# pierrebarbera/epa-ng

Measured on AMD Instinct MI355X. Metric: query placements/sec (whole node), 512-tip GTR+G4 DNA ref, preplace+thorough, higher is better.
Workload: dtype f64; 1 GPU; cfg2: 512-tip DNA GTR+G4 ref, W=1500, 150 bp reads, dyn-heur 0.99999, preplace+thorough; branches=1021, parallelism=query-shard x1 (weak)

## Files before the change

epa_ng_amd/api.py:

```python
import ctypes as C
import os

import numpy as np

HERE = os.path.dirname(os.path.abspath(__file__))
DEV_SO = os.environ.get("EPA_DEV_SO", os.path.join(HERE, "libepa_dev.so"))

__all__ = ["EpaError", "dev_lib", "device_count", "encode_queries", "Evaluator", "PAIR_DTYPE",
           "RESULT_DTYPE", "ROW_DTYPE", "DEV_SO", "Packed4", "pack_codes_4bit", "unpack_codes_4bit", "Comm",
           "comm_unique_id", "mapped_rccl_path", "comm_set_library", "comm_library_path", "comm_set_default_timeout",
           "pci_id_str", "FLAG_LOOKUP_BLOCKS", "FLAG_LOOKUP_AUTO", "LOOKUP_RESIDENT", "LOOKUP_BLOCKS", "ERR_NO_MEMORY",
           "footprint", "lookup_plan", "set_mem_cap", "quadrature_legendre01", "quadrature_laguerre", "posterior_rule",
           "profile_from_phred"]

FLAG_LOOKUP_BLOCKS = 0x40
FLAG_LOOKUP_AUTO = 0x80
LOOKUP_RESIDENT = 0
LOOKUP_BLOCKS = 1
ERR_NO_MEMORY = -10

PAIR_DTYPE = np.dtype([("branch_id", np.uint32), ("seq_id", np.uint32)])
RESULT_DTYPE = np.dtype([("lnl", np.float64), ("pendant_length", np.float64),
                         ("distal_length", np.float64)])

ROW_DTYPE = np.dtype([("branch_id", np.uint32), ("seq_id", np.uint32), ("lnl", np.float64),
                      ("pendant_length", np.float64), ("distal_length", np.float64)])


class EpaError(RuntimeError):
    def __init__(self, code, msg):
        super().__init__("epa_dev error %d: %s" % (code, msg))
        self.code = code


class _RefDesc(C.Structure):
    _fields_ = [("states", C.c_uint32), ("rate_cats", C.c_uint32), ("sites", C.c_uint32),
                ("branches", C.c_uint32),
                ("eigenvals", C.c_void_p), ("eigenvecs_u", C.c_void_p),
                ("eigenvecs_uinv", C.c_void_p), ("freqs", C.c_void_p), ("rates", C.c_void_p),
                ("rate_weights", C.c_void_p), ("prop_invar", C.c_double),
                ("prox_clv", C.c_void_p), ("prox_scaler", C.c_void_p), ("dist_clv", C.c_void_p),
                ("dist_tipchars", C.c_void_p), ("dist_scaler", C.c_void_p),
                ("branch_length", C.c_void_p),
                ("tipmap", C.c_void_p), ("tipmap_size", C.c_uint32),
                ("blo_min_branch", C.c_double), ("blo_max_branch", C.c_double),
                ("blo_default_branch", C.c_double), ("blo_epsilon", C.c_double),
                ("pendant_default", C.c_double), ("blo_max_rounds", C.c_uint32),
                ("blo_max_newton", C.c_uint32), ("flags", C.c_uint32), ("aa_x_as_n", C.c_uint32),
                ("invariant_state", C.c_void_p)]


class _Stats(C.Structure):
    _fields_ = [("pairs", C.c_uint64), ("rounds", C.c_uint64), ("newton_evals", C.c_uint64),
                ("reverts", C.c_uint64)]


class _Footprint(C.Structure):
    _fields_ = [(n, C.c_uint64) for n in ("reft", "scsum", "lookup", "lookup2", "refi", "misc", "create_temp",
                                          "reference", "bank", "steady", "peak")]


_LIB = None


def dev_lib():
    global _LIB
    if _LIB is None:
        if not os.path.exists(DEV_SO):
            raise ImportError("libepa_dev.so is missing: run `python __graft_entry__.py` "
                              "(build()) -- the HIP extension is the only compute path")
        try:
            import torch
            if torch.cuda.is_available():
                torch.cuda.init()
        except ImportError:
            pass
        L = C.CDLL(DEV_SO)
        L.epa_dev_device_count.restype = C.c_int
        L.epa_dev_create.argtypes = [C.POINTER(_RefDesc), C.c_int, C.POINTER(C.c_void_p)]
        L.epa_dev_destroy.argtypes = [C.c_void_p]
        L.epa_dev_last_error.restype = C.c_char_p
        L.epa_dev_last_error.argtypes = [C.c_void_p]
        L.epa_dev_set_stream.argtypes = [C.c_void_p, C.c_void_p]
        L.epa_dev_build_lookup.argtypes = [C.c_void_p]
        L.epa_dev_set_option.argtypes = [C.c_void_p, C.c_char_p, C.c_int]
        L.epa_encode_queries.argtypes = [C.c_uint32, C.c_uint32, C.c_uint32,
                                         C.POINTER(C.c_char_p), C.c_int, C.c_int, C.c_void_p,
                                         C.c_void_p, C.c_void_p, C.POINTER(C.c_uint32)]
        L.epa_encode_queries_compact.argtypes = [C.c_uint32, C.c_uint32, C.c_uint32,
                                                 C.POINTER(C.c_char_p), C.c_int, C.c_int, C.c_uint32,
                                                 C.c_void_p, C.c_void_p, C.c_void_p,
                                                 C.POINTER(C.c_uint32)]
        L.epa_dev_set_query_layout.argtypes = [C.c_void_p, C.c_uint32]
        L.epa_dev_preplace.argtypes = [C.c_void_p, C.c_void_p, C.c_void_p, C.c_void_p, C.c_uint32,
                                       C.c_void_p]
        L.epa_dev_preplace_bounded.argtypes = [C.c_void_p, C.c_void_p, C.c_void_p, C.c_void_p, C.c_uint32, C.c_uint32,
                                               C.c_void_p, C.c_void_p]
        L.epa_dev_preplace_screen_probe.argtypes = [C.c_void_p, C.c_void_p, C.c_void_p, C.c_void_p, C.c_uint32, C.c_uint32,
                                                    C.c_double, C.c_void_p, C.c_void_p, C.c_void_p]
        L.epa_dev_preplace_screen_runs.argtypes = [C.c_void_p]
        L.epa_dev_preplace_screen_runs.restype = C.c_uint64
        L.epa_dev_thorough.argtypes = [C.c_void_p, C.c_void_p, C.c_uint64, C.c_void_p, C.c_void_p,
                                       C.c_void_p, C.c_uint32, C.c_void_p, C.POINTER(_Stats)]
        L.epa_dev_score_at.argtypes = [C.c_void_p, C.c_void_p, C.c_void_p, C.c_void_p, C.c_void_p, C.c_uint64,
                                       C.c_void_p, C.c_void_p, C.c_void_p, C.c_uint32, C.c_void_p]
        L.epa_dev_site_lnl.argtypes = [C.c_void_p, C.c_void_p, C.c_void_p, C.c_void_p, C.c_void_p, C.c_uint64,
                                       C.c_void_p, C.c_void_p, C.c_void_p, C.c_uint32, C.c_uint32, C.c_void_p]
        L.epa_dev_rell_support.argtypes = [C.c_void_p, C.c_void_p, C.c_void_p, C.c_void_p, C.c_void_p, C.c_uint64,
                                           C.c_void_p, C.c_void_p, C.c_void_p, C.c_uint32, C.c_void_p, C.c_uint32,
                                           C.c_uint64, C.c_void_p]
        L.epa_dev_rell_tests.argtypes = L.epa_dev_rell_support.argtypes + [C.c_void_p, C.c_void_p]
        L.epa_dev_rell_au.argtypes = L.epa_dev_rell_support.argtypes[:-1] + [C.c_void_p, C.c_uint32, C.c_void_p, C.c_void_p,
                                                                             C.c_void_p]
        L.epa_dev_rell_kh.argtypes = L.epa_dev_rell_tests.argtypes
        L.epa_dev_marginal_like.argtypes = [C.c_void_p, C.c_void_p, C.c_uint64, C.c_void_p, C.c_void_p, C.c_uint32,
                                            C.c_void_p, C.c_void_p, C.c_uint32, C.c_void_p, C.c_void_p, C.c_void_p,
                                            C.c_uint32, C.c_void_p, C.c_void_p]
        L.epa_dev_preplace_profile.argtypes = [C.c_void_p, C.c_void_p, C.c_uint32, C.c_void_p, C.c_void_p, C.c_uint32,
                                               C.c_void_p]
        L.epa_dev_thorough_profile.argtypes = [C.c_void_p, C.c_void_p, C.c_uint64, C.c_void_p, C.c_uint32, C.c_void_p,
                                               C.c_void_p, C.c_uint32, C.c_void_p, C.POINTER(_Stats)]
        L.epa_dev_score_at_profile.argtypes = [C.c_void_p, C.c_void_p, C.c_void_p, C.c_void_p, C.c_void_p, C.c_uint64,
                                               C.c_void_p, C.c_uint32, C.c_void_p, C.c_void_p, C.c_uint32, C.c_void_p]
        L.epa_dev_site_lnl_profile.argtypes = [C.c_void_p, C.c_void_p, C.c_void_p, C.c_void_p, C.c_void_p, C.c_uint64,
                                               C.c_void_p, C.c_uint32, C.c_void_p, C.c_void_p, C.c_uint32, C.c_uint32,
                                               C.c_void_p]
        L.epa_dev_place_chunk_profile.argtypes = [C.c_void_p, C.c_void_p, C.c_uint32, C.c_void_p, C.c_void_p, C.c_uint32,
                                                  C.c_double, C.c_void_p, C.c_void_p, C.c_uint64, C.POINTER(C.c_uint64),
                                                  C.POINTER(_Stats)]
        L.epa_profile_from_phred.argtypes = [C.c_uint32, C.c_uint32, C.c_uint32, C.c_void_p, C.c_void_p, C.c_void_p,
                                             C.c_void_p]
        L.epa_quadrature_legendre01.argtypes = [C.c_uint32, C.c_void_p, C.c_void_p]
        L.epa_quadrature_laguerre.argtypes = [C.c_uint32, C.c_void_p, C.c_void_p]
        L.epa_dev_set_heuristic.argtypes = [C.c_void_p, C.c_int, C.c_double]
        L.epa_dev_set_query_packing.argtypes = [C.c_void_p, C.c_int]
        L.epa_pack_codes_4bit.argtypes = [C.c_void_p, C.c_uint32, C.c_uint32, C.c_void_p]
        L.epa_unpack_codes_4bit.argtypes = [C.c_void_p, C.c_uint32, C.c_uint32, C.c_void_p]
        L.epa_dev_select_candidates.argtypes = [C.c_void_p, C.c_void_p, C.c_uint32, C.c_double,
                                                C.c_void_p, C.c_uint64, C.POINTER(C.c_uint64)]
        L.epa_dev_place_chunk.argtypes = [C.c_void_p, C.c_void_p, C.c_void_p, C.c_void_p, C.c_uint32,
                                          C.c_uint32, C.c_double, C.c_void_p, C.c_void_p,
                                          C.c_uint64, C.POINTER(C.c_uint64), C.POINTER(_Stats)]
        L.epa_dev_dedup_queries.argtypes = [C.c_void_p, C.c_void_p, C.c_void_p, C.c_void_p, C.c_uint32, C.c_void_p,
                                            C.c_void_p, C.POINTER(C.c_uint32)]
        L.epa_dev_place_chunk_dedup.argtypes = [C.c_void_p, C.c_void_p, C.c_void_p, C.c_void_p, C.c_uint32, C.c_uint32,
                                                C.c_double, C.c_void_p, C.c_void_p, C.c_uint64, C.POINTER(C.c_uint64),
                                                C.POINTER(_Stats), C.c_void_p, C.c_void_p, C.POINTER(C.c_uint32)]
        L.epa_dev_chunk_stage.argtypes = [C.c_void_p, C.c_int, C.c_void_p, C.c_void_p, C.c_void_p, C.c_uint32]
        L.epa_dev_chunk_launch.argtypes = [C.c_void_p, C.c_int, C.c_uint32, C.c_double, C.c_void_p,
                                           C.c_void_p, C.c_uint64, C.c_uint32]
        L.epa_dev_chunk_launch_begin.argtypes = [C.c_void_p, C.c_int, C.c_uint32, C.c_double, C.c_void_p,
                                           C.c_void_p, C.c_uint64, C.c_uint32]
        L.epa_dev_chunk_launch_end.argtypes = [C.c_void_p, C.c_int]
        L.epa_dev_chunk_launch_many_begin.argtypes = [C.c_void_p, C.POINTER(C.c_int), C.c_int, C.c_uint32, C.c_double,
                                                      C.c_uint64, C.c_uint32]
        L.epa_dev_chunk_launch_many.argtypes = L.epa_dev_chunk_launch_many_begin.argtypes
        L.epa_dev_chunk_finish.argtypes = [C.c_void_p, C.c_int, C.POINTER(C.c_void_p),
                                           C.POINTER(C.c_void_p), C.POINTER(C.c_uint64), C.POINTER(_Stats)]
        L.epa_dev_tree_logl.argtypes = [C.c_void_p, C.c_uint32, C.POINTER(C.c_double)]
        L.epa_dev_place_all.argtypes = [C.c_void_p, C.c_void_p, C.c_void_p, C.c_void_p, C.c_uint32,
                                        C.c_uint32, C.c_double, C.c_int, C.c_uint32, C.c_uint32,
                                        C.c_void_p, C.c_void_p, C.c_void_p, C.c_void_p,
                                        C.POINTER(_Stats)]
        L.epa_comm_get_unique_id.argtypes = [C.c_void_p]
        L.epa_comm_create.argtypes = [C.c_void_p, C.c_void_p, C.c_int, C.c_int, C.c_uint32, C.c_int,
                                      C.POINTER(C.c_void_p)]
        L.epa_comm_destroy.argtypes = [C.c_void_p]
        L.epa_comm_destroy.restype = None
        L.epa_dev_gather_results.argtypes = [C.c_void_p, C.c_void_p, C.c_void_p, C.c_void_p, C.c_uint64,
                                             C.c_uint32, C.POINTER(C.c_uint64)]
        L.epa_dev_gather_slot.argtypes = [C.c_void_p, C.c_void_p, C.c_int, C.c_uint32, C.POINTER(C.c_uint64)]
        L.epa_comm_collect.argtypes = [C.c_void_p, C.c_uint64, C.POINTER(C.c_void_p), C.POINTER(C.c_uint32),
                                       C.POINTER(C.c_uint64)]
        L.epa_comm_flush.argtypes = [C.c_void_p, C.c_void_p, C.POINTER(C.c_uint64), C.POINTER(C.c_uint32)]
        L.epa_comm_carried_rows.argtypes = [C.c_void_p]
        L.epa_comm_carried_rows.restype = C.c_uint64
        L.epa_dev_gather_rows.argtypes = [C.c_void_p, C.c_void_p, C.c_void_p, C.c_uint64, C.POINTER(C.c_uint64)]
        L.epa_dev_place_all_rows.argtypes = [C.c_void_p, C.c_void_p, C.c_void_p, C.c_void_p, C.c_uint32, C.c_uint32, C.c_double,
                                             C.c_int, C.c_uint32, C.c_uint32, C.c_uint32, C.POINTER(C.c_void_p),
                                             C.POINTER(C.c_uint64), C.c_void_p]
        L.epa_comm_abort.argtypes = [C.c_void_p]
        L.epa_comm_abort.restype = None
        L.epa_comm_set_library.argtypes = [C.c_char_p]
        L.epa_comm_library_path.restype = C.c_char_p
        L.epa_comm_set_timeout.argtypes = [C.c_void_p, C.c_double]
        L.epa_comm_probe.argtypes = [C.c_void_p, C.c_void_p, C.c_double, C.POINTER(C.c_uint64)]
        L.epa_comm_set_self_send.argtypes = [C.c_void_p, C.c_int]
        L.epa_comm_device_rows.argtypes = [C.c_void_p, C.c_uint64, C.c_int]
        L.epa_comm_device_rows.restype = C.c_void_p
        L.epa_dev_mem_info.argtypes = [C.c_void_p, C.POINTER(C.c_uint64), C.POINTER(C.c_uint64)]
        L.epa_dev_xcd_shares.argtypes = [C.c_void_p, C.POINTER(C.c_double)]
        L.epa_dev_xcd_shares.restype = C.c_int
        L.epa_dev_last_kernel_ms.restype = C.c_double
        L.epa_dev_last_sclk_mhz.argtypes = [C.c_void_p]
        L.epa_dev_last_sclk_mhz.restype = C.c_double
        L.epa_dev_last_kernel_ms.argtypes = [C.c_void_p, C.c_char_p]
        L.epa_dev_footprint.argtypes = [C.c_uint32, C.c_uint32, C.c_uint64, C.c_uint64, C.c_int, C.c_int, C.c_uint32,
                                        C.c_int, C.POINTER(_Footprint)]
        L.epa_dev_lookup_plan.argtypes = [C.c_uint64, C.c_uint32, C.c_uint32, C.c_uint64, C.c_uint64, C.c_int, C.c_int,
                                          C.c_int, C.POINTER(C.c_int), C.POINTER(C.c_uint32)]
        L.epa_dev_set_mem_cap.argtypes = [C.c_uint64]
        L.epa_dev_set_mem_cap.restype = None
        L.epa_dev_lookup_mode.argtypes = [C.c_void_p, C.POINTER(C.c_int), C.POINTER(C.c_uint32)]
        _LIB = L
    return _LIB


def device_count():
    return dev_lib().epa_dev_device_count()


def footprint(states, rate_cats, sites, branches, flags=0, from_tree=False, block_branches=0, banks=1):
    L = dev_lib()
    f = _Footprint()
    rc = L.epa_dev_footprint(states, rate_cats, sites, branches, int(flags), int(from_tree), block_branches, banks,
                             C.byref(f))
    if rc:
        raise EpaError(rc, (L.epa_dev_last_error(None) or b"").decode())
    return {n: int(getattr(f, n)) for n, _ in _Footprint._fields_}


def lookup_plan(usable_bytes, states, rate_cats, sites, branches, flags=0, from_tree=False, banks=1):
    L = dev_lib()
    mode, blk = C.c_int(0), C.c_uint32(0)
    rc = L.epa_dev_lookup_plan(int(usable_bytes), states, rate_cats, sites, branches, int(flags), int(from_tree), banks,
                               C.byref(mode), C.byref(blk))
    if rc:
        raise EpaError(rc, (L.epa_dev_last_error(None) or b"").decode())
    return mode.value, blk.value


def set_mem_cap(nbytes):
    dev_lib().epa_dev_set_mem_cap(int(nbytes))


class Packed4:

    def __init__(self, data, stride):
        self.data, self.stride = data, int(stride)


def pack_codes_4bit(codes):
    codes = np.ascontiguousarray(codes, np.uint8)
    Q, stride = codes.shape
    out = np.zeros((Q, (stride + 1) // 2), np.uint8)
    rc = dev_lib().epa_pack_codes_4bit(codes.ctypes.data, Q, stride, out.ctypes.data)
    if rc:
        raise EpaError(rc, "pack_codes_4bit: a code does not fit four bits")
    return Packed4(out, stride)


def unpack_codes_4bit(p):
# ... 68 lines not shown
                                       wb.ctypes.data, ws.ctypes.data, C.byref(bad)))
    stride = (int(ws.max()) + 15) // 16 * 16
    if stride == W:
        stride += 16
    codes = np.zeros((Q, stride), np.uint8)
    check(L.epa_encode_queries_compact(states, W, Q, arr, int(premasking), int(aa_x_as_n), stride,
                                       codes.ctypes.data, wb.ctypes.data, ws.ctypes.data, C.byref(bad)))
    return codes, wb, ws


def profile_from_phred(states, codes, phred, win_span, out=None):
    codes = np.ascontiguousarray(codes, np.uint8)
    phred = np.ascontiguousarray(phred, np.uint8)
    win_span = np.ascontiguousarray(win_span, np.uint32)
    if codes.ndim != 2 or phred.shape != codes.shape or len(win_span) != codes.shape[0]:
        raise ValueError("profile_from_phred: codes and phred must be [Q][stride] arrays of one shape, win_span [Q]")
    Q, stride = codes.shape
    if out is None:
        out = np.zeros((Q, stride, states), np.float64)
    assert out.shape == (Q, stride, states) and out.dtype == np.float64 and out.flags["C_CONTIGUOUS"]
    L = dev_lib()
    rc = L.epa_profile_from_phred(states, Q, stride, codes.ctypes.data, phred.ctypes.data, win_span.ctypes.data,
                                  out.ctypes.data)
    if rc:
        raise EpaError(rc, (L.epa_dev_last_error(None) or b"").decode())
    return out


class Evaluator:

    def __init__(self, states, rates, weights, eigenvals, u, uinv, freqs, branch_length,
                 prox_clv, dist_clv, prox_scaler=None, dist_scaler=None, dist_tip=None,
                 tipmap=None, device=0, aa_x_as_n=False, pinv=0.0, invariant_state=None, flags=0):
        L = dev_lib()
        B = len(branch_length)
        self.B, self.s, self.c = B, states, len(rates)
        W = None
        for a in list(prox_clv):
            W = a.shape[0]
            break
        self.W = W
        f64 = lambda a: np.ascontiguousarray(a, dtype=np.float64)
        keep = [f64(eigenvals), f64(u), f64(uinv), f64(freqs), f64(rates), f64(weights),
                f64(branch_length)]

        def ptr_array(items, dtype):
            arr = (C.c_void_p * B)()
            held = []
            for i, it in enumerate(items if items is not None else [None] * B):
                if it is None:
                    arr[i] = None
                else:
                    a = np.ascontiguousarray(it, dtype=dtype)
                    held.append(a)
                    arr[i] = a.ctypes.data
            return arr, held

        pc, h1 = ptr_array(prox_clv, np.float64)
        dc, h2 = ptr_array(dist_clv, np.float64)
        ps, h3 = ptr_array(prox_scaler, np.uint32)
        ds, h4 = ptr_array(dist_scaler, np.uint32)
        dt, h5 = ptr_array(dist_tip, np.uint8)
        tm = np.ascontiguousarray(tipmap, dtype=np.uint32) if tipmap is not None else None
        d = _RefDesc()
        d.states, d.rate_cats, d.sites, d.branches = states, self.c, W, B
        d.eigenvals, d.eigenvecs_u, d.eigenvecs_uinv = (keep[0].ctypes.data, keep[1].ctypes.data,
                                                       keep[2].ctypes.data)
        d.freqs, d.rates, d.rate_weights = keep[3].ctypes.data, keep[4].ctypes.data, keep[5].ctypes.data
        d.prop_invar = float(pinv)
        inv = None
        if invariant_state is not None:
            inv = np.ascontiguousarray(invariant_state, dtype=np.int8)
            d.invariant_state = inv.ctypes.data
        d.prox_clv = C.cast(pc, C.c_void_p)
        d.prox_scaler = C.cast(ps, C.c_void_p)
        d.dist_clv = C.cast(dc, C.c_void_p)
        d.dist_tipchars = C.cast(dt, C.c_void_p) if dist_tip is not None else None
        d.dist_scaler = C.cast(ds, C.c_void_p)
        d.branch_length = keep[6].ctypes.data
        if tm is not None:
            d.tipmap, d.tipmap_size = tm.ctypes.data, len(tm)
        d.aa_x_as_n = int(aa_x_as_n)
        d.flags = int(flags)
        h = C.c_void_p()
        rc = L.epa_dev_create(C.byref(d), device, C.byref(h))
        if rc:
            raise EpaError(rc, L.epa_dev_last_error(None).decode())
        self.h = h
        self.L = L
        self.last_stats = None

    def close(self):
        if getattr(self, "h", None):
            self.L.epa_dev_destroy(self.h)
            self.h = None

    def __del__(self):
        self.close()

    def _check(self, rc):
        if rc:
            raise EpaError(rc, self.L.epa_dev_last_error(self.h).decode())

    def set_stream(self, stream_ptr):
        self._check(self.L.epa_dev_set_stream(self.h, stream_ptr))

    def set_option(self, key, value=1):
        self._check(self.L.epa_dev_set_option(self.h, key.encode(), int(value)))

    def build_lookup(self):
        self._check(self.L.epa_dev_build_lookup(self.h))

    def _layout(self, codes):
        packed = isinstance(codes, Packed4)
        row = codes.stride if packed else (int(codes.shape[1]) if len(codes.shape) == 2 else self.W)
        self._check(self.L.epa_dev_set_query_layout(self.h, 0 if row == self.W else row))
        self._check(self.L.epa_dev_set_query_packing(self.h, 4 if packed else 8))

    def preplace(self, codes, win_begin, win_span, Q=None, out=None):
        Q = len(win_begin) if Q is None else Q
        if out is None:
            out = np.empty((Q, self.B), np.float64)
        self._layout(codes)
        self._check(self.L.epa_dev_preplace(self.h, _ptr(codes), _ptr(win_begin), _ptr(win_span),
                                            Q, _ptr(out)))
        return out

    def preplace_bounded(self, codes, win_begin, win_span, max_span, seg_keys=False):
        Q = len(win_begin)
        out = np.empty((Q, self.B), np.float64)
        keys = np.zeros((Q, ((self.B + 63) // 64 + 7) // 8 * 8), np.uint64) if seg_keys else None
        self._layout(codes)
        self._check(self.L.epa_dev_preplace_bounded(self.h, _ptr(codes), _ptr(win_begin), _ptr(win_span), Q,
                                                    int(max_span), _ptr(out), _ptr(keys)))
        return (out, keys) if seg_keys else out

    def preplace_screen_runs(self):
        return int(self.L.epa_dev_preplace_screen_runs(self.h))

    def preplace_screen_probe(self, codes, win_begin, win_span, max_span, threshold=0.99999, arrays=True):
        Q = len(win_begin)
        nseg = (self.B + 63) // 64
        seg32 = np.full((Q, nseg), np.nan, np.float32) if arrays else None
        mask = np.zeros(Q, np.uint64) if arrays else None
        info = np.zeros(8, np.float64)
        self._layout(codes)
        self._check(self.L.epa_dev_preplace_screen_probe(self.h, _ptr(codes), _ptr(win_begin), _ptr(win_span), Q,
                                                         int(max_span), float(threshold), _ptr(seg32), _ptr(mask),
                                                         _ptr(info)))
        return {"ran": bool(info[0]), "delta": float(info[1]), "included": int(info[2]), "M": float(info[3]),
                "nonfinite": int(info[4]), "band_t": float(info[5]), "ms_screen": float(info[6]),
                "ms_band": float(info[7]), "seg32": seg32, "mask": mask}

    def thorough(self, pairs, codes, win_begin, win_span, Q=None, n_pairs=None, out=None):
        Q = len(win_begin) if Q is None else Q
        n = len(pairs) if n_pairs is None else n_pairs
        if out is None:
            out = np.empty(n, RESULT_DTYPE)
        st = _Stats()
        self._layout(codes)
        self._check(self.L.epa_dev_thorough(self.h, _ptr(pairs), n, _ptr(codes), _ptr(win_begin),
                                            _ptr(win_span), Q, _ptr(out), C.byref(st)))
        self.last_stats = {"pairs": st.pairs, "rounds": st.rounds,
                           "newton_evals": st.newton_evals, "reverts": st.reverts}
        return out

    def _entries(self, pairs, pendant, distal, proximal, codes, win_begin, Q, stream_id=None):
        n, Q = len(pairs), (len(win_begin) if Q is None else Q)
        host = (np.ndarray, list, tuple)
        pendant, distal, proximal = (np.ascontiguousarray(a, dtype=np.float64) if isinstance(a, host) else a
                                     for a in (pendant, distal, proximal))
        if isinstance(stream_id, host):
            stream_id = np.ascontiguousarray(stream_id, dtype=np.uint64)
        self._layout(codes)
        return n, Q, pendant, distal, proximal, stream_id

    @staticmethod
    def _want(who, want, table):
        want = tuple(want)
        unknown = [w for w in want if w not in table]
        if unknown:
            raise ValueError("%s: unknown output %r" % (who, unknown[0]))
        return {w: np.empty(*table[w]) for w in want}

    def score_at(self, pairs, pendant, distal, codes, win_begin, win_span, proximal=None, Q=None, out=None):
        n, Q, pendant, distal, proximal, _ = self._entries(pairs, pendant, distal, proximal, codes, win_begin, Q)
        if out is None:
            out = np.empty(n, np.float64)
        self._check(self.L.epa_dev_score_at(self.h, _ptr(pairs), _ptr(pendant), _ptr(distal), _ptr(proximal), n,
                                            _ptr(codes), _ptr(win_begin), _ptr(win_span), Q, _ptr(out)))
        return out

    def site_lnl(self, pairs, pendant, distal, codes, win_begin, win_span, proximal=None, pitch=None, Q=None, out=None):
        n, Q, pendant, distal, proximal, _ = self._entries(pairs, pendant, distal, proximal, codes, win_begin, Q)
        if pitch is None:
            pitch = int(np.max(np.asarray(win_span)[:Q])) if Q else 0
        if out is None:
            out = np.empty((n, int(pitch)), np.float64)
        self._check(self.L.epa_dev_site_lnl(self.h, _ptr(pairs), _ptr(pendant), _ptr(distal), _ptr(proximal), n,
                                            _ptr(codes), _ptr(win_begin), _ptr(win_span), Q, int(pitch), _ptr(out)))
        return out

    def marginal_like(self, pairs, codes, win_begin, win_span, x_frac, x_logw, p_len, p_logw, Q=None, out=None, grid=False):
        n, Q = self._entries(pairs, None, None, None, codes, win_begin, Q)[:2]
        x_frac, x_logw, p_len, p_logw = (np.ascontiguousarray(a, dtype=np.float64) for a in (x_frac, x_logw, p_len, p_logw))
        if x_frac.shape != x_logw.shape or p_len.shape != p_logw.shape or x_frac.ndim != 1 or p_len.ndim != 1:
            raise ValueError("marginal_like: nodes and log weights must be 1-d arrays of equal length")
        Kx, Kp = len(x_frac), len(p_len)
        if out is None:
            out = np.empty(n, np.float64)
        g = np.empty((n, Kx, Kp), np.float64) if grid else None
        self._check(self.L.epa_dev_marginal_like(self.h, _ptr(pairs), n, _ptr(x_frac), _ptr(x_logw), Kx, _ptr(p_len),
                                                 _ptr(p_logw), Kp, _ptr(codes), _ptr(win_begin), _ptr(win_span), Q,
                                                 _ptr(out), _ptr(g)))
        return (out, g) if grid else out

    def rell_support(self, pairs, pendant, distal, codes, win_begin, win_span, replicates, seed=1, stream_id=None,
                     proximal=None, Q=None, out=None):
        n, Q, pendant, distal, proximal, stream_id = self._entries(pairs, pendant, distal, proximal, codes, win_begin, Q,
                                                                   stream_id)
        if out is None:
            out = np.empty(n, np.float64)
        self._check(self.L.epa_dev_rell_support(self.h, _ptr(pairs), _ptr(pendant), _ptr(distal), _ptr(proximal), n,
                                                _ptr(codes), _ptr(win_begin), _ptr(win_span), Q, _ptr(stream_id),
                                                int(replicates), int(seed), _ptr(out)))
        return out

    def rell_tests(self, pairs, pendant, distal, codes, win_begin, win_span, replicates, seed=1, stream_id=None,
                   proximal=None, want=("support", "elw", "p_sh"), Q=None):
        out = self._want("rell_tests", want, {w: ((len(pairs),), np.float64) for w in ("support", "elw", "p_sh")})
        n, Q, pendant, distal, proximal, stream_id = self._entries(pairs, pendant, distal, proximal, codes, win_begin, Q,
                                                                   stream_id)
        self._check(self.L.epa_dev_rell_tests(self.h, _ptr(pairs), _ptr(pendant), _ptr(distal), _ptr(proximal), n,
                                              _ptr(codes), _ptr(win_begin), _ptr(win_span), Q, _ptr(stream_id),
                                              int(replicates), int(seed), _ptr(out.get("support")), _ptr(out.get("elw")),
                                              _ptr(out.get("p_sh"))))
        return out

    def rell_au(self, pairs, pendant, distal, codes, win_begin, win_span, replicates, seed=1, stream_id=None,
                proximal=None, scales=None, want=("p_au", "counts", "fit"), Q=None):
        n, S = len(pairs), (10 if scales is None else np.size(scales))
        out = self._want("rell_au", want, {"p_au": ((n,), np.float64), "counts": ((S, n), np.uint32), "fit": ((n, 2), np.float64)})
        if scales is not None:
            scales = np.ascontiguousarray(scales, dtype=np.uint32)
            if scales.ndim != 1 or len(scales) == 0:
                raise ValueError("rell_au: scales must be a non-empty 1-d array (None: the default scales)")
        n, Q, pendant, distal, proximal, stream_id = self._entries(pairs, pendant, distal, proximal, codes, win_begin, Q,
                                                                   stream_id)
        self._check(self.L.epa_dev_rell_au(self.h, _ptr(pairs), _ptr(pendant), _ptr(distal), _ptr(proximal), n,
                                           _ptr(codes), _ptr(win_begin), _ptr(win_span), Q, _ptr(stream_id),
                                           int(replicates), int(seed), _ptr(scales), 0 if scales is None else S,
                                           _ptr(out.get("p_au")), _ptr(out.get("counts")), _ptr(out.get("fit"))))
        return out

    def rell_kh(self, pairs, pendant, distal, codes, win_begin, win_span, replicates, seed=1, stream_id=None,
                proximal=None, want=("p_kh", "p_wkh", "p_wsh"), Q=None):
        out = self._want("rell_kh", want, {w: ((len(pairs),), np.float64) for w in ("p_kh", "p_wkh", "p_wsh")})
        n, Q, pendant, distal, proximal, stream_id = self._entries(pairs, pendant, distal, proximal, codes, win_begin, Q,
                                                                   stream_id)
        self._check(self.L.epa_dev_rell_kh(self.h, _ptr(pairs), _ptr(pendant), _ptr(distal), _ptr(proximal), n,
                                           _ptr(codes), _ptr(win_begin), _ptr(win_span), Q, _ptr(stream_id),
                                           int(replicates), int(seed), _ptr(out.get("p_kh")), _ptr(out.get("p_wkh")),
                                           _ptr(out.get("p_wsh"))))
        return out

    @staticmethod
    def _prof(prof):
        if isinstance(prof, np.ndarray):
            prof = np.ascontiguousarray(prof, dtype=np.float64)
        return prof, int(prof.shape[1])

    def _stats(self, st):
        self.last_stats = {"pairs": st.pairs, "rounds": st.rounds, "newton_evals": st.newton_evals, "reverts": st.reverts}

    def preplace_profile(self, prof, win_begin, win_span, Q=None, out=None):
        Q = len(win_begin) if Q is None else Q
        prof, stride = self._prof(prof)
        if out is None:
            out = np.empty((Q, self.B), np.float64)
        self._check(self.L.epa_dev_preplace_profile(self.h, _ptr(prof), stride, _ptr(win_begin), _ptr(win_span), Q, _ptr(out)))
        return out

    def thorough_profile(self, pairs, prof, win_begin, win_span, Q=None, n_pairs=None, out=None):
        Q = len(win_begin) if Q is None else Q
        n = len(pairs) if n_pairs is None else n_pairs
        prof, stride = self._prof(prof)
        if out is None:
            out = np.empty(n, RESULT_DTYPE)
        st = _Stats()
        self._check(self.L.epa_dev_thorough_profile(self.h, _ptr(pairs), n, _ptr(prof), stride, _ptr(win_begin), _ptr(win_span),
                                                    Q, _ptr(out), C.byref(st)))
        self._stats(st)
        return out

    def _profile_entries(self, pairs, pendant, distal, proximal, win_begin, Q):
        host = (np.ndarray, list, tuple)
        pendant, distal, proximal = (np.ascontiguousarray(a, dtype=np.float64) if isinstance(a, host) else a
                                     for a in (pendant, distal, proximal))
        return len(pairs), (len(win_begin) if Q is None else Q), pendant, distal, proximal

    def score_at_profile(self, pairs, pendant, distal, prof, win_begin, win_span, proximal=None, Q=None, out=None):
        n, Q, pendant, distal, proximal = self._profile_entries(pairs, pendant, distal, proximal, win_begin, Q)
        prof, stride = self._prof(prof)
        if out is None:
            out = np.empty(n, np.float64)
        self._check(self.L.epa_dev_score_at_profile(self.h, _ptr(pairs), _ptr(pendant), _ptr(distal), _ptr(proximal), n,
# ... 335 lines not shown
```

epa_ng_amd/build.py:

```python
import os
import subprocess
import sys

HERE = os.path.dirname(os.path.abspath(__file__))
ROOT = os.path.dirname(HERE)
CSRC = os.path.join(HERE, "csrc")
HIPCC = os.environ.get("HIPCC", "/opt/rocm/bin/hipcc")

DEV_SOURCES = ["epa_dev.hip", "chunk.hip", "preplace.hip", "select.hip", "thorough_dna.hip", "thorough_dna_tipd.hip", "thorough_dna_tipd2h.hip", "thorough_aa.hip", "thorough_aa_mfma.hip", "thorough_generic.hip", "score_at.hip", "marginal.hip", "rell.hip", "profile.hip", "dedup.hip", "comm.hip"]
EXTRA_FLAGS = {"thorough_dna.hip": ["-mllvm", "-amdgpu-sched-strategy=iterative-ilp"],
               "thorough_dna_tipd.hip": ["-mllvm", "-amdgpu-sched-strategy=iterative-ilp"],
               "thorough_aa_mfma.hip": ["-mllvm", "-amdgpu-sched-strategy=iterative-ilp"]}
EXTRA_DEPS = {"thorough_dna_tipd.hip": ["thorough_dna.hip"], "thorough_dna_tipd2h.hip": ["thorough_dna.hip"]}
DEV_FLAGS = ["--offload-arch=gfx950", "-O3", "-std=c++17", "-fPIC", "-I", os.path.join(ROOT, "include"),
             "-I", CSRC, "-Wall", "-Wno-unused-function", "-Wno-unused-result"]


def _newer(target, deps):
    if not os.path.exists(target):
        return True
    t = os.path.getmtime(target)
    return any(os.path.getmtime(d) > t for d in deps)


def build_dev(force=False, verbose=False):
    out = os.path.join(HERE, "libepa_dev.so")
    objdir = os.path.join(HERE, "build")
    os.makedirs(objdir, exist_ok=True)
    hdrs = [os.path.join(CSRC, "epa_dev_internal.hpp"), os.path.join(CSRC, "wave_util.hpp"), os.path.join(CSRC, "rccl_abi.hpp"),
            os.path.join(ROOT, "include", "epa_dev.h")]
    objs, procs = [], []
    for src in DEV_SOURCES:
        sp = os.path.join(CSRC, src)
        op = os.path.join(objdir, src.replace(".hip", ".o"))
        objs.append(op)
        if force or _newer(op, [sp] + hdrs + [os.path.join(CSRC, d) for d in EXTRA_DEPS.get(src, [])]):
            cmd = [HIPCC] + DEV_FLAGS + EXTRA_FLAGS.get(src, []) + ["-c", sp, "-o", op]
            if verbose:
                print(" ".join(cmd), file=sys.stderr)
            procs.append((src, subprocess.Popen(cmd), [HIPCC] + DEV_FLAGS + ["-c", sp, "-o", op]))
    for src, p, plain in procs:
        if p.wait() != 0:
            if not EXTRA_FLAGS.get(src) or subprocess.call(plain) != 0:
                raise RuntimeError("hipcc failed on " + src)
    if force or procs or _newer(out, objs):
        cmd = [HIPCC, "--offload-arch=gfx950", "-shared", "-fPIC", "-o", out + ".tmp"] + objs
        subprocess.check_call(cmd)
        os.replace(out + ".tmp", out)
    return out


HOST_SOURCES = ["model.cpp", "aa_models.cpp", "parse_model.cpp", "tree.cpp", "place.cpp", "place_ranks.cpp", "rescore.cpp", "place_profile.cpp", "place_dedup.cpp", "io.cpp", "capi.cpp"]
HOST_FLAGS = ["-O2", "-std=c++17", "-fPIC", "-fopenmp", "-Wall", "-Wextra", "-Wno-unused-parameter",
              "-I", os.path.join(ROOT, "include")]


def build_host(force=False, verbose=False):
    hdir = os.path.join(CSRC, "host")
    out = os.path.join(HERE, "libepa_host.so")
    exe = os.path.join(HERE, "epa-ng-amd")
    srcs = [os.path.join(hdir, s) for s in HOST_SOURCES]
    deps = srcs + [os.path.join(hdir, "epa_host.hpp"), os.path.join(ROOT, "include", "epa_dev.h")]
    link = ["-L", HERE, "-lepa_dev", "-Wl,-rpath,$ORIGIN"]
    if force or _newer(out, deps):
        cmd = ["g++"] + HOST_FLAGS + ["-shared", "-o", out + ".tmp"] + srcs + link
        if verbose:
            print(" ".join(cmd), file=sys.stderr)
        subprocess.check_call(cmd)
        os.replace(out + ".tmp", out)
    main = os.path.join(hdir, "main.cpp")
    if force or _newer(exe, deps + [main, out]):
        cmd = ["g++"] + HOST_FLAGS + ["-o", exe + ".tmp", main, "-L", HERE, "-lepa_host", "-lepa_dev",
                                      "-Wl,-rpath,$ORIGIN"]
        subprocess.check_call(cmd)
        os.replace(exe + ".tmp", exe)
    return out


if __name__ == "__main__":
    print(build_dev(force="--force" in sys.argv, verbose=True))
    print(build_host(force="--force" in sys.argv, verbose=True))
```

epa_ng_amd/csrc/epa_dev.hip:

```cpp
#include "epa_dev_internal.hpp"

#include <math.h>
#include <string.h>

#include <algorithm>
#include <numeric>
#include <atomic>
#include <thread>

static thread_local std::string g_create_err;

int epa_fail(epa_ctx* ctx, int code, const std::string& msg) {
  if (ctx) ctx->err = msg; else g_create_err = msg;
  return code;
}

namespace {
__global__ void __launch_bounds__(256) k_zero(uint4* __restrict__ a, size_t na, uint4* __restrict__ b, size_t nb) {
  const size_t stride = (size_t)gridDim.x * 256, i0 = (size_t)blockIdx.x * 256 + threadIdx.x;
  const uint4 z = make_uint4(0u, 0u, 0u, 0u);
  for (size_t i = i0; i < na; i += stride) a[i] = z;
  for (size_t i = i0; i < nb; i += stride) b[i] = z;
}
}
// ... 412 lines not shown
        memset(out + (hi - lo), 0, stride - (hi - lo));
      }
    }
  };
  if (nt == 1) {
    work(0);
  } else {
    std::vector<std::thread> th;
    for (unsigned t = 0; t < nt; ++t) th.emplace_back(work, t);
    for (auto& x : th) x.join();
  }
  for (unsigned t = 0; t < nt; ++t)
    if (code[t] != EPA_OK) { if (bad_query) *bad_query = bad[t]; return code[t]; }
  return EPA_OK;
}

extern "C" int epa_encode_queries(uint32_t states, uint32_t sites, uint32_t Q,
                                  const char* const* seqs, int premasking, int aa_x_as_n,
                                  uint8_t* codes, uint32_t* win_begin, uint32_t* win_span,
                                  uint32_t* bad_query) {
  return encode_impl(states, sites, Q, seqs, premasking, aa_x_as_n, false, 0, codes, win_begin, win_span,
                     bad_query);
}

extern "C" int epa_encode_queries_compact(uint32_t states, uint32_t sites, uint32_t Q,
                                          const char* const* seqs, int premasking, int aa_x_as_n,
                                          uint32_t stride, uint8_t* codes, uint32_t* win_begin,
                                          uint32_t* win_span, uint32_t* bad_query) {
  if (stride && !codes) return EPA_ERR_INVALID_ARG;
  return encode_impl(states, sites, Q, seqs, premasking, aa_x_as_n, true, stride, codes, win_begin,
                     win_span, bad_query);
}

namespace {
void tridiag_eigenvalues(const std::vector<double>& d, const std::vector<double>& o, std::vector<double>& ev) {
  const size_t K = d.size();
  double lo = d[0], hi = d[0];
  for (size_t i = 0; i < K; ++i) {
    const double r = (i ? std::fabs(o[i - 1]) : 0.0) + (i + 1 < K ? std::fabs(o[i]) : 0.0);
    lo = std::min(lo, d[i] - r);
    hi = std::max(hi, d[i] + r);
  }
  auto below = [&](double x) {
    size_t n = 0;
    double q = 1.0;
    for (size_t i = 0; i < K; ++i) {
      q = d[i] - x - (i ? o[i - 1] * o[i - 1] / q : 0.0);
      if (q == 0.0) q = 1e-300;
      if (q < 0.0) ++n;
    }
    return n;
  };
  ev.resize(K);
  for (size_t j = 0; j < K; ++j) {
    double a = lo, b = hi;
    for (int it = 0; it < 200 && b - a > 4e-16 * std::max(std::fabs(a), std::fabs(b)); ++it) {
      const double mid = 0.5 * (a + b);
      if (below(mid) > j) b = mid; else a = mid;
    }
    ev[j] = 0.5 * (a + b);
  }
}

double log_sum_exp(const double* v, uint32_t K) {
  double mx = v[0], sum = 0.0;
  for (uint32_t j = 1; j < K; ++j) mx = std::max(mx, v[j]);
  for (uint32_t j = 0; j < K; ++j) sum += std::exp(v[j] - mx);
  return mx + std::log(sum);
}
}

extern "C" int epa_quadrature_legendre01(uint32_t K, double* nodes, double* log_weights) {
  if (K < 1 || K > 64 || !nodes || !log_weights) return EPA_ERR_INVALID_ARG;
  std::vector<double> d(K, 0.0), o(K > 1 ? K - 1 : 0), x;
  for (uint32_t i = 1; i < K; ++i) o[i - 1] = (double)i / std::sqrt(4.0 * i * i - 1.0);
  tridiag_eigenvalues(d, o, x);
  for (uint32_t j = 0; j < K; ++j) {
    double t = x[j], dp = 1.0;
    for (int it = 0; it < 3; ++it) {
      double p0 = 1.0, p1 = t;
      for (uint32_t n = 1; n < K; ++n) { const double p2 = ((2.0 * n + 1.0) * t * p1 - n * p0) / (n + 1.0); p0 = p1; p1 = p2; }
      dp = K * (t * p1 - p0) / (t * t - 1.0);
      if (it < 2) t -= p1 / dp;
    }
    nodes[j] = 0.5 * (1.0 + t);
    log_weights[j] = -std::log((1.0 - t) * (1.0 + t)) - 2.0 * std::log(std::fabs(dp));
  }
  const double norm = log_sum_exp(log_weights, K);
  for (uint32_t j = 0; j < K; ++j) log_weights[j] -= norm;
  return EPA_OK;
}

extern "C" int epa_quadrature_laguerre(uint32_t K, double* nodes, double* log_weights) {
  if (K < 1 || K > 64 || !nodes || !log_weights) return EPA_ERR_INVALID_ARG;
  std::vector<double> d(K), o(K > 1 ? K - 1 : 0), x;
  for (uint32_t i = 0; i < K; ++i) d[i] = 2.0 * i + 1.0;
  for (uint32_t i = 1; i < K; ++i) o[i - 1] = (double)i;
  tridiag_eigenvalues(d, o, x);
  for (uint32_t j = 0; j < K; ++j) {
    double t = x[j], lm = 1.0;
    for (int it = 0; it < 3; ++it) {
      double l0 = 1.0, l1 = 1.0 - t;
      for (uint32_t n = 1; n < K; ++n) { const double l2 = ((2.0 * n + 1.0 - t) * l1 - n * l0) / (n + 1.0); l0 = l1; l1 = l2; }
      lm = l0;
      if (it < 2) t -= l1 * t / (K * (l1 - l0));
    }
    nodes[j] = t;
    log_weights[j] = std::log(t) - 2.0 * std::log((double)K) - 2.0 * std::log(std::fabs(lm));
  }
  const double norm = log_sum_exp(log_weights, K);
  for (uint32_t j = 0; j < K; ++j) log_weights[j] -= norm;
  return EPA_OK;
}

extern "C" int epa_dev_device_count(void) {
  int n = 0;
  if (hipGetDeviceCount(&n) != hipSuccess) { (void)hipGetLastError(); return 0; }
  return n;
}

extern "C" const char* epa_dev_last_error(const epa_ctx* ctx) {
  return ctx ? ctx->err.c_str() : g_create_err.c_str();
}

extern "C" int epa_dev_set_query_layout(epa_ctx* ctx, uint32_t code_stride) {
  if (!ctx) return EPA_ERR_INVALID_ARG;
  ctx->code_stride = code_stride;
  return EPA_OK;
}

extern "C" int epa_dev_set_option(epa_ctx* ctx, const char* key, int value) {
  if (!ctx || !key) return EPA_ERR_INVALID_ARG;
  if (strcmp(key, "lookup_block") == 0) {
    if (!ctx->lookup_blocks) return epa_fail(ctx, EPA_ERR_INVALID_ARG, "set_option: lookup_block needs a context in the blocked lookup layout");
    if (value <= 0 || (value & 63)) return epa_fail(ctx, EPA_ERR_INVALID_ARG, "set_option: lookup_block must be a positive multiple of 64");
    for (void* p : ctx->blk_buf)
      if (p) return epa_fail(ctx, EPA_ERR_INVALID_ARG, "set_option: lookup_block must be set before the first preplacement");
    ctx->lookup_block = (uint32_t)value;
    return EPA_OK;
  }
  const bool dedup_key = strcmp(key, "dedup_key_bits") == 0;
  if (dedup_key || strcmp(key, "dedup_sort_bits") == 0) {
    if (value < 0 || value > 64) return epa_fail(ctx, EPA_ERR_INVALID_ARG, std::string("set_option: ") + key + " must be 0 .. 64");
    (dedup_key ? ctx->opt.dedup_key_bits : ctx->opt.dedup_sort_bits) = value;
    return EPA_OK;
  }
  struct Entry { const char* name; int EpaOptions::*field; };
  static const Entry table[] = {
      {"thorough_generic", &EpaOptions::thorough_generic}, {"preplace_generic", &EpaOptions::preplace_generic},
      {"select_full_rows", &EpaOptions::select_full_rows}, {"select_sort", &EpaOptions::select_sort},
      {"queued_thorough", &EpaOptions::queued_thorough},   {"xcd_balance", &EpaOptions::xcd_balance},
      {"aa_valu", &EpaOptions::aa_valu},                   {"timers", &EpaOptions::timers},
      {"newton_lds", &EpaOptions::newton_lds},             {"tip_distal", &EpaOptions::tip_distal},
      {"preplace_screen", &EpaOptions::preplace_screen},   {"preplace_screen_scale", &EpaOptions::preplace_screen_scale}};
  for (const Entry& e : table)
    if (strcmp(key, e.name) == 0) {
      ctx->opt.*e.field = value;
      ctx->generic_thorough = ctx->generic_native || ctx->opt.thorough_generic != 0;
      return EPA_OK;
    }
  return epa_fail(ctx, EPA_ERR_INVALID_ARG, std::string("set_option: unknown key '") + key + "'");
}

extern "C" int epa_dev_set_heuristic(epa_ctx* ctx, int mode, double param) {
  if (!ctx) return EPA_ERR_INVALID_ARG;
  if (mode < EPA_HEUR_DYNAMIC || mode > EPA_HEUR_BASEBALL)
    return epa_fail(ctx, EPA_ERR_INVALID_ARG, "set_heuristic: unknown mode");
  if (mode == EPA_HEUR_FIXED && !(param >= 0.0 && param <= 1.0))
    return epa_fail(ctx, EPA_ERR_INVALID_ARG, "set_heuristic: the fraction must lie in [0, 1]");
  ctx->heur_mode = mode;
  ctx->heur_param = param;
  return EPA_OK;
}

extern "C" int epa_dev_set_query_packing(epa_ctx* ctx, int bits) {
  if (!ctx) return EPA_ERR_INVALID_ARG;
  if (bits != 8 && bits != 4) return epa_fail(ctx, EPA_ERR_INVALID_ARG, "set_query_packing: 8 or 4 bits per code");
  if (bits == 4 && ctx->s != 4)
    return epa_fail(ctx, EPA_ERR_UNSUPPORTED, "set_query_packing: the 4-bit format holds nucleotide codes only");
  ctx->code_packed4 = bits == 4;
  return EPA_OK;
}

extern "C" int epa_pack_codes_4bit(const uint8_t* codes, uint32_t Q, uint32_t stride, uint8_t* packed) {
  if (!codes || !packed) return EPA_ERR_INVALID_ARG;
  const size_t ps = ((size_t)stride + 1) / 2;
  const unsigned cap = g_encode_threads.load(std::memory_order_relaxed);
  const unsigned hw = cap ? cap : std::max(1u, std::thread::hardware_concurrency());
  const unsigned nt = (unsigned)std::min<uint64_t>(std::min(hw, 32u), std::max<uint64_t>(1, (uint64_t)Q * stride >> 20));
  std::vector<int> bad(nt, 0);
  auto work = [&](unsigned t) {
    const uint32_t q0 = (uint32_t)((uint64_t)Q * t / nt), q1 = (uint32_t)((uint64_t)Q * (t + 1) / nt);
    unsigned over = 0;
    for (uint32_t q = q0; q < q1; ++q) {
      const uint8_t* r = codes + (size_t)q * stride;
      uint8_t* o = packed + (size_t)q * ps;
      for (uint32_t p = 0; p < stride / 2; ++p) {
        const uint8_t hi = r[2 * p], lo = r[2 * p + 1];
        over |= hi | lo;
        o[p] = (uint8_t)((hi << 4) | lo);
      }
      if (stride & 1) { const uint8_t hi = r[stride - 1]; over |= hi; o[ps - 1] = (uint8_t)(hi << 4); }
    }
    bad[t] = over > 15;
  };
  if (nt == 1) work(0);
  else {
    std::vector<std::thread> th;
    for (unsigned t = 0; t < nt; ++t) th.emplace_back(work, t);
    for (auto& x : th) x.join();
  }
  for (unsigned t = 0; t < nt; ++t) if (bad[t]) return EPA_ERR_INVALID_ARG;
  return EPA_OK;
}

extern "C" int epa_unpack_codes_4bit(const uint8_t* packed, uint32_t Q, uint32_t stride, uint8_t* codes) {
  if (!codes || !packed) return EPA_ERR_INVALID_ARG;
  const size_t ps = ((size_t)stride + 1) / 2;
  for (uint32_t q = 0; q < Q; ++q)
    for (uint32_t i = 0; i < stride; ++i) {
      const uint8_t b = packed[(size_t)q * ps + i / 2];
      codes[(size_t)q * stride + i] = (i & 1) ? (b & 15u) : (b >> 4);
    }
  return EPA_OK;
}

extern "C" int epa_dev_set_stream(epa_ctx* ctx, void* s) {
  if (!ctx) return EPA_ERR_INVALID_ARG;
  ctx->stream = (hipStream_t)s;
  return EPA_OK;
}

extern "C" void epa_dev_destroy(epa_ctx* ctx) {
  if (!ctx) return;
  (void)hipSetDevice(ctx->device);
  (void)hipDeviceSynchronize();
  for (int i = 0; i < epa_ctx::N_BANKS * epa_ctx::N_SCRATCH; ++i) if (ctx->scratch[i]) (void)hipFree(ctx->scratch[i]);
  if (ctx->refT) (void)hipFree(ctx->refT);
  if (ctx->scSum) (void)hipFree(ctx->scSum);
  if (ctx->blen) (void)hipFree(ctx->blen);
  if (ctx->lookup) (void)hipFree(ctx->lookup);
  if (ctx->lookup2) (void)hipFree(ctx->lookup2);
  if (ctx->lookup2f) (void)hipFree(ctx->lookup2f);
  if (ctx->prof_tab) (void)hipFree(ctx->prof_tab);
  for (void* p : ctx->blk_buf) if (p) (void)hipFree(p);
  for (auto& v : ctx->blk_ev) for (hipEvent_t e : v) if (e) (void)hipEventDestroy(e);
  if (ctx->th_ctr) (void)hipFree(ctx->th_ctr);
  for (hipEvent_t e : ctx->ev_rb) if (e) (void)hipEventDestroy(e);
  if (ctx->refI) (void)hipFree(ctx->refI);
  if (ctx->cinv) (void)hipFree(ctx->cinv);
  if (ctx->resc0) (void)hipFree(ctx->resc0);
  if (ctx->tip_row) (void)hipFree(ctx->tip_row);
  if (ctx->tipmask) (void)hipFree(ctx->tipmask);
  if (ctx->tipd) (void)hipFree(ctx->tipd);
  for (hipStream_t st : ctx->side_stream) if (st) (void)hipStreamDestroy(st);
  for (hipEvent_t e : ctx->ev_fork) if (e) (void)hipEventDestroy(e);
  for (hipEvent_t e : ctx->ev_join) if (e) (void)hipEventDestroy(e);
  if (ctx->dmodel) (void)hipFree(ctx->dmodel);
  for (ChunkSlot& sl : ctx->slots) {
    if (sl.h_in) (void)hipHostFree(sl.h_in);
    if (sl.h_out) (void)hipHostFree(sl.h_out);
    if (sl.h_stats) (void)hipHostFree(sl.h_stats);
    if (sl.h_sel) (void)hipHostFree(sl.h_sel);
    if (sl.d_in) (void)hipFree(sl.d_in);
    if (sl.d_unpacked) (void)hipFree(sl.d_unpacked);
    if (sl.d_pairs) (void)hipFree(sl.d_pairs);
    if (sl.d_res) (void)hipFree(sl.d_res);
    if (sl.d_stats) (void)hipFree(sl.d_stats);
    if (sl.d_merge) (void)hipFree(sl.d_merge);
    if (sl.d_gpairs) (void)hipFree(sl.d_gpairs);
    if (sl.d_gres) (void)hipFree(sl.d_gres);
    if (sl.d_goff) (void)hipFree(sl.d_goff);
    if (sl.h_goff) (void)hipHostFree(sl.h_goff);
    for (hipEvent_t e : {sl.ev_up, sl.ev_done, sl.ev_down, sl.ev_base}) if (e) (void)hipEventDestroy(e);
    if (sl.stream) (void)hipStreamDestroy(sl.stream);
  }
  if (ctx->copy_stream) (void)hipStreamDestroy(ctx->copy_stream);
  if (ctx->down_stream) (void)hipStreamDestroy(ctx->down_stream);
  std::vector<EvTimer*> ts = {&ctx->t_lookup};
  for (auto& bk : ctx->t_bank) for (auto& t : bk) ts.push_back(&t);
  for (auto* t : ts) { if (t->a) (void)hipEventDestroy(t->a); if (t->b) (void)hipEventDestroy(t->b); }
  delete ctx;
}

static int precompute_from_tree(epa_ctx* ctx, const epa_tree_desc* t, const uint32_t* d_tipmap);

static int padded_cats(int s, int c_in, uint32_t flags, bool from_tree) {
  int c = (c_in == 1 || c_in == 2) ? 4 : c_in;
  if (s == 4 && c_in >= 3 && (c_in & 3)) c = (c_in + 3) & ~3;
  if (s == 20 && (c_in == 3 || (c_in >= 5 && c_in <= 7))) c = (c_in + 3) & ~3;
  if (c_in >= 3 && c != c_in && (flags & EPA_FLAG_RATE_SCALERS) && !from_tree) c = c_in;
  return c;
}

static bool tuned_thorough_shape(int s, int c, uint32_t flags, bool zero0) {
  const bool sliding = !(flags & EPA_FLAG_RAXML_BLO);
  const bool dna_groups = s == 4 && (c & 3) == 0 && c <= 16;
  const bool tuned_local = (s == 4 && zero0) || s == 20;
  const bool tuned_cats = c == 4 || (dna_groups && sliding && zero0) || (s == 20 && c == 8);
  return tuned_cats && (sliding || tuned_local) &&
         !(flags & (EPA_FLAG_NEWTON_SLOW_BISECT | EPA_FLAG_NEWTON_STRICT_DF | EPA_FLAG_KEEP_EIGENVALUES));
}

static std::atomic<uint64_t> g_mem_cap{0};
extern "C" void epa_dev_set_mem_cap(uint64_t bytes) { g_mem_cap.store(bytes, std::memory_order_relaxed); }

constexpr uint32_t EPA_BLOCK_DEFAULT = 1024;
// ... 682 lines not shown

extern "C" int epa_dev_create(const epa_ref_desc* desc, int device, epa_ctx** out) {
  if (!desc || !out) return epa_fail(nullptr, EPA_ERR_INVALID_ARG, "null argument");
  *out = nullptr;
  if (epa_dev_device_count() <= 0)
    return epa_fail(nullptr, EPA_ERR_NO_DEVICE,
                    "no HIP device visible: libepa_dev has no CPU fallback by design");
  epa_ctx* ctx = new epa_ctx();
  int rc = create_impl(desc, device, ctx);
  if (rc != EPA_OK) {
    g_create_err = ctx->err;
    epa_dev_destroy(ctx);
    return rc;
  }
  *out = ctx;
  return EPA_OK;
}

extern "C" int epa_dev_build_lookup(epa_ctx* ctx) {
  if (!ctx) return EPA_ERR_INVALID_ARG;
  if (ctx->lookup_built || ctx->lookup_blocks) return EPA_OK;
  EPA_HIP(ctx, hipSetDevice(ctx->device));
  int rc = launch_build_lookup(ctx);
  if (rc) return rc;
  EPA_HIP(ctx, hipStreamSynchronize(ctx->stream));
  ctx->lookup_built = true;
  return EPA_OK;
}

const uint32_t* host_view(const uint32_t* p, size_t n, std::vector<uint32_t>& buf, hipStream_t st) {
  if (!epa_is_device_ptr(p)) return p;
  buf.resize(n);
  (void)hipStreamSynchronize(st);
  if (hipMemcpy(buf.data(), p, n * sizeof(uint32_t), hipMemcpyDeviceToHost) != hipSuccess)
    return nullptr;
  return buf.data();
}

static int check_windows(epa_ctx* ctx, const uint32_t* hb, const uint32_t* hs, uint32_t Q,
                         uint32_t* max_span, bool allow_empty = false) {
  uint32_t mx = 0;
  for (uint32_t q = 0; q < Q; ++q) {
    if (hs[q] == 0 && !allow_empty)
      return epa_fail(ctx, EPA_ERR_QUERY_ALL_GAP,
                      "Sequence " + std::to_string(q) + " does not appear to have any non-gap sites!");
    if ((uint64_t)hb[q] + hs[q] > ctx->W)
      return epa_fail(ctx, EPA_ERR_QUERY_WIDTH,
                      "Query sequence length not same as reference alignment!");
    mx = std::max(mx, hs[q]);
  }
  if (ctx->code_stride && mx > ctx->code_stride)
    return epa_fail(ctx, EPA_ERR_INVALID_ARG, "a window is longer than the compact code stride");
  *max_span = mx;
  return EPA_OK;
}

extern "C" int epa_dev_preplace(epa_ctx* ctx, const uint8_t* q_codes, const uint32_t* win_begin,
                                const uint32_t* win_span, uint32_t Q, double* lnl) {
  return epa_dev_preplace_bounded(ctx, q_codes, win_begin, win_span, Q, 0, lnl, nullptr);
}

extern "C" int epa_dev_preplace_bounded(epa_ctx* ctx, const uint8_t* q_codes, const uint32_t* win_begin,
                                        const uint32_t* win_span, uint32_t Q, uint32_t max_span, double* lnl,
                                        uint64_t* seg_keys) {
  if (!ctx || !q_codes || !win_begin || !win_span || !lnl)
    return epa_fail(ctx, EPA_ERR_INVALID_ARG, "null argument");
  if (Q == 0) return EPA_OK;
  EPA_HIP(ctx, hipSetDevice(ctx->device));
  int rc = epa_dev_build_lookup(ctx);
  if (rc) return rc;
  if (max_span > ctx->W) max_span = ctx->W;
  if (max_span && !epa_is_device_ptr(win_span))
    for (uint32_t q = 0; q < Q; ++q)
      if (win_span[q] > max_span) return epa_fail(ctx, EPA_ERR_INVALID_ARG, "preplace: a window is longer than max_span");
  const uint32_t nseg = (ctx->B + 63) / 64, segp = (nseg + 7u) & ~7u;
  unsigned long long* d_seg = nullptr;
  if (seg_keys) {
    if (nseg > 64) return epa_fail(ctx, EPA_ERR_INVALID_ARG, "preplace: segment maxima exist up to 4096 branches");
    d_seg = (unsigned long long*)epa_scratch(ctx, SLOT_SEGMAX, sizeof(unsigned long long) * (size_t)Q * segp);
    if (!d_seg) return epa_fail(ctx, EPA_ERR_HIP, "hipMalloc(segment maxima)");
  }
  const uint8_t* d_codes = epa_codes_to_device(ctx, q_codes, Q);
  const uint32_t* d_begin = (const uint32_t*)epa_to_device(ctx, SLOT_BEGIN, win_begin, sizeof(uint32_t) * Q);
  const uint32_t* d_span = (const uint32_t*)epa_to_device(ctx, SLOT_SPAN, win_span, sizeof(uint32_t) * Q);
  if (!d_codes || !d_begin || !d_span) return epa_fail(ctx, EPA_ERR_HIP, "query upload failed");
  const bool out_dev = epa_is_device_ptr(lnl);
  double* d_lnl = out_dev ? lnl : (double*)epa_scratch(ctx, SLOT_TABLE, sizeof(double) * (size_t)Q * ctx->B);
  if (!d_lnl) return epa_fail(ctx, EPA_ERR_HIP, "hipMalloc(lnl)");
  const uint32_t* d_status = nullptr;
  rc = launch_preplace(ctx, d_codes, d_begin, d_span, Q, PreTable{d_lnl, ctx->B, d_seg, segp}, max_span, &d_status);
  if (rc) return rc;
  if (!out_dev)
    EPA_HIP(ctx, hipMemcpyAsync(lnl, d_lnl, sizeof(double) * (size_t)Q * ctx->B,
                                hipMemcpyDeviceToHost, ctx->stream));
  if (d_seg)
    EPA_HIP(ctx, hipMemcpyAsync(seg_keys, d_seg, sizeof(unsigned long long) * (size_t)Q * segp,
                                epa_is_device_ptr(seg_keys) ? hipMemcpyDeviceToDevice : hipMemcpyDeviceToHost, ctx->stream));
  EPA_HIP(ctx, hipStreamSynchronize(ctx->stream));
  return preplace_check_status(ctx, d_status);
}

extern "C" uint64_t epa_dev_preplace_screen_runs(const epa_ctx* ctx) { return ctx ? ctx->screen_runs : 0; }

extern "C" int epa_dev_preplace_screen_probe(epa_ctx* ctx, const uint8_t* q_codes, const uint32_t* win_begin,
                                             const uint32_t* win_span, uint32_t Q, uint32_t max_span, double threshold,
                                             float* seg32, uint64_t* seg_mask, double* info) {
  if (!ctx || !q_codes || !win_begin || !win_span || !info)
    return epa_fail(ctx, EPA_ERR_INVALID_ARG, "null argument");
  for (int i = 0; i < 8; ++i) info[i] = 0.0;
  if (Q == 0) return EPA_OK;
  EPA_HIP(ctx, hipSetDevice(ctx->device));
  int rc = epa_dev_build_lookup(ctx);
  if (rc) return rc;
  if (max_span > ctx->W) max_span = ctx->W;
  if (max_span && !epa_is_device_ptr(win_span))
    for (uint32_t q = 0; q < Q; ++q)
      if (win_span[q] > max_span) return epa_fail(ctx, EPA_ERR_INVALID_ARG, "preplace: a window is longer than max_span");
  if (ctx->s == 4 && ctx->lookup2 && (rc = launch_build_lookup2f(ctx))) return rc;
  const uint8_t* d_codes = epa_codes_to_device(ctx, q_codes, Q);
  const uint32_t* d_begin = (const uint32_t*)epa_to_device(ctx, SLOT_BEGIN, win_begin, sizeof(uint32_t) * Q);
  const uint32_t* d_span = (const uint32_t*)epa_to_device(ctx, SLOT_SPAN, win_span, sizeof(uint32_t) * Q);
  if (!d_codes || !d_begin || !d_span) return epa_fail(ctx, EPA_ERR_HIP, "query upload failed");
  PreScreenProbe probe;
  probe.band_t = epa_select_band_t(threshold, ctx->B);
  const uint32_t* d_status = nullptr;
  rc = launch_preplace(ctx, d_codes, d_begin, d_span, Q, PreTable{}, max_span, &d_status, &probe);
  if (rc) return rc;
  EPA_HIP(ctx, hipStreamSynchronize(ctx->stream));
  if ((rc = preplace_check_status(ctx, d_status))) return rc;
  info[0] = probe.ran ? 1.0 : 0.0;
  info[3] = ctx->screen_M;
  info[4] = (double)ctx->screen_nonfinite;
  info[5] = probe.band_t;
  if (!probe.ran) return EPA_OK;
  const uint32_t nseg = (ctx->B + 63) / 64, segp = (nseg + 7u) & ~7u;
  unsigned long long n_incl = 0;
  EPA_HIP(ctx, hipMemcpy(&n_incl, probe.n_incl, sizeof(n_incl), hipMemcpyDeviceToHost));
  info[1] = probe.delta;
  info[2] = (double)n_incl;
  info[6] = probe.ms_screen;
  info[7] = probe.ms_band;
  if (seg_mask) EPA_HIP(ctx, hipMemcpy(seg_mask, probe.mask, sizeof(uint64_t) * Q, hipMemcpyDeviceToHost));
  if (seg32) {
    std::vector<uint32_t> keys((size_t)Q * segp);
    EPA_HIP(ctx, hipMemcpy(keys.data(), probe.seg32, sizeof(uint32_t) * keys.size(), hipMemcpyDeviceToHost));
    for (uint32_t q = 0; q < Q; ++q)
      for (uint32_t s = 0; s < nseg; ++s) {
        const uint32_t k = keys[(size_t)q * segp + s], u = (k >> 31) ? (k & 0x7fffffffu) : ~k;
        float v = NAN;
        if (k) memcpy(&v, &u, 4);
        seg32[(size_t)q * nseg + s] = v;
      }
  }
  return EPA_OK;
}

extern "C" int epa_dev_thorough(epa_ctx* ctx, const epa_pair* pairs, uint64_t n_pairs,
                                const uint8_t* q_codes, const uint32_t* win_begin,
                                const uint32_t* win_span, uint32_t Q, epa_result* out,
                                epa_thorough_stats* stats) {
  if (!ctx || !q_codes || !win_begin || !win_span || (n_pairs && (!pairs || !out)))
    return epa_fail(ctx, EPA_ERR_INVALID_ARG, "null argument");
  if (stats) memset(stats, 0, sizeof(*stats));
  if (n_pairs == 0) return EPA_OK;
  EPA_HIP(ctx, hipSetDevice(ctx->device));
  if (ctx->refI) {
    int brc = epa_dev_build_lookup(ctx);
    if (brc) return brc;
  }
  std::vector<uint32_t> hb_buf, hs_buf;
  const uint32_t* hb = host_view(win_begin, Q, hb_buf, ctx->stream);
  const uint32_t* hs = host_view(win_span, Q, hs_buf, ctx->stream);
  if (!hb || !hs) return epa_fail(ctx, EPA_ERR_HIP, "cannot read window arrays");
  uint32_t max_span = 0;
  int rc = check_windows(ctx, hb, hs, Q, &max_span);
  if (rc) return rc;
  if (!epa_is_device_ptr(pairs)) {
    for (uint64_t i = 0; i < n_pairs; ++i)
      if (pairs[i].branch_id >= ctx->B || pairs[i].seq_id >= Q)
        return epa_fail(ctx, EPA_ERR_INVALID_ARG, "pair index out of range");
  }
  const uint8_t* d_codes = epa_codes_to_device(ctx, q_codes, Q);
  const uint32_t* d_begin = (const uint32_t*)epa_to_device(ctx, SLOT_BEGIN, win_begin, sizeof(uint32_t) * Q);
  const uint32_t* d_span = (const uint32_t*)epa_to_device(ctx, SLOT_SPAN, win_span, sizeof(uint32_t) * Q);
  const epa_pair* d_pairs = (const epa_pair*)epa_to_device(ctx, SLOT_PAIRS, pairs, sizeof(epa_pair) * n_pairs);
  if (!d_codes || !d_begin || !d_span || !d_pairs)
    return epa_fail(ctx, EPA_ERR_HIP, "thorough input upload failed");
  const bool out_dev = epa_is_device_ptr(out);
  epa_result* d_out = out_dev ? out : (epa_result*)epa_scratch(ctx, SLOT_RESULTS, sizeof(epa_result) * n_pairs);
  unsigned long long* d_stats = (unsigned long long*)epa_scratch(ctx, SLOT_STATS, 256);
  if (!d_out || !d_stats) return epa_fail(ctx, EPA_ERR_HIP, "hipMalloc(thorough out)");
  rc = epa_zero_async(ctx, d_stats, 128);
  if (rc) return rc;
  rc = launch_thorough(ctx, d_pairs, n_pairs, d_codes, d_begin, d_span, max_span, d_out, d_stats);
  if (rc) return rc;
  unsigned long long hst[16];
  if (!out_dev)
    EPA_HIP(ctx, hipMemcpyAsync(out, d_out, sizeof(epa_result) * n_pairs, hipMemcpyDeviceToHost,
                                ctx->stream));
  if (!out_dev || stats) {
    EPA_HIP(ctx, hipMemcpyAsync(hst, d_stats, 128, hipMemcpyDeviceToHost, ctx->stream));
    EPA_HIP(ctx, hipStreamSynchronize(ctx->stream));
    return chunk_stats(ctx, n_pairs, hst, stats);
  }
  return EPA_OK;
}


namespace {

struct EntryArgs {
  const epa_pair* pairs;
  const double *pendant, *distal, *proximal;
  uint64_t n;
  const uint8_t* q_codes;
  const uint32_t *win_begin, *win_span;
  uint32_t Q;
  const double* prof = nullptr;
  uint32_t prof_stride = 0;
};

struct EntryCall {
  epa_ctx* ctx;
  const char* who;
  EntryArgs a;
  EntryStage st;
  std::vector<uint32_t> hb_buf, hs_buf;
  const uint64_t* d_sid = nullptr;
  bool empty = false;
  struct Out { void *user, *dev; size_t bytes; } out[3] = {};
  int n_out = 0;

  int stage() {
    const uint32_t* hb = host_view(a.win_begin, a.Q, hb_buf, ctx->stream);
    st.h_span = host_view(a.win_span, a.Q, hs_buf, ctx->stream);
    if (!hb || !st.h_span) return epa_fail(ctx, EPA_ERR_HIP, "cannot read window arrays");
    int rc = a.prof ? (int)EPA_OK : check_windows(ctx, hb, st.h_span, a.Q, &st.max_span, true);
    if (rc) return rc;
    const bool hp = !epa_is_device_ptr(a.pairs), hpe = a.pendant && !epa_is_device_ptr(a.pendant);
    const bool hd = a.distal && !epa_is_device_ptr(a.distal), hx = a.proximal && !epa_is_device_ptr(a.proximal);
    auto bad = [&](uint64_t i, const char* what) {
      return epa_fail(ctx, EPA_ERR_INVALID_ARG, std::string(who) + ": entry " + std::to_string(i) + ": " + what);
    };
    auto length_ok = [](double t) { return std::isfinite(t) && t >= 0.0; };
    for (uint64_t i = 0; i < a.n; ++i) {
      if (hp && a.pairs[i].branch_id >= ctx->B) return bad(i, "branch id out of range");
      if (hp && a.pairs[i].seq_id >= a.Q) return bad(i, "sequence id out of range");
      if (hpe && !length_ok(a.pendant[i])) return bad(i, "pendant length is negative or not finite");
      if (hd && !length_ok(a.distal[i])) return bad(i, "distal length is negative or not finite");
      if (hx && !length_ok(a.proximal[i])) return bad(i, "proximal length is negative or not finite");
      if (!a.proximal && hp && hd && a.distal[i] > ctx->h_blen[a.pairs[i].branch_id])
        return bad(i, "distal length beyond the branch's length");
    }
    auto lengths = [&](int slot, const double* t) { return t ? (const double*)epa_to_device(ctx, slot, t, sizeof(double) * a.n) : nullptr; };
    st.n = a.n;
    st.Q = a.Q;
    st.d_begin = (const uint32_t*)epa_to_device(ctx, SLOT_BEGIN, a.win_begin, sizeof(uint32_t) * a.Q);
    st.d_span = (const uint32_t*)epa_to_device(ctx, SLOT_SPAN, a.win_span, sizeof(uint32_t) * a.Q);
    if (a.prof) {
      if (!st.d_span) return epa_fail(ctx, EPA_ERR_HIP, std::string(who) + " input upload failed");
      const double* d_prof = nullptr;
      rc = epa_profile_stage(ctx, who, a.prof, a.prof_stride, hb, st.h_span, st.d_span, a.Q, true, &st.max_span, &d_prof, &st.d_qe);
      if (rc) return rc;
      st.qe_stride = a.prof_stride;
    } else {
      st.d_codes = epa_codes_to_device(ctx, a.q_codes, a.Q);
    }
    st.d_pairs = (const epa_pair*)epa_to_device(ctx, SLOT_PAIRS, a.pairs, sizeof(epa_pair) * a.n);
    st.d_pen = lengths(SLOT_PENDANT, a.pendant);
    st.d_dis = lengths(SLOT_DISTAL, a.distal);
    st.d_prx = lengths(SLOT_PROXIMAL, a.proximal);
    if ((!st.d_codes && !st.d_qe) || !st.d_begin || !st.d_span || !st.d_pairs || (a.pendant && !st.d_pen) || (a.distal && !st.d_dis) ||
        (a.proximal && !st.d_prx))
      return epa_fail(ctx, EPA_ERR_HIP, std::string(who) + " input upload failed");
    return EPA_OK;
  }

  template <class Checks>
  int begin(std::initializer_list<const void*> need, const uint64_t* const* stream_id, Checks own_checks) {
    bool null_arg = !ctx || (a.n && (!a.pairs || (!a.q_codes && !a.prof) || !a.win_begin || !a.win_span));
    for (const void* p : need) null_arg |= a.n && !p;
    if (null_arg) return epa_fail(ctx, EPA_ERR_INVALID_ARG, "null argument");
    int rc = own_checks();
    if (rc) return rc;
    empty = a.n == 0;
    if (empty) return EPA_OK;
    if (stream_id && a.n > 0xffffffffull)
      return epa_fail(ctx, EPA_ERR_INVALID_ARG, std::string(who) + ": more than 2^32 - 1 entries in one call");
    EPA_HIP(ctx, hipSetDevice(ctx->device));
    rc = stage();
    if (rc) return rc;
    if (stream_id && *stream_id) {
      d_sid = (const uint64_t*)epa_to_device(ctx, SLOT_RELL_STREAMS, *stream_id, sizeof(uint64_t) * a.Q);
      if (!d_sid) return epa_fail(ctx, EPA_ERR_HIP, std::string(who) + " input upload failed");
    }
    return EPA_OK;
  }
  int check_replicates(uint32_t replicates) {
    if (replicates == 0 || replicates > (1u << 20))
      return epa_fail(ctx, EPA_ERR_INVALID_ARG, std::string(who) + ": replicates must be 1 .. 2^20");
    return EPA_OK;
  }

  void output(void* p, size_t bytes) { out[n_out++] = Out{p, p && epa_is_device_ptr(p) ? p : nullptr, bytes}; }
  template <class T> T* dev(int i) const { return (T*)out[i].dev; }
  template <class Launch>
// ... 489 lines not shown
```

epa_ng_amd/csrc/epa_dev_internal.hpp:

```cpp
#pragma once

#include <hip/hip_runtime.h>
#include <stdint.h>

#include <algorithm>
#include <cmath>
#include <string>
#include <vector>

#include <rocprim/device/device_radix_sort.hpp>

#include "epa_dev.h"

using epa_radix_cfg = rocprim::radix_sort_config<rocprim::default_config, rocprim::default_config,
                                                 rocprim::default_config, 0>;

#define EPA_MAX_STATES 20
#define EPA_MAX_CATS 16
#define EPA_MAX_COLS 24
#define EPA_GRID_Y 65535u

struct ModelDNA {
  double U[16];
  double Ui[16];
// ... 65 lines not shown
inline double epa_select_band_x(double threshold, uint32_t B) { return 1.0 - std::log((1.0 - threshold) / (double)B); }
inline double epa_select_band_t(double threshold, uint32_t B) {
  return std::max(epa_select_band_x(threshold, B), std::log((double)B) + 38.0);
}

bool epa_select_takes_seg(const epa_ctx* ctx, const PreTable& t, uint32_t Q, double threshold);

struct SelectPending {
  PreTable table;
  const uint32_t* pre_status = nullptr;
  uint32_t Q = 0, cap = 0;
  double threshold = 0.0;
  epa_pair* d_pairs = nullptr;
  uint64_t max_pairs = 0;
  const uint32_t* d_span = nullptr;
  unsigned long long *stage = nullptr, *keys_a = nullptr, *keys_b = nullptr;
  uint32_t *counts = nullptr, *offsets = nullptr;
  uint32_t *bitmap = nullptr, *boffs = nullptr;
  uint32_t wpr = 0;
  void* temp = nullptr;
  size_t sort_bytes = 0;
  uint32_t* rb = nullptr;
  bool have_status = false;
  hipEvent_t ev_rb = nullptr;
  const uint32_t* d_rb = nullptr;
  bool emitted = false;
  int queued_cls = -1;
  uint32_t cls_hist[EPA_N_CLSX] = {};
  bool have_hist = false;
  bool tip_split = false;
};

enum class SlotState : int {
  Free,
  Staged,
  Begun,
  Launched,
  GroupMember,
};
constexpr int EPA_MAX_GROUP = 8;

struct ChunkInputs {
  const uint8_t* codes;
  const uint32_t *begin, *span;
};

struct __attribute__((visibility("hidden"))) ChunkSlot {
  void* h_in = nullptr;
  size_t h_in_sz = 0;
  void* d_in = nullptr;
  const uint8_t* x_codes = nullptr;
  const uint32_t* x_begin = nullptr;
  const uint32_t* x_span = nullptr;
  size_t d_in_sz = 0;
  uint8_t* d_unpacked = nullptr;
  size_t d_unpacked_sz = 0;
  size_t codes_bytes = 0;
  uint32_t Q = 0, stride = 0;
  bool packed4 = false;
  epa_pair* d_pairs = nullptr;
  epa_result* d_res = nullptr;
  size_t d_pairs_sz = 0, d_res_sz = 0;
  void* h_out = nullptr;
  size_t h_out_sz = 0;
  unsigned long long* h_stats = nullptr;
  unsigned long long* d_stats = nullptr;
  hipEvent_t ev_up = nullptr, ev_done = nullptr, ev_down = nullptr, ev_base = nullptr;
  hipStream_t stream = nullptr;
  const epa_pair* out_pairs = nullptr;
  const epa_result* out_res = nullptr;
  uint64_t n = 0;
  SlotState state = SlotState::Free;
  bool unfinished() const { return state == SlotState::Begun || state == SlotState::Launched || state == SlotState::GroupMember; }
  ChunkInputs staged_inputs() const {
    if (x_codes) return {x_codes, x_begin, x_span};
    const char* d = (const char*)d_in;
    const uint32_t* b = (const uint32_t*)(d + codes_bytes);
    return {(const uint8_t*)d, b, b + Q};
  }
  SelectPending sel;
  uint32_t* h_sel = nullptr;
  const uint8_t* l_codes = nullptr;
  const uint32_t *l_begin = nullptr, *l_span = nullptr;
  epa_pair* l_pairs = nullptr;
  epa_result* l_res = nullptr;
  uint32_t l_max_span = 0, l_flags = 0;
  int leader = -1;
  int g_index = 0;
  int g_n = 0;
  int g_left = 0;
  int g_slots[EPA_MAX_GROUP] = {};
  uint32_t g_qoff[EPA_MAX_GROUP + 1] = {};
  uint32_t own_Q = 0;
  const uint8_t* own_x_codes = nullptr;
  const uint32_t *own_x_begin = nullptr, *own_x_span = nullptr;
  void* d_merge = nullptr;
  size_t d_merge_sz = 0;
  epa_pair* d_gpairs = nullptr;
  epa_result* d_gres = nullptr;
  size_t g_cap = 0;
  uint32_t* d_goff = nullptr;
  uint32_t* h_goff = nullptr;

  void lead_merged(uint32_t total, const uint8_t* codes, const uint32_t* begin, const uint32_t* span) {
    own_Q = Q; own_x_codes = x_codes; own_x_begin = x_begin; own_x_span = x_span;
    Q = total; x_codes = codes; x_begin = begin; x_span = span;
  }
  void restore_own() { Q = own_Q; x_codes = own_x_codes; x_begin = own_x_begin; x_span = own_x_span; }
  void group_begun(ChunkSlot* all, const int* slots, int n, const uint32_t* qoff) {
    g_n = n;
    for (int i = 0; i <= n; ++i) g_qoff[i] = qoff[i];
    for (int i = 0; i < n; ++i) {
      g_slots[i] = slots[i];
      all[slots[i]].leader = slots[0];
      all[slots[i]].g_index = i;
      if (i) all[slots[i]].state = SlotState::GroupMember;
    }
  }
  void group_launched(ChunkSlot* all) {
    restore_own();
    g_left = g_n;
    for (int i = 1; i < g_n; ++i) {
      all[g_slots[i]].state = SlotState::Launched;
      all[g_slots[i]].l_flags = l_flags;
    }
  }
  void launch_over(ChunkSlot* all, SlotState to) {
    state = to;
    if (g_n <= 1) return;
    restore_own();
    for (int i = 0; i < g_n; ++i) {
      all[g_slots[i]].leader = -1;
      if (i) all[g_slots[i]].state = to;
    }
    g_n = 0;
    g_left = 0;
  }
};

struct EpaOptions {
  int thorough_generic = 0;
  int preplace_generic = 0;
  int select_full_rows = 0;
  int select_sort = 0;
  int queued_thorough = 0;
  int xcd_balance = 1;
  int aa_valu = 0;
  int timers = 1;
  int newton_lds = 0;
  int tip_distal = 1;
  int dedup_key_bits = 64;
  int preplace_screen = 1;
  int preplace_screen_scale = 1;
  int dedup_sort_bits = 32;
};

struct epa_ctx {
  int device = 0;
  EpaOptions opt;
  int n_cu = 256;
  hipStream_t stream = nullptr;
  std::string err;

  int s = 0, c = 0, ncols = 0;
  int c_in = 0;
  uint32_t W = 0, B = 0;
  ModelDev hmodel;
  ModelDev* dmodel = nullptr;
  ModelDNA dna;
  bool dna_zero0 = false;
  bool rate_scalers = false;
  bool generic_thorough = false;
  bool generic_native = false;
  BloConsts blo;
  int aa_x_as_n = 0;
  uint32_t code_stride = 0;

  double* refT = nullptr;
  uint32_t* scSum = nullptr;
  double* blen = nullptr;
  double* lookup = nullptr;
  double* refI = nullptr;
  uint8_t* resc0 = nullptr;
  double* cinv = nullptr;
  double inv_w0 = 0.0;
  double* lookup2 = nullptr;
  float2* lookup2f = nullptr;
  bool lookup2f_refused = false;
  uint64_t screen_runs = 0;
  double screen_M = 0.0;
  uint64_t screen_nonfinite = 0;
  uint32_t* tip_row = nullptr;
  uint8_t* tipmask = nullptr;
  double* tipd = nullptr;
  bool lookup_built = false;
  double* prof_tab = nullptr;
  bool lookup_blocks = false;
  uint32_t lookup_block = 1024;
  std::vector<double> h_blen;

  static constexpr int N_SCRATCH = 26;
  static constexpr int N_SLOTS = 24;
  static constexpr int N_BANKS = 1 + N_SLOTS;
  int bank = 0;
  void* scratch[N_BANKS * N_SCRATCH] = {};
  size_t scratch_sz[N_BANKS * N_SCRATCH] = {};

  uint32_t select_cap = 64;
  uint32_t* th_ctr = nullptr;
  bool code_packed4 = false;
  int heur_mode = 0;
  double heur_param = 0.0;

  hipStream_t copy_stream = nullptr, down_stream = nullptr;
  ChunkSlot slots[N_SLOTS];

  enum { T_PREPLACE = 0, T_THOROUGH = 1, T_SELECT = 2, T_SCORE = 3, T_SITES = 4, T_RELL = 5, T_MARGINAL = 6, T_RELL_TESTS = 7, T_RELL_AU = 8, T_RELL_KH = 9, T_PREPLACE_PROFILE = 10, T_DEDUP = 11, N_TIMERS = 12 };
  EvTimer t_lookup;
  std::vector<hipEvent_t> blk_ev[N_BANKS];
  uint32_t blk_ev_n[N_BANKS] = {};
  void* blk_buf[N_BANKS] = {};
  size_t blk_sz[N_BANKS] = {};
  EvTimer t_bank[N_BANKS][N_TIMERS];
  uint32_t xcd_cum[9] = {0u, 1u << 17, 2u << 17, 3u << 17, 4u << 17, 5u << 17, 6u << 17, 7u << 17, 1u << 20};
  double xcd_w[8] = {0.125, 0.125, 0.125, 0.125, 0.125, 0.125, 0.125, 0.125};
  double last_sclk_mhz = 0.0;
  bool xstamp_ok = false;
  hipEvent_t ev_rb[N_BANKS] = {};
  hipStream_t side_stream[N_BANKS] = {};
  hipEvent_t ev_fork[N_BANKS] = {}, ev_join[N_BANKS] = {};
  const void* clean_stats[N_BANKS] = {};
  bool clean_ctr[N_BANKS] = {};
  int t_last[N_TIMERS] = {};
  epa_thorough_stats last_stats{};
};

int epa_fail(epa_ctx* ctx, int code, const std::string& msg);
void* epa_scratch(epa_ctx* ctx, int slot, size_t bytes);
inline size_t align256(size_t x) { return (x + 255) & ~(size_t)255; }
struct Carver {
  char* base = nullptr;
  size_t off = 0;
  void* tail(size_t bytes) { char* p = base ? base + off : nullptr; off += bytes; return p; }
  template <typename T> T* take(size_t n) { return static_cast<T*>(tail(align256(sizeof(T) * n))); }
};
inline uint32_t* epa_th_ctr(epa_ctx* ctx) { return ctx->th_ctr ? ctx->th_ctr + 64 * ctx->bank : nullptr; }
int epa_zero_async(epa_ctx* ctx, void* p, size_t bytes, void* p2 = nullptr, size_t bytes2 = 0);
inline int epa_th_ctr_reset(epa_ctx* ctx, size_t bytes = 64) {
  if (ctx->clean_ctr[ctx->bank]) { ctx->clean_ctr[ctx->bank] = false; return 0; }
  return epa_zero_async(ctx, epa_th_ctr(ctx), bytes);
}
bool epa_is_device_ptr(const void* p);
const void* epa_to_device(epa_ctx* ctx, int slot, const void* p, size_t bytes);
const uint8_t* epa_codes_to_device(epa_ctx* ctx, const uint8_t* q_codes, uint32_t Q);
__attribute__((visibility("hidden"))) void launch_unpack4(hipStream_t st, const uint8_t* d_packed, uint8_t* d_codes, uint32_t Q, uint32_t stride);
__attribute__((visibility("hidden"))) const uint32_t* host_view(const uint32_t* p, size_t n, std::vector<uint32_t>& buf, hipStream_t st);
void epa_xcd_feedback(epa_ctx* ctx, uint64_t n_pairs, const unsigned long long* hst);
__attribute__((visibility("hidden"))) int chunk_stats(epa_ctx* ctx, uint64_t n, const unsigned long long* hst, epa_thorough_stats* stats);
#define EPA_XSTAMP_MASK 0x7ffffffffffull
void epa_timer_start(epa_ctx* ctx, EvTimer& t);
void epa_timer_stop(epa_ctx* ctx, EvTimer& t);
inline EvTimer& epa_t(epa_ctx* ctx, int which) { ctx->t_last[which] = ctx->bank; return ctx->t_bank[ctx->bank][which]; }

#define EPA_HIP(ctx, call)                                                               \
  do {                                                                                    \
    hipError_t e__ = (call);                                                              \
    if (e__ != hipSuccess)                                                                \
      return epa_fail(ctx, EPA_ERR_HIP, std::string(#call) + ": " + hipGetErrorString(e__)); \
  } while (0)

enum EpaSlot : int {
  SLOT_CODES = 0,
  SLOT_BEGIN = 1,
  SLOT_SPAN = 2,
  SLOT_OUT = 3,
  SLOT_PAIRS = 4,
  SLOT_CLV_PROX = 0,
  SLOT_CLV_DIST = 1,
  SLOT_TIPMAP = 2,
  SLOT_SCALER_PROX = 3,
  SLOT_SCALER_DIST = 4,
  SLOT_TABLE = 3,
  SLOT_RESULTS = 5,
  SLOT_PREPLACE = 6,
  SLOT_STATS = 6,
  SLOT_SELECT = 7,
  SLOT_NEWTON = 7,
  SLOT_CLASS_SORT = 8,
  SLOT_TREE_LNL = 9,
  SLOT_TH_TIMING = 9,
  SLOT_SEGMAX = 10,
  SLOT_PACKED4 = 10,
  SLOT_ROWS_OUT = 11,
  SLOT_ROWS = 12,
  SLOT_PENDANT = 7,
  SLOT_DISTAL = 8,
  SLOT_PROXIMAL = 9,
  SLOT_MG_RULE = 7,
  SLOT_MG_WAVES = 9,
  SLOT_RELL_SORT = 13,
  SLOT_RELL_BOUNDS = 14,
  SLOT_RELL_GROUPS = 15,
  SLOT_RELL_ROWS = 16,
  SLOT_RELL_STREAMS = 17,
  SLOT_RELL_TESTS = 18,
  SLOT_RELL_AU = 19,
  SLOT_RELL_KH = 20,
  SLOT_PROFILE = 21,
  SLOT_PROFILE_EIGEN = 22,
  SLOT_DEDUP = 23,
  SLOT_DEDUP_IN = 24,
  SLOT_DEDUP_ROWS = 25,
};

struct EntryStage {
  const epa_pair* d_pairs = nullptr;
  const double *d_pen = nullptr, *d_dis = nullptr, *d_prx = nullptr;
  uint64_t n = 0;
  const uint8_t* d_codes = nullptr;
  const uint32_t *d_begin = nullptr, *d_span = nullptr;
  const uint32_t* h_span = nullptr;
  const double* d_qe = nullptr;
  uint32_t qe_stride = 0;
  uint32_t Q = 0;
  uint32_t max_span = 0;
};

__host__ __device__ inline bool epa_tip_class_ok(int cls) { return cls <= 2 || cls == 10 || cls == 11; }
__host__ __device__ inline int epa_tip_class(int cls) { return cls <= 2 ? 12 + cls : cls == 10 ? 15 : cls == 11 ? 16 : cls; }
__host__ __device__ inline int epa_base_class(int key) { return key < 12 ? key : key <= 14 ? key - 12 : key == 15 ? 10 : 11; }
inline bool epa_tipd_active(const epa_ctx* ctx) {
  return ctx->tip_row && ctx->opt.tip_distal && ctx->s == 4 && !ctx->generic_thorough && ctx->dna.ng == 1 &&
         ctx->dna_zero0 && ctx->blo.sliding && !ctx->cinv;
}
constexpr uint32_t EPA_AA_LDS_MAX_SPAN = 102;
__host__ __device__ inline int epa_span_class(int states, uint32_t span) {
  if (states != 4) return span <= 64 ? 0 : span <= 128 ? 1 : span <= 192 ? 2 : 3;
  if (span > 64 && span <= 96) return 10;
  if (span > 128 && span <= 160) return 11;
  const uint32_t nch = (span + 63) / 64;
  return nch <= 4 ? (nch ? (int)nch - 1 : 0) : nch <= 6 ? 4 : nch <= 8 ? 5 : nch <= 12 ? 6 : nch <= 16 ? 7 : nch <= 24 ? 8 : 9;
}

int launch_transform(epa_ctx* ctx, const double* d_clv_or_null, const uint8_t* d_tip_or_null,
                     const uint32_t* d_tipmap, uint32_t tipmap_size, double* dst);
int launch_build_lookup(epa_ctx* ctx);
int launch_build_lookup2(epa_ctx* ctx);
int launch_build_lookup2f(epa_ctx* ctx);
double epa_screen_delta(const epa_ctx* ctx, uint32_t span_bound);
struct PreScreenProbe {
  double band_t = 0.0;
  bool ran = false;
  double delta = 0.0;
  const uint32_t* seg32 = nullptr;
  const unsigned long long* mask = nullptr;
  const unsigned long long* n_incl = nullptr;
  float ms_screen = -1.f, ms_band = -1.f;
};
uint32_t epa_block_branches(const epa_ctx* ctx);
size_t epa_block_bytes(int s, uint32_t W, uint32_t blk, size_t* off2);
void* epa_block_buffer(epa_ctx* ctx);
int launch_build_lookup_block(epa_ctx* ctx, uint32_t b0, uint32_t nb, double* blk_lookup);
int launch_build_lookup2_block(epa_ctx* ctx, uint32_t nb, const double* blk_lookup, double* blk_lookup2);
int launch_preplace(epa_ctx* ctx, const uint8_t* d_codes, const uint32_t* d_begin, const uint32_t* d_span, uint32_t Q,
                    const PreTable& t, uint32_t max_span, const uint32_t** d_status, PreScreenProbe* probe = nullptr);
int preplace_check_status(epa_ctx* ctx, const uint32_t* d_status);
__attribute__((visibility("hidden"))) int preplace_window_error(epa_ctx* ctx, const uint32_t* st);
__attribute__((visibility("hidden"))) void launch_scan_counts(epa_ctx* ctx, uint32_t* cnt, uint32_t K, const uint32_t* tip_row = nullptr,
                                                               uint32_t* tip_total = nullptr);
int launch_thorough(epa_ctx* ctx, const epa_pair* d_pairs, uint64_t n_pairs, const uint8_t* d_codes,
                    const uint32_t* d_begin, const uint32_t* d_span, uint32_t max_span,
                    epa_result* d_out, unsigned long long* d_stats,
                    const uint32_t* cls_hist = nullptr);
int launch_thorough_queued(epa_ctx* ctx, const epa_pair* d_pairs, const uint32_t* d_spec, uint64_t max_pairs,
                           const uint8_t* d_codes, const uint32_t* d_begin, const uint32_t* d_span, uint32_t max_span,
                           epa_result* d_out, unsigned long long* d_stats);
int launch_select_emit(epa_ctx* ctx, SelectPending* sp);
int launch_thorough_aa(epa_ctx* ctx, const epa_pair* d_pairs, const uint32_t* d_order, uint64_t n_pairs,
                       const uint8_t* d_codes, const uint32_t* d_begin, const uint32_t* d_span,
                       uint32_t max_span, bool want_lds, epa_result* d_out, unsigned long long* d_stats);
int launch_thorough_generic(epa_ctx* ctx, const epa_pair* d_pairs, uint64_t n_pairs, const uint8_t* d_codes,
                            const uint32_t* d_begin, const uint32_t* d_span, uint32_t max_span,
                            epa_result* d_out, unsigned long long* d_stats,
                            const uint32_t* d_order = nullptr, bool caller_times = false,
                            const double* d_qe = nullptr, uint32_t qe_stride = 0);
int launch_thorough_aa_mfma(epa_ctx* ctx, const epa_pair* d_pairs, const uint32_t* d_order, uint64_t n_pairs,
                            const uint8_t* d_codes, const uint32_t* d_begin, const uint32_t* d_span,
                            uint32_t max_span, epa_result* d_out, unsigned long long* d_stats);
__attribute__((visibility("hidden"))) uint32_t epa_column_mask(int s, int col);
__attribute__((visibility("hidden"))) int epa_profile_stage(epa_ctx* ctx, const char* who, const double* prof, uint32_t stride,
                                                            const uint32_t* hb, const uint32_t* hs, const uint32_t* d_span, uint32_t Q,
                                                            bool allow_empty, uint32_t* max_span, const double** d_prof, const double** d_qe);
int launch_score_at(epa_ctx* ctx, const EntryStage& e, double* d_lnl);
enum SiteLnlFlags : unsigned { SITES_PLAIN = 0u, SITES_PAD = 1u, SITES_TIMED = 2u };
int launch_site_lnl(epa_ctx* ctx, const EntryStage& e, const uint32_t* d_order, uint64_t n_rows, uint32_t pitch,
                    double* d_rows, unsigned flags);
struct RellDraws {
  const uint64_t* d_stream_id;
  uint32_t replicates;
  uint64_t seed;
};
int launch_rell(epa_ctx* ctx, const EntryStage& e, const RellDraws& dr, double* d_support);
int launch_rell_tests(epa_ctx* ctx, const EntryStage& e, const RellDraws& dr, double* d_support, double* d_elw, double* d_p_sh);
int launch_rell_au(epa_ctx* ctx, const EntryStage& e, const RellDraws& dr, const uint32_t* h_scale_pm, uint32_t n_scales,
                   double* d_p_au, uint32_t* d_counts, double* d_fit);
__attribute__((visibility("hidden"))) int launch_rell_kh(epa_ctx* ctx, const EntryStage& e, const RellDraws& dr, double* d_p_kh, double* d_p_wkh, double* d_p_wsh);
int launch_marginal(epa_ctx* ctx, const EntryStage& e, const double* d_rule, uint32_t Kx, uint32_t Kp, double* d_marginal,
                    double* d_grid);
int launch_select(epa_ctx* ctx, const PreTable& t, const uint32_t* pre_status, uint32_t Q, double threshold,
                  epa_pair* d_pairs, uint64_t max_pairs, uint64_t* n_pairs,
                  const uint32_t* d_span = nullptr);
int launch_select_begin(epa_ctx* ctx, const PreTable& t, const uint32_t* pre_status, uint32_t Q, double threshold,
                        epa_pair* d_pairs, uint64_t max_pairs, const uint32_t* d_span, uint32_t* rb, SelectPending* sp);
int launch_select_end(epa_ctx* ctx, SelectPending* sp, uint64_t* n_pairs);
int select_check_status(epa_ctx* ctx, const SelectPending* sp);
```

epa_ng_amd/csrc/preplace.hip:

```cpp
#include "epa_dev_internal.hpp"
#include "wave_util.hpp"

#include <cstdlib>
#include <cstring>

#include <algorithm>

namespace {

constexpr int GQ = 256;
constexpr int CH = 160;
constexpr int SPREAD = 96;
constexpr int TROWS = CH + SPREAD;
constexpr int NB = 16;
constexpr int CW = CH / 4;

struct Group {
  uint32_t start;
  uint32_t count;
  uint32_t min_begin;
  uint32_t cls;
};

__device__ __forceinline__ void validate_window(uint32_t i, uint32_t begin, uint32_t span, uint32_t W,
                                                uint32_t cmax, uint32_t* status) {
  if (span == 0) atomicMax(&status[0], 0x80000000u | i);
  else if ((uint64_t)begin + span > W || span > cmax) atomicMax(&status[1], 0x80000000u | i);
}
__global__ void k_validate(const uint32_t* __restrict__ win_begin, const uint32_t* __restrict__ win_span,
                           uint32_t Q, uint32_t W, uint32_t cmax, uint32_t* __restrict__ status) {
  const uint32_t i = blockIdx.x * blockDim.x + threadIdx.x;
  if (i < Q) validate_window(i, win_begin[i], win_span[i], W, cmax, status);
}

__global__ void k_iota(uint32_t* v, uint32_t n) {
  const uint32_t i = blockIdx.x * blockDim.x + threadIdx.x;
  if (i < n) v[i] = i;
}

__global__ void __launch_bounds__(256) k_count_keys(const uint32_t* __restrict__ keys, uint32_t Q,
                                                    uint32_t* __restrict__ cnt, uint32_t* __restrict__ rank) {
  const uint32_t q = blockIdx.x * 256 + threadIdx.x;
  if (q < Q) rank[q] = atomicAdd(&cnt[keys[q]], 1u);
}
__global__ void __launch_bounds__(1024) k_scan_counts(uint32_t* __restrict__ cnt, uint32_t K,
                                                      const uint32_t* __restrict__ tip_row = nullptr,
                                                      uint32_t* __restrict__ tip_total = nullptr) {
  __shared__ uint32_t wsum[16];
  __shared__ uint32_t carry_s;
  __shared__ uint32_t tips_s;
  const uint32_t t = threadIdx.x, lane = t & 63u, wv = t >> 6;
  if (t == 0) { carry_s = 0; tips_s = 0; }
  __syncthreads();
  constexpr uint32_t PER = 8;
  uint32_t tips = 0;
  for (uint32_t base = 0; base < K; base += 1024 * PER) {
    uint32_t v[PER], tot = 0;
#pragma unroll
    for (uint32_t i = 0; i < PER; ++i) {
      const uint32_t k = base + t * PER + i;
      v[i] = k < K ? cnt[k] : 0u;
      tot += v[i];
      if (tip_row && k + 1 < K && tip_row[k] != 0xffffffffu) tips += v[i];
    }
    uint32_t inc = tot;
#pragma unroll
    for (int o = 1; o < 64; o <<= 1) {
      const uint32_t u = __shfl_up(inc, o);
      if ((int)lane >= o) inc += u;
    }
    if (lane == 63) wsum[wv] = inc;
    __syncthreads();
    uint32_t before = carry_s;
    for (uint32_t w = 0; w < wv; ++w) before += wsum[w];
    uint32_t run = before + inc - tot;
#pragma unroll
    for (uint32_t i = 0; i < PER; ++i) {
      const uint32_t k = base + t * PER + i;
      if (k < K) cnt[k] = run;
      run += v[i];
    }
    __syncthreads();
    if (t == 1023) carry_s = run;
    __syncthreads();
  }
  if (tip_total) {
    if (tips) atomicAdd(&tips_s, tips);
    __syncthreads();
    if (t == 0) *tip_total = tips_s;
  }
}
__global__ void __launch_bounds__(256) k_scatter_sorted(const uint32_t* __restrict__ keys,
                                                        const uint32_t* __restrict__ rank,
                                                        const uint32_t* __restrict__ offs, uint32_t Q,
                                                        uint32_t* __restrict__ sorted_keys,
                                                        uint32_t* __restrict__ perm) {
  const uint32_t q = blockIdx.x * 256 + threadIdx.x;
  if (q >= Q) return;
  const uint32_t k = keys[q], pos = offs[k] + rank[q];
  sorted_keys[pos] = k;
  perm[pos] = q;
}

__global__ void __launch_bounds__(256) k_make_groups(const uint32_t* __restrict__ sorted_keys, uint32_t Q,
                                                     uint32_t Wp, uint32_t n_blocks,
                                                     uint32_t class_blocks, uint32_t gq0, uint32_t gq1,
                                                     uint32_t spr0, uint32_t max_runs, Group* __restrict__ groups,
                                                     uint32_t max_groups, uint32_t* __restrict__ status,
                                                     const uint32_t* __restrict__ n_dev = nullptr, uint32_t seg_div = 0) {
  extern __shared__ uint32_t sh[];
  if (n_dev) Q = min(Q, *n_dev);
  uint32_t* lo = sh;
  uint32_t* runbase = lo + n_blocks + 1;
  uint32_t* run_start = runbase + n_blocks + 1;
  uint32_t* run_end = run_start + max_runs;
  uint32_t* run_off = run_end + max_runs;
  auto lower_bound = [&](uint32_t a, uint32_t b, uint64_t key) {
    while (a < b) {
      const uint32_t m = (a + b) >> 1;
      if ((uint64_t)sorted_keys[m] < key) a = m + 1; else b = m;
    }
    return a;
  };
  for (uint32_t k = threadIdx.x; k <= n_blocks; k += blockDim.x)
    lo[k] = k == n_blocks ? Q : lower_bound(0, Q, (uint64_t)k * Wp);
  for (uint32_t i = threadIdx.x; i < max_groups; i += blockDim.x) groups[i] = Group{0, 0, 0, 0};
  __syncthreads();
  if (threadIdx.x == 0) {
    uint32_t r = 0;
    for (uint32_t b = 0; b < n_blocks; ++b) {
      const uint32_t gq = b >= class_blocks ? gq1 : gq0;
      runbase[b] = r;
      r += (lo[b + 1] - lo[b] + gq - 1) / gq;
    }
    runbase[n_blocks] = r;
  }
  __syncthreads();
  const uint32_t nruns = min(runbase[n_blocks], max_runs);
  for (uint32_t r = threadIdx.x; r < nruns; r += blockDim.x) {
    uint32_t b = 0;
    while (b + 1 < n_blocks && r >= runbase[b + 1]) ++b;
    const uint32_t gq = b >= class_blocks ? gq1 : gq0;
    const uint32_t start = lo[b] + (r - runbase[b]) * gq, end = min(lo[b + 1], start + gq);
    const uint32_t k0 = sorted_keys[start], k1 = sorted_keys[end - 1];
    const uint32_t spr = b >= class_blocks ? (uint32_t)SPREAD : spr0;
    run_start[r] = start;
    run_end[r] = end;
    run_off[r] = (k1 - k0 < spr) ? 1u : (k1 / spr - k0 / spr + 1);
  }
  __syncthreads();
  uint32_t* cnt = run_off + max_runs + 1;
  for (uint32_t r = threadIdx.x; r < nruns; r += blockDim.x) cnt[r] = run_off[r];
  __syncthreads();
  for (uint32_t r = threadIdx.x; r <= nruns; r += blockDim.x) {
    uint32_t g = 0;
    for (uint32_t i = 0; i < r; ++i) g += cnt[i];
    run_off[r] = g;
  }
  __syncthreads();
  if (threadIdx.x == 0) {
    const uint32_t r1 = class_blocks < n_blocks ? min(runbase[class_blocks], nruns) : nruns;
    status[4] = min(run_off[nruns], max_groups);
    status[5] = min(run_off[r1], max_groups);
  }
  for (uint32_t r = threadIdx.x; r < nruns; r += blockDim.x) {
    uint32_t b = 0;
    while (b + 1 < n_blocks && r >= runbase[b + 1]) ++b;
    const uint32_t cls = b >= class_blocks ? 1u : 0u;
    const uint32_t start = run_start[r], end = run_end[r], g0 = run_off[r], n = run_off[r + 1] - g0;
    if (n == 1) {
      if (g0 < max_groups) groups[g0] = Group{start, end - start, seg_div ? sorted_keys[start] / seg_div : 0u, cls};
    } else {
      const uint32_t spr = cls ? (uint32_t)SPREAD : spr0;
      const uint32_t kb = sorted_keys[start] / spr;
      uint32_t a = start;
      for (uint32_t k = 0; k < n; ++k) {
        const uint32_t e = k + 1 == n ? end : lower_bound(a, end, (uint64_t)(kb + k + 1) * spr);
        if (g0 + k < max_groups) groups[g0 + k] = Group{a, e - a, (seg_div && e > a) ? sorted_keys[a] / seg_div : 0u, cls};
        a = e;
      }
    }
  }
}

template <int NCOLS, bool ACC>
__global__ void __launch_bounds__(GQ, ACC ? 2 : 4) k_preplace(const double* __restrict__ lookup,
                                                 const uint8_t* __restrict__ codes,
                                                 const uint32_t* __restrict__ win_begin,
                                                 const uint32_t* __restrict__ win_span,
                                                 const uint32_t* __restrict__ perm,
                                                 const Group* __restrict__ groups, uint32_t W,
                                                 uint32_t cstride, uint32_t crel,
                                                 uint32_t B, uint32_t pitch, size_t codes_bytes, uint32_t want_cls,
                                                 const uint32_t* __restrict__ status,
                                                 double* __restrict__ lnl) {
  constexpr bool SWZ = NCOLS == 16;
  extern __shared__ __attribute__((aligned(16))) char smem[];
  double* tile = reinterpret_cast<double*>(smem);
  double* accs = tile + (size_t)TROWS * NCOLS;
  __shared__ uint32_t s_maxspan;
  const uint32_t gbeg = want_cls ? status[5] : 0, gend = want_cls ? status[4] : status[5];
  const uint32_t ng = gend - gbeg, ntiles = (B + NB - 1) / NB;
  const int t = threadIdx.x;
  for (uint32_t item = blockIdx.x; item < ng * ntiles; item += gridDim.x) {
  const Group g = groups[gbeg + item % ng];
  const uint32_t b0 = (item / ng) * NB;
  const uint32_t nb = min((uint32_t)NB, B - b0);
  __syncthreads();
  if (g.count == 0) continue;
  const bool active = t < (int)g.count;
  uint32_t qi = 0, begin = 0, span = 0;
  if (active) {
    qi = perm[g.start + t];
    begin = win_begin[qi];
    span = win_span[qi];
    if ((uint64_t)begin + span > W || (crel && span > cstride)) span = 0;
  }
  if (t == 0) s_maxspan = 0;
  __syncthreads();
  atomicMax(&s_maxspan, span);
  if (ACC) for (uint32_t j = 0; j < nb; ++j) accs[j * GQ + t] = 0.0;
  __syncthreads();
  const uint32_t gmin = win_begin[perm[g.start]];
  const uint32_t gspread = win_begin[perm[g.start + g.count - 1]] - gmin;
  const uint32_t rel = begin - gmin;
  const uint32_t nchunks = ACC ? (s_maxspan + CH - 1) / CH : 1;

  for (uint32_t c = 0; c < nchunks; ++c) {
    const uint32_t cbase = c * CH;
    const bool mine = active && cbase < span;
    const uint32_t rem = mine ? span - cbase : 0;
    uint32_t cw[CW];
    if (mine) {
      const size_t addr = (size_t)qi * cstride + (crel ? 0u : begin) + cbase;
      const size_t a0 = addr & ~(size_t)3;
      const uint32_t sh = (uint32_t)(addr & 3) * 8;
      const size_t last = (codes_bytes - 1) & ~(size_t)3;
      const uint32_t* p = reinterpret_cast<const uint32_t*>(codes);
      uint32_t prev = p[min(a0, last) >> 2];
#pragma unroll
      for (int i = 0; i < CW; ++i) {
        const uint32_t nxt = p[min(a0 + 4 * (i + 1), last) >> 2];
        const uint32_t v = __funnelshift_r(prev, nxt, sh);
        uint32_t o = v << 3;
        if (SWZ) {
          const uint32_t r = rel + 4 * i;
          o ^= (((r >> 1) & 15) << 3) | ((((r + 1) >> 1) & 15) << 11) | ((((r + 2) >> 1) & 15) << 19) |
               ((((r + 3) >> 1) & 15) << 27);
        }
        cw[i] = o;
        prev = nxt;
      }
    } else {
#pragma unroll
      for (int i = 0; i < CW; ++i) cw[i] = 0;
    }
    const uint32_t row0 = gmin + cbase;
    const uint32_t need = min((uint32_t)TROWS, gspread + min((uint32_t)CH, s_maxspan - cbase));
    for (uint32_t j = 0; j < nb; ++j) {
      __syncthreads();
      {
        const uint32_t rows = (row0 < W) ? min(need, W - row0) : 0;
        const double2* src = reinterpret_cast<const double2*>(
            lookup + ((size_t)(b0 + j) * W + row0) * NCOLS);
        double2* dst = reinterpret_cast<double2*>(tile);
        const uint32_t n2 = rows * NCOLS / 2;
        constexpr int PF = (TROWS * NCOLS / 2 + GQ - 1) / GQ;
        double2 pf[PF];
#pragma unroll
        for (int u = 0; u < PF; ++u) {
          const uint32_t i = u * GQ + t;
          if (i < n2) pf[u] = src[i];
        }
#pragma unroll
        for (int u = 0; u < PF; ++u) {
          const uint32_t i = u * GQ + t;
          if (i < n2) {
            double2 v = pf[u];
            uint32_t o = i;
            if (SWZ) {
              const uint32_t r = i >> 3, f = (r >> 1) & 15;
              o = (r << 3) | ((i & 7) ^ (f >> 1));
              if (f & 1) { const double x = v.x; v.x = v.y; v.y = x; }
            }
            dst[o] = v;
          }
        }
      }
      __syncthreads();
      if (mine) {
        double sum = ACC ? accs[j * GQ + t] : 0.0;
        uint32_t zj;
        asm volatile("v_mov_b32 %0, 0" : "=v"(zj) : "v"(j));
        const char* base = reinterpret_cast<const char*>(tile);
        const char* mybase = base + (size_t)(rel * (NCOLS * 8) + zj);
        auto at = [&](uint32_t s, uint32_t boff) -> double {
          return *reinterpret_cast<const double*>(mybase + s * (NCOLS * 8) + boff);
        };
        const uint32_t cur = min(rem, (uint32_t)CH);
        const uint32_t nfull = cur >> 2, ntail = cur & 3;
        constexpr int GPB = 2, NBATCH = CW / GPB;
        double rb[2][GPB * 4];
        auto issue = [&](int bt) {
#pragma unroll
          for (int g = 0; g < GPB; ++g) {
            const int i = bt * GPB + g;
            const uint32_t w = cw[i], s0 = 4 * i;
            rb[bt & 1][g * 4 + 0] = at(s0 + 0, w & 0xff);
            rb[bt & 1][g * 4 + 1] = at(s0 + 1, (w >> 8) & 0xff);
            rb[bt & 1][g * 4 + 2] = at(s0 + 2, (w >> 16) & 0xff);
            rb[bt & 1][g * 4 + 3] = at(s0 + 3, w >> 24);
          }
        };
        issue(0);
        __builtin_amdgcn_sched_barrier(0);
#pragma unroll
        for (int bt = 0; bt < NBATCH; ++bt) {
          if (bt + 1 < NBATCH) issue(bt + 1);
          __builtin_amdgcn_sched_barrier(0);
#pragma unroll
          for (int g = 0; g < GPB; ++g) {
            const double* v = &rb[bt & 1][g * 4];
            double s1 = v[0] + v[1];
            const double s2 = v[2] + v[3];
            s1 += s2;
            sum += ((uint32_t)(bt * GPB + g) < nfull) ? s1 : 0.0;
          }
          __builtin_amdgcn_sched_barrier(0);
        }
        if (ntail) {
          uint32_t w = 0;
#pragma unroll
          for (int i = 0; i < CW; ++i) w = ((uint32_t)i == nfull) ? cw[i] : w;
          const uint32_t s0 = 4 * nfull;
// ... 86 lines not shown
                                                    uint16_t* __restrict__ tails,
                                                    uint32_t* __restrict__ keys, uint32_t K,
                                                    uint32_t* __restrict__ status) {
  __shared__ uint16_t s_tab[256];
  s_tab[threadIdx.x] = PAIR_TAB.v[threadIdx.x];
  __syncthreads();
  const uint32_t l16 = threadIdx.x & 15, grp = (threadIdx.x >> 4) & 3u;
  const uint32_t cmax = min(span_bound, crel ? cstride : 0xffffffffu);
  constexpr uint32_t ZERO_W = ZERO_OFF | (ZERO_OFF << 16);
  constexpr int NWI = (PW + 15) / 16;
  const uint32_t lane_base = (2u * l16 * rowl) * 0x10001u + (rowl << 16);
  for (uint32_t q0 = blockIdx.x * 16; q0 < Q; q0 += gridDim.x * 16) {
    const uint32_t q = q0 + (threadIdx.x >> 4);
    const bool live = q < Q;
    const uint32_t begin = live ? win_begin[q] : 0u;
    uint32_t span = live ? win_span[q] : 0u;
    if (live && l16 == 0) validate_window(q, begin, span, W, cmax, status);
    if ((uint64_t)begin + span > W || span > cmax) span = 0;
    const uint8_t* c = codes + (size_t)(live ? q : 0u) * cstride + (crel ? 0u : begin);
    const uint32_t nfull = span >> 2, ntail = span & 3, npairs = 2 * nfull;
    uint32_t* prow = reinterpret_cast<uint32_t*>(packed + (size_t)(live ? q : 0u) * NP16);
    uint32_t racc = 0;
    uint32_t ctail = 0;
    if (l16 < ntail) ctail = c[4 * nfull + l16];
    for (uint32_t pb = 0; pb < NP16; pb += CP) {
      uint32_t cb[NWI][4];
#pragma unroll
      for (int i = 0; i < NWI; ++i) {
        const uint32_t gw = pb / 2 + (uint32_t)i * 16 + l16;
        const bool on = (i * 16 + (int)l16 < PW) && gw < nfull;
#pragma unroll
        for (int k = 0; k < 4; ++k) cb[i][k] = on ? c[4 * gw + k] : 0u;
      }
#pragma unroll
      for (int i = 0; i < NWI; ++i) {
        const uint32_t wl = (uint32_t)i * 16 + l16, gw = pb / 2 + wl;
        if (i * 16 + (int)l16 >= PW) continue;
        uint32_t c0 = cb[i][0], c1 = cb[i][1], c2 = cb[i][2], c3 = cb[i][3];
        if (__builtin_expect(((c0 | c1 | c2 | c3) >> 4) != 0u, 0)) {
          c0 = c0 > 15u ? 0u : c0; c1 = c1 > 15u ? 0u : c1; c2 = c2 > 15u ? 0u : c2; c3 = c3 > 15u ? 0u : c3;
        }
        const uint32_t e0 = s_tab[(c0 << 4) | c1], e1 = s_tab[(c2 << 4) | c3];
        const uint32_t word = ((e1 << 16) | e0) + lane_base + (uint32_t)i * ((32u * rowl) * 0x10001u);
        const bool on = gw < nfull;
        if (on) racc |= word;
        if (live) prow[gw] = on ? (word & 0x7fff7fffu) : ZERO_W;
      }
    }
    bool rare = (racc & 0x80008000u) != 0u;
    if (l16 < 4) {
      uint32_t v = ZERO_OFF;
      if (l16 < ntail) {
        uint32_t sy = dna_sym(ctail);
        rare |= sy > 4;
        sy = min(sy, 5u);
        const uint32_t kt = npairs % CP;
        const uint32_t e = l16 == 1 ? pair_entry(5, sy) : pair_entry(sy, 5);
        v = (kt + (l16 == 2 ? 1u : 0u)) * rowl + e * 8;
      }
      if (live) tails[(size_t)q * 4 + l16] = (uint16_t)v;
    }
    const bool any_rare = ((__ballot(rare) >> (16 * grp)) & 0xffffull) != 0ull;
    if (live && l16 == 0) {
      const uint32_t key = min((any_rare ? 2 * Wp : 0) + (begin & 1u) * Wp + min(begin, Wp - 1), K - 1);
      keys[q] = key;
    }
  }
}

#ifndef PP_XCD
#define PP_XCD 1
#endif
using epa_wave::seg_key;
struct SegTrack {
  double m = -INFINITY;
  __device__ __forceinline__ void add(unsigned long long* __restrict__ segmax, uint32_t segp, uint32_t qi, uint32_t b,
                                      bool last, double v) {
    m = fmax(m, v);
    if ((b & 63u) == 63u || last) {
      atomicMax(&segmax[(size_t)qi * segp + (b >> 6)], seg_key(m));
      m = -INFINITY;
    }
  }
};

#ifndef PP_PRIO
#define PP_PRIO 1
#endif
template <int NBATCH>
__device__ __forceinline__ void gather_prio(int bt) {
#if PP_PRIO == 1
  if (bt == 0) __builtin_amdgcn_s_setprio(3);
  else if (bt == NBATCH / 4) __builtin_amdgcn_s_setprio(2);
  else if (bt == NBATCH / 2) __builtin_amdgcn_s_setprio(1);
  else if (bt == (3 * NBATCH) / 4) __builtin_amdgcn_s_setprio(0);
#elif PP_PRIO == 2
  if (bt == 0) __builtin_amdgcn_s_setprio(3);
  else if (bt == NBATCH / 2) __builtin_amdgcn_s_setprio(0);
#elif PP_PRIO == 3
  if (bt == 0) __builtin_amdgcn_s_setprio(3);
  else if (bt == (2 * NBATCH) / 5) __builtin_amdgcn_s_setprio(2);
  else if (bt == (7 * NBATCH) / 10) __builtin_amdgcn_s_setprio(1);
  else if (bt == (9 * NBATCH) / 10) __builtin_amdgcn_s_setprio(0);
#elif PP_PRIO == 4
  if (bt == 0) __builtin_amdgcn_s_setprio(3);
  else if (bt == NBATCH / 10) __builtin_amdgcn_s_setprio(2);
  else if (bt == (3 * NBATCH) / 10) __builtin_amdgcn_s_setprio(1);
  else if (bt == (6 * NBATCH) / 10) __builtin_amdgcn_s_setprio(0);
#endif
}

struct ItemWalk { uint32_t pos, end, step, lo; };
__device__ __forceinline__ ItemWalk item_walk(uint32_t total) {
  if (PP_XCD && (gridDim.x & 7u) == 0) {
    const uint32_t x = blockIdx.x & 7u, local = blockIdx.x >> 3;
    const uint32_t lo = (uint32_t)((uint64_t)total * x / 8), hi = (uint32_t)((uint64_t)total * (x + 1) / 8);
    return {lo + local, hi, gridDim.x >> 3, lo};
  }
  return {blockIdx.x, total, gridDim.x, 0u};
}

#ifndef PP_XCD_GROUPS
#define PP_XCD_GROUPS 1
#endif
__device__ __forceinline__ void item_group_tile(uint32_t v, uint32_t lo, uint32_t hi, uint32_t ng, uint32_t ntiles,
                                                uint32_t& grp, uint32_t& tile) {
  if (!PP_XCD_GROUPS) { grp = v % ng; tile = v / ng; return; }
  const uint32_t gl = lo / ntiles, tl = lo - gl * ntiles, gh = (hi - 1) / ntiles, th = (hi - 1) - gh * ntiles;
  uint32_t r = v - lo;
  for (uint32_t t = 0; t < ntiles; ++t) {
    const uint32_t first = gl + (t < tl ? 1u : 0u), last1 = gh + 1u - (t > th ? 1u : 0u);
    const uint32_t c = last1 > first ? last1 - first : 0u;
    if (r < c) { grp = first + r; tile = t; return; }
    r -= c;
  }
  grp = 0; tile = ntiles;
}

__device__ __forceinline__ uint32_t choose_tile(uint32_t ng, uint32_t B, uint32_t nwg) {
  uint32_t best = 32, best_cost = 0xffffffffu;
  for (uint32_t n = 16; n <= 96; n += 8) {
    const uint32_t items = ng * ((B + n - 1) / n);
    const uint32_t cost = ((items + nwg - 1) / nwg) * (n + 3);
    if (cost <= best_cost) { best_cost = cost; best = n; }
  }
  return best;
}

#ifdef PP_SCHED_PIN
#define PP_SCHED_BARRIER() __builtin_amdgcn_sched_barrier(0)
#else
#define PP_SCHED_BARRIER()
#endif
template <bool ACC, int SPR, int ROWL, bool SPARSE = false>
__global__ void __launch_bounds__(GQ2, 4) k_preplace_pairs(
    const double* __restrict__ lookup2, const uint16_t* __restrict__ packed,
    const uint16_t* __restrict__ tails, const uint32_t* __restrict__ win_begin,
    const uint32_t* __restrict__ win_span, const uint32_t* __restrict__ perm,
    const Group* __restrict__ groups, uint32_t W, uint32_t B, uint32_t pitch, uint32_t NP16,
    const uint32_t* __restrict__ status, double* __restrict__ lnl,
    unsigned long long* __restrict__ segmax, uint32_t segp) {
  constexpr int TR2 = (CH + SPR) / 2;
  extern __shared__ __attribute__((aligned(16))) char smem[];
  static_assert(ROWL % 16 == 0 && ROWL >= PROWB && ((TR2 - 1) * ROWL + PROWB) < 65536, "16-bit LDS offsets");
  double* accs = reinterpret_cast<double*>(smem + (size_t)TR2 * ROWL);
  __shared__ uint32_t s_maxspan;
  __shared__ uint32_t s_qi[GQ2];
  constexpr uint32_t BSTR = GQ2 + 4;
  const uint32_t ng = status[5];
  const uint32_t NBP = SPARSE ? 64u : ACC ? NB2_ACC : choose_tile(ng, B, gridDim.x);
  const uint32_t ntiles = SPARSE ? 1u : (B + NBP - 1) / NBP;
  const int t = threadIdx.x;
  const ItemWalk iw = SPARSE ? ItemWalk{blockIdx.x, ng, gridDim.x, 0u} : item_walk(ng * ntiles);
  for (uint32_t item = iw.pos; item < iw.end; item += iw.step) {
  uint32_t item_g = item, item_t = 0;
  if (!SPARSE) item_group_tile(item, iw.lo, iw.end, ng, ntiles, item_g, item_t);
  const Group g = groups[item_g];
  const uint32_t b0 = SPARSE ? min(g.min_begin * 64u, B - 1u) : item_t * NBP;
  const uint32_t nb = min(NBP, B - b0);
  __syncthreads();
  if (g.count == 0) continue;
  const bool active = t < (int)g.count;
  uint32_t qi = 0, begin = 0, span = 0;
  if (active) {
    qi = perm[g.start + t];
    begin = win_begin[qi];
    span = win_span[qi];
    if ((uint64_t)begin + span > W) span = 0;
  }
  if (t == 0) s_maxspan = 0;
  const uint32_t my_q = (active && span > 0) ? qi : 0xffffffffu;
  s_qi[t] = my_q;
  __syncthreads();
  {
    uint32_t m = span;
#pragma unroll
    for (int off = 32; off; off >>= 1) m = max(m, (uint32_t)__shfl_xor((int)m, off));
    if ((t & 63) == 0) atomicMax(&s_maxspan, m);
  }
  if (ACC) for (uint32_t j = 0; j < nb; ++j) accs[j * GQ2 + t] = 0.0;
  __syncthreads();
  const uint32_t gmin = win_begin[perm[g.start]];
  const uint32_t gspread = win_begin[perm[g.start + g.count - 1]] - gmin;
  const uint32_t rowoff = ((begin - gmin) >> 1) * ROWL;
  const uint32_t rowoff2 = rowoff | (rowoff << 16);
  const uint32_t nchunks = ACC ? (s_maxspan + CH - 1) / CH : 1;
  uint32_t t0 = 0, t1 = 0, t2 = 0, tailchunk = 0xffffffffu;
  if (active && (span & 3)) {
    const uint16_t* tq = tails + (size_t)qi * 4;
    t0 = tq[0] + rowoff; t1 = tq[1] + rowoff; t2 = tq[2] + rowoff;
    tailchunk = ((span >> 2) * 2) / CP;
  }
  auto at = [&](uint32_t off) -> double { return *reinterpret_cast<const double*>(smem + off); };
  SegTrack seg;

  for (uint32_t c = 0; c < nchunks; ++c) {
    const uint32_t cbase = c * CH;
    const bool mine = active && cbase < span;
    uint32_t cw[PW];
    if (mine) {
      const uint4* p = reinterpret_cast<const uint4*>(packed + (size_t)qi * NP16 + (size_t)c * CP);
#pragma unroll
      for (int i = 0; i < PW / 4; ++i) {
        const uint4 v = p[i];
        cw[4 * i] = v.x + rowoff2;
        cw[4 * i + 1] = v.y + rowoff2;
        cw[4 * i + 2] = v.z + rowoff2;
        cw[4 * i + 3] = v.w + rowoff2;
      }
    } else {
#pragma unroll
      for (int i = 0; i < PW; ++i) cw[i] = 0;
    }
    const uint32_t row0 = gmin + cbase;
    const uint32_t need = min((uint32_t)TR2, (gspread >> 1) + (min((uint32_t)CH, s_maxspan - cbase) + 1) / 2);
    const uint32_t rows = (row0 < W) ? min(need, (W - row0 + 1) / 2) : 0;
    const uint32_t n2 = rows * (PE / 2);
    constexpr int PF = (TR2 * (PE / 2) + GQ2 - 1) / GQ2;
    auto request = [&](uint32_t j, double2 (&pfs)[PF]) {
      const double2* src = reinterpret_cast<const double2*>(
          lookup2 + (((size_t)(b0 + j) * 2 + (row0 & 1u)) * ((W + 1) / 2) + (row0 >> 1)) * PE);
#pragma unroll
      for (int u = 0; u < PF; ++u) {
        const uint32_t i = u * GQ2 + t;
        pfs[u] = make_double2(0.0, 0.0);
        if (i < n2) pfs[u] = src[i];
      }
    };
    auto stage = [&](const double2 (&pfs)[PF], uint32_t boff) {
#pragma unroll
      for (int u = 0; u < PF; ++u) {
        const uint32_t i = u * GQ2 + t;
        if (i < n2) {
          if (ROWL == PROWB) {
            reinterpret_cast<double2*>(smem + boff)[i] = pfs[u];
          } else {
            const uint32_t r = i / (PE / 2), c2 = i - r * (PE / 2);
            *reinterpret_cast<double2*>(smem + boff + r * ROWL + c2 * 16) = pfs[u];
          }
        }
      }
    };
    auto gather = [&](uint32_t j, uint32_t boff) {
      if (mine) {
        double sum = ACC ? accs[j * GQ2 + t] : 0.0;
#pragma unroll
        for (int i = 0; i < PW; ++i) asm volatile("" : "+v"(cw[i]));
#ifndef PP_WPB
#define PP_WPB 2
#endif
        constexpr int WPB = PP_WPB, NBATCH = PW / WPB;
        double rb[2][WPB * 2];
        auto issue = [&](int bt) {
#pragma unroll
          for (int w = 0; w < WPB; ++w) {
            const uint32_t v = cw[bt * WPB + w];
            rb[bt & 1][2 * w] = at((v & 0xffffu) + boff);
            rb[bt & 1][2 * w + 1] = at((v >> 16) + boff);
          }
        };
        issue(0);
        PP_SCHED_BARRIER();
#pragma unroll
        for (int bt = 0; bt < NBATCH; ++bt) {
          gather_prio<NBATCH>(bt);
          if (bt + 1 < NBATCH) issue(bt + 1);
          PP_SCHED_BARRIER();
#pragma unroll
          for (int w = 0; w < WPB; ++w) {
            const double s1 = rb[bt & 1][2 * w] + rb[bt & 1][2 * w + 1];
            sum += s1;
          }
          PP_SCHED_BARRIER();
        }
        if (c == tailchunk) {
          sum += at(t0 + boff);
          sum += at(t1 + boff);
          sum += at(t2 + boff);
        }
        if (ACC) {
          accs[j * GQ2 + t] = sum;
        } else {
          accs[(j & 7u) * BSTR + t] = sum;
          if (segmax) seg.add(segmax, segp, qi, b0 + j, j + 1 == nb, sum);
        }
      }
    };
    auto emit_burst = [&](uint32_t kb) {
      __builtin_amdgcn_wave_barrier();
      const uint32_t lane = (uint32_t)t & 63u, wbase = (uint32_t)t & ~63u, c4 = lane & 3u;
      const uint32_t ncol = min(8u, nb - 8u * kb), bcol = b0 + 8u * kb + 2u * c4;
      const uint32_t r0 = 2u * c4, r1 = 2u * c4 + 1u;
#pragma unroll
      for (uint32_t k = 0; k < 4; ++k) {
        const uint32_t tq = wbase + k * 16 + (lane >> 2);
        const uint32_t q = s_qi[tq];
        if (q != 0xffffffffu && 2u * c4 < ncol) {
          const double a0 = accs[r0 * BSTR + tq];
          double* dst = lnl + (size_t)q * pitch + bcol;
          if (2u * c4 + 1u < ncol) *reinterpret_cast<double2*>(dst) = make_double2(a0, accs[r1 * BSTR + tq]);
          else *dst = a0;
        }
      }
      __builtin_amdgcn_wave_barrier();
    };
    auto flush = [&](uint32_t j) {
      if (ACC) return;
      if ((j & 7u) == 7u) emit_burst(j >> 3);
      else if (j + 1 == nb) emit_burst(j >> 3);
    };
    {
      double2 pf[PF];
      request(0, pf);
      for (uint32_t j = 0; j < nb; ++j) {
        __syncthreads();
        stage(pf, 0);
        __syncthreads();
        if (j + 1 < nb) request(j + 1, pf);
        PP_SCHED_BARRIER();
        gather(j, 0);
        flush(j);
      }
    }
  }
  if (ACC && active) {
    double* out = lnl + (size_t)qi * pitch + b0;
    for (uint32_t j = 0; j < nb; ++j) out[j] = accs[j * GQ2 + t];
  }
  }
}

typedef float f2 __attribute__((ext_vector_type(2)));

__device__ __forceinline__ uint32_t seg_key32(float v) {
  const uint32_t u = __float_as_uint(v);
  return (u >> 31) ? ~u : (u | 0x80000000u);
}
__device__ __forceinline__ float seg_val32(uint32_t k) { return __uint_as_float((k >> 31) ? (k & 0x7fffffffu) : ~k); }

__global__ void __launch_bounds__(256) k_build_lookup2f(const double* __restrict__ lookup2, uint32_t W, uint32_t B,
                                                        float2* __restrict__ lookup2f, uint32_t p0,
                                                        uint32_t* __restrict__ stats) {
  const uint32_t p = p0 + blockIdx.y, Wh = (W + 1) / 2, n = 2 * Wh * PE;
  const uint32_t i = blockIdx.x * 256 + threadIdx.x;
  float amax = 0.f;
  uint32_t bad = 0;
  if (i < n) {
    const uint32_t par = i / (Wh * PE), rem = i - par * Wh * PE, r = rem / PE, e = rem - r * PE;
    const bool valid = 2 * r + par < W, two = 2 * p + 1 < B;
    float x = 0.f, y = 0.f;
    if (valid) {
      x = (float)lookup2[(size_t)(2 * p) * n + i];
      y = two ? (float)lookup2[(size_t)(2 * p + 1) * n + i] : (e == PE - 1 ? 0.f : -INFINITY);
      const bool fx = isfinite(x), fy = !two || isfinite(y);
      bad = (fx ? 0u : 1u) + (fy ? 0u : 1u);
      if (fx) amax = fabsf(x);
      if (two && fy) amax = fmaxf(amax, fabsf(y));
    }
    lookup2f[(size_t)p * n + i] = make_float2(x, y);
  }
#pragma unroll
  for (int off = 32; off; off >>= 1) {
    amax = fmaxf(amax, __shfl_xor(amax, off));
    bad += (uint32_t)__shfl_xor((int)bad, off);
  }
  if ((threadIdx.x & 63) == 0) {
    if (amax > 0.f) atomicMax(&stats[0], __float_as_uint(amax));
    if (bad) atomicAdd(&stats[1], bad);
  }
}

template <int SPR, int ROWL>
__global__ void __launch_bounds__(GQ2, 4) k_preplace_screen(
    const float2* __restrict__ lookup2f, const uint16_t* __restrict__ packed,
    const uint16_t* __restrict__ tails, const uint32_t* __restrict__ win_begin,
    const uint32_t* __restrict__ win_span, const uint32_t* __restrict__ perm,
    const Group* __restrict__ groups, uint32_t W, uint32_t BP, uint32_t NP16,
    const uint32_t* __restrict__ status, uint32_t* __restrict__ seg32, uint32_t segp) {
  constexpr int TR2 = (CH + SPR) / 2;
  extern __shared__ __attribute__((aligned(16))) char smem[];
  static_assert(ROWL % 16 == 0 && ROWL >= PROWB && ((TR2 - 1) * ROWL + PROWB) < 65536, "16-bit LDS offsets");
  __shared__ uint32_t s_maxspan;
  const uint32_t ng = status[5];
  const uint32_t NBP = choose_tile(ng, BP, gridDim.x);
  const uint32_t ntiles = (BP + NBP - 1) / NBP;
  const int t = threadIdx.x;
  const ItemWalk iw = item_walk(ng * ntiles);
  for (uint32_t item = iw.pos; item < iw.end; item += iw.step) {
    uint32_t item_g, item_t;
    item_group_tile(item, iw.lo, iw.end, ng, ntiles, item_g, item_t);
    const Group g = groups[item_g];
    const uint32_t b0 = item_t * NBP;
    const uint32_t nb = min(NBP, BP - b0);
    __syncthreads();
    if (g.count == 0) continue;
    const bool active = t < (int)g.count;
    uint32_t qi = 0, begin = 0, span = 0;
    if (active) {
      qi = perm[g.start + t];
      begin = win_begin[qi];
      span = win_span[qi];
      if ((uint64_t)begin + span > W) span = 0;
    }
    if (t == 0) s_maxspan = 0;
    __syncthreads();
    {
      uint32_t m = span;
#pragma unroll
      for (int off = 32; off; off >>= 1) m = max(m, (uint32_t)__shfl_xor((int)m, off));
      if ((t & 63) == 0) atomicMax(&s_maxspan, m);
    }
    __syncthreads();
    const uint32_t gmin = win_begin[perm[g.start]];
    const uint32_t gspread = win_begin[perm[g.start + g.count - 1]] - gmin;
    const uint32_t rowoff = ((begin - gmin) >> 1) * ROWL;
    const uint32_t rowoff2 = rowoff | (rowoff << 16);
    const bool mine = active && span > 0;
    uint32_t t0 = 0, t1 = 0, t2 = 0;
    if (mine && (span & 3)) {
      const uint16_t* tq = tails + (size_t)qi * 4;
      t0 = tq[0] + rowoff; t1 = tq[1] + rowoff; t2 = tq[2] + rowoff;
    }
    auto at = [&](uint32_t off) -> f2 { return *reinterpret_cast<const f2*>(smem + off); };
    uint32_t cw[PW];
    if (mine) {
      const uint4* p = reinterpret_cast<const uint4*>(packed + (size_t)qi * NP16);
#pragma unroll
      for (int i = 0; i < PW / 4; ++i) {
        const uint4 v = p[i];
        cw[4 * i] = v.x + rowoff2;
        cw[4 * i + 1] = v.y + rowoff2;
        cw[4 * i + 2] = v.z + rowoff2;
        cw[4 * i + 3] = v.w + rowoff2;
      }
    } else {
#pragma unroll
      for (int i = 0; i < PW; ++i) cw[i] = 0;
    }
    const uint32_t row0 = gmin;
    const uint32_t need = min((uint32_t)TR2, (gspread >> 1) + (min((uint32_t)CH, s_maxspan) + 1) / 2);
    const uint32_t rows = (row0 < W) ? min(need, (W - row0 + 1) / 2) : 0;
    const uint32_t n2 = rows * (PE / 2);
    constexpr int PF = (TR2 * (PE / 2) + GQ2 - 1) / GQ2;
    auto request = [&](uint32_t j, float4 (&pfs)[PF]) {
      const float4* src = reinterpret_cast<const float4*>(
          lookup2f + (((size_t)(b0 + j) * 2 + (row0 & 1u)) * ((W + 1) / 2) + (row0 >> 1)) * PE);
#pragma unroll
      for (int u = 0; u < PF; ++u) {
        const uint32_t i = u * GQ2 + t;
        pfs[u] = make_float4(0.f, 0.f, 0.f, 0.f);
        if (i < n2) pfs[u] = src[i];
      }
    };
    auto stage = [&](const float4 (&pfs)[PF]) {
#pragma unroll
      for (int u = 0; u < PF; ++u) {
        const uint32_t i = u * GQ2 + t;
        if (i < n2) {
          if (ROWL == PROWB) {
            reinterpret_cast<float4*>(smem)[i] = pfs[u];
          } else {
            const uint32_t r = i / (PE / 2), c2 = i - r * (PE / 2);
            *reinterpret_cast<float4*>(smem + r * ROWL + c2 * 16) = pfs[u];
          }
        }
      }
    };
    float segm = -INFINITY;
    auto gather = [&](uint32_t j) {
      if (!mine) return;
      f2 sum = {0.f, 0.f};
#pragma unroll
      for (int i = 0; i < PW; ++i) asm volatile("" : "+v"(cw[i]));
      constexpr int WPB = PP_WPB, NBATCH = PW / WPB;
      f2 rb[2][WPB * 2];
      auto issue = [&](int bt) {
#pragma unroll
        for (int w = 0; w < WPB; ++w) {
          const uint32_t v = cw[bt * WPB + w];
          rb[bt & 1][2 * w] = at(v & 0xffffu);
          rb[bt & 1][2 * w + 1] = at(v >> 16);
        }
      };
      issue(0);
#pragma unroll
      for (int bt = 0; bt < NBATCH; ++bt) {
        gather_prio<NBATCH>(bt);
        if (bt + 1 < NBATCH) issue(bt + 1);
#pragma unroll
        for (int w = 0; w < WPB; ++w) {
          const f2 s1 = rb[bt & 1][2 * w] + rb[bt & 1][2 * w + 1];
          sum += s1;
        }
      }
      if (span & 3) {
        sum += at(t0);
        sum += at(t1);
        sum += at(t2);
      }
      segm = fmaxf(segm, fmaxf(sum.x, sum.y));
      const uint32_t bp = b0 + j;
      if ((bp & 31u) == 31u || j + 1 == nb) {
        atomicMax(&seg32[(size_t)qi * segp + (bp >> 5)], seg_key32(segm));
        segm = -INFINITY;
      }
    };
    float4 pf[PF];
    request(0, pf);
    for (uint32_t j = 0; j < nb; ++j) {
      __syncthreads();
      stage(pf);
      __syncthreads();
      if (j + 1 < nb) request(j + 1, pf);
      gather(j);
    }
  }
}

__global__ void __launch_bounds__(256) k_screen_band(const uint32_t* __restrict__ seg32, uint32_t Q, uint32_t nseg,
                                                     uint32_t seg32p, double band, double delta,
                                                     const uint32_t* __restrict__ qkeys, uint32_t KB,
                                                     unsigned long long* __restrict__ segmax, uint32_t segp,
                                                     uint32_t* __restrict__ ccnt, uint32_t* __restrict__ rank,
                                                     unsigned long long* __restrict__ mask,
                                                     unsigned long long* __restrict__ n_incl) {
  const uint32_t q = blockIdx.x * 256 + threadIdx.x;
  uint32_t cnt = 0;
  if (q < Q) {
    const uint32_t* row = seg32 + (size_t)q * seg32p;
    const uint32_t qk = qkeys[q];
    float r = -INFINITY;
    bool all = qk < KB;
    for (uint32_t s = 0; s < nseg; ++s) {
      const uint32_t k = row[s];
      if (k) r = fmaxf(r, seg_val32(k)); else all = false;
    }
    unsigned long long m = 0;
    if (all) {
      const double lo = (double)r - band;
      for (uint32_t s = 0; s < nseg; ++s) {
        const double v = (double)seg_val32(row[s]);
        if (v >= lo) {
          m |= 1ull << s;
          if (ccnt) rank[(size_t)q * seg32p + s] = atomicAdd(&ccnt[s * KB + qk], 1u);
        } else if (segmax) {
          segmax[(size_t)q * segp + s] = seg_key(v + delta);
        }
      }
    }
    mask[q] = m;
    cnt = (uint32_t)__popcll(m);
  }
#pragma unroll
  for (int off = 32; off; off >>= 1) cnt += (uint32_t)__shfl_xor((int)cnt, off);
  if ((threadIdx.x & 63) == 0 && cnt) atomicAdd(n_incl, (unsigned long long)cnt);
}

__global__ void __launch_bounds__(256) k_scatter_cells(const unsigned long long* __restrict__ mask,
                                                       const uint32_t* __restrict__ qkeys, const uint32_t* __restrict__ rank,
                                                       const uint32_t* __restrict__ offs, uint32_t Q, uint32_t seg32p,
                                                       uint32_t KB, uint32_t ncell, uint32_t* __restrict__ sorted_keys,
                                                       uint32_t* __restrict__ perm) {
  const uint32_t q = blockIdx.x * 256 + threadIdx.x;
  if (q >= Q) return;
  unsigned long long m = mask[q];
  const uint32_t qk = qkeys[q];
  while (m) {
    const uint32_t s = (uint32_t)__ffsll((long long)m) - 1u;
    m &= m - 1;
    const uint32_t key = s * KB + qk, pos = offs[key] + rank[(size_t)q * seg32p + s];
    if (pos < ncell) {
      sorted_keys[pos] = key;
      perm[pos] = q;
    }
  }
}

constexpr int CHS = 128;
constexpr int PWS = CHS / 2;
constexpr int TROWS_S = CHS + SPREAD;

template <int NCOLS>
__global__ void __launch_bounds__(256) k_pack_sites(const uint8_t* __restrict__ codes,
                                                    const uint32_t* __restrict__ win_begin,
                                                    const uint32_t* __restrict__ win_span, uint32_t Q,
                                                    uint32_t W, uint32_t cstride, uint32_t crel,
                                                    uint32_t span_bound, uint32_t NP16,
                                                    uint16_t* __restrict__ packed,
                                                    uint16_t* __restrict__ tails,
                                                    uint32_t* __restrict__ keys, uint32_t K,
                                                    uint32_t* __restrict__ status) {
  const uint32_t q = blockIdx.x * 4 + (threadIdx.x >> 6);
  const uint32_t lane = threadIdx.x & 63;
  if (q >= Q) return;
  const uint32_t begin = win_begin[q];
  uint32_t span = win_span[q];
  const uint32_t cmax = min(span_bound, crel ? cstride : 0xffffffffu);
  if (lane == 0) validate_window(q, begin, span, W, cmax, status);
  if ((uint64_t)begin + span > W || span > cmax) span = 0;
  const uint8_t* c = codes + (size_t)q * cstride + (crel ? 0u : begin);
  const uint32_t nsum = span & ~3u;
  for (uint32_t p = lane; p < NP16; p += 64) {
    uint32_t v = 0;
    if (p < nsum) v = (p % CHS) * (NCOLS * 8) + min((uint32_t)c[p], (uint32_t)NCOLS - 1) * 8;
    packed[(size_t)q * NP16 + p] = (uint16_t)v;
  }
  if (lane < 4) {
    uint32_t v = 0;
    if (lane < (span & 3))
      v = ((nsum + lane) % CHS) * (NCOLS * 8) + min((uint32_t)c[nsum + lane], (uint32_t)NCOLS - 1) * 8;
    tails[(size_t)q * 4 + lane] = (uint16_t)v;
  }
  if (lane == 0) {
    const uint32_t key = min(begin, K - 1);
    keys[q] = key;
  }
}

template <int NCOLS, bool ACC>
__global__ void __launch_bounds__(GQ2, 4) k_preplace_sites(
    const double* __restrict__ lookup, const uint16_t* __restrict__ packed,
    const uint16_t* __restrict__ tails, const uint32_t* __restrict__ win_begin,
    const uint32_t* __restrict__ win_span, const uint32_t* __restrict__ perm,
    const Group* __restrict__ groups, uint32_t W, uint32_t B, uint32_t pitch, uint32_t NP16,
    const uint32_t* __restrict__ status, double* __restrict__ lnl,
    unsigned long long* __restrict__ segmax, uint32_t segp) {
  constexpr uint32_t ROWB = NCOLS * 8;
  extern __shared__ __attribute__((aligned(16))) char smem[];
  double* accs = reinterpret_cast<double*>(smem + (size_t)TROWS_S * ROWB);
  __shared__ uint32_t s_maxspan;
  __shared__ uint32_t s_qi[GQ2];
  constexpr uint32_t BSTR = GQ2 + 4;
  const uint32_t ng = status[5];
  const uint32_t NBP = ACC ? NB2_ACC_S : choose_tile(ng, B, gridDim.x);
  const uint32_t ntiles = (B + NBP - 1) / NBP;
  const int t = threadIdx.x;
  auto at = [&](uint32_t off) -> double { return *reinterpret_cast<const double*>(smem + off); };
  const ItemWalk iw = item_walk(ng * ntiles);
  for (uint32_t item = iw.pos; item < iw.end; item += iw.step) {
    const Group g = groups[item % ng];
    const uint32_t b0 = (item / ng) * NBP;
    const uint32_t nb = min(NBP, B - b0);
    __syncthreads();
    SegTrack seg;
    if (g.count == 0) continue;
    const bool active = t < (int)g.count;
    uint32_t qi = 0, begin = 0, span = 0;
    if (active) {
      qi = perm[g.start + t];
      begin = win_begin[qi];
      span = win_span[qi];
      if ((uint64_t)begin + span > W) span = 0;
    }
    if (t == 0) s_maxspan = 0;
    s_qi[t] = (active && span > 0) ? qi : 0xffffffffu;
    __syncthreads();
    {
      uint32_t m = span;
#pragma unroll
      for (int off = 32; off; off >>= 1) m = max(m, (uint32_t)__shfl_xor((int)m, off));
      if ((t & 63) == 0) atomicMax(&s_maxspan, m);
    }
    if (ACC) for (uint32_t j = 0; j < nb; ++j) accs[j * GQ2 + t] = 0.0;
    __syncthreads();
    const uint32_t gmin = win_begin[perm[g.start]];
    const uint32_t gspread = win_begin[perm[g.start + g.count - 1]] - gmin;
    const uint32_t rowoff = (begin - gmin) * ROWB;
    const uint32_t rowoff2 = rowoff | (rowoff << 16);
    const uint32_t nchunks = ACC ? (s_maxspan + CHS - 1) / CHS : 1;
    const uint32_t nsum = span & ~3u, ntail = span & 3;
    uint32_t t0 = 0, t1 = 0, t2 = 0, tailchunk = 0xffffffffu;
    if (active && ntail) {
      const uint16_t* tq = tails + (size_t)qi * 4;
      t0 = tq[0] + rowoff; t1 = tq[1] + rowoff; t2 = tq[2] + rowoff;
      tailchunk = nsum / CHS;
    }
    for (uint32_t c = 0; c < nchunks; ++c) {
      const uint32_t cbase = c * CHS;
      const bool mine = active && cbase < span;
      const uint32_t gfull = mine ? (min(nsum, cbase + CHS) > cbase ? (min(nsum, cbase + CHS) - cbase) >> 2 : 0) : 0;
      uint32_t cw[PWS];
      if (mine) {
        const uint4* p = reinterpret_cast<const uint4*>(packed + (size_t)qi * NP16 + (size_t)c * CHS);
#pragma unroll
        for (int i = 0; i < PWS / 4; ++i) {
          const uint4 v = p[i];
          cw[4 * i] = v.x + rowoff2;
          cw[4 * i + 1] = v.y + rowoff2;
          cw[4 * i + 2] = v.z + rowoff2;
          cw[4 * i + 3] = v.w + rowoff2;
        }
      } else {
#pragma unroll
        for (int i = 0; i < PWS; ++i) cw[i] = 0;
      }
      const uint32_t row0 = gmin + cbase;
      const uint32_t need = min((uint32_t)TROWS_S, gspread + min((uint32_t)CHS, s_maxspan - cbase));
      const uint32_t rows = (row0 < W) ? min(need, W - row0) : 0;
      const uint32_t n2 = rows * (NCOLS / 2);
      constexpr int PF = (TROWS_S * (NCOLS / 2) + GQ2 - 1) / GQ2;
      double2 pf[PF];
      auto request = [&](uint32_t j) {
        const double2* src = reinterpret_cast<const double2*>(lookup + ((size_t)(b0 + j) * W + row0) * NCOLS);
#pragma unroll
        for (int u = 0; u < PF; ++u) {
          const uint32_t i = u * GQ2 + t;
          pf[u] = make_double2(0.0, 0.0);
          if (i < n2) pf[u] = src[i];
        }
      };
      request(0);
      for (uint32_t j = 0; j < nb; ++j) {
        __syncthreads();
        {
          double2* dst = reinterpret_cast<double2*>(smem);
#pragma unroll
          for (int u = 0; u < PF; ++u) {
            const uint32_t i = u * GQ2 + t;
            if (i < n2) dst[i] = pf[u];
          }
        }
        __syncthreads();
        if (j + 1 < nb) request(j + 1);
        __builtin_amdgcn_sched_barrier(0);
        if (mine) {
          double sum = ACC ? accs[j * GQ2 + t] : 0.0;
#pragma unroll
// ... 11 lines not shown
          issue(0);
          __builtin_amdgcn_sched_barrier(0);
#pragma unroll
          for (int bt = 0; bt < NBATCH; ++bt) {
            gather_prio<NBATCH>(bt);
            if (bt + 1 < NBATCH) issue(bt + 1);
            __builtin_amdgcn_sched_barrier(0);
#pragma unroll
            for (int gq = 0; gq < 2; ++gq) {
              const double* v = &rb[bt & 1][gq * 4];
              double s1 = v[0] + v[1];
              const double s2 = v[2] + v[3];
              s1 += s2;
              sum += ((uint32_t)(bt * 2 + gq) < gfull) ? s1 : 0.0;
            }
            __builtin_amdgcn_sched_barrier(0);
          }
          if (c == tailchunk) {
            sum += at(t0);
            if (ntail > 1) sum += at(t1);
            if (ntail > 2) sum += at(t2);
          }
          if (ACC) {
            accs[j * GQ2 + t] = sum;
          } else {
            accs[(j & 7u) * BSTR + t] = sum;
            if (segmax) seg.add(segmax, segp, qi, b0 + j, j + 1 == nb, sum);
          }
        }
        if (!ACC && ((j & 7u) == 7u || j + 1 == nb)) {
          __builtin_amdgcn_wave_barrier();
          const uint32_t lane = (uint32_t)t & 63u, wbase = (uint32_t)t & ~63u, col = lane & 7u;
          const uint32_t ncol = (j & 7u) + 1u, bcol = b0 + (j & ~7u) + col;
#pragma unroll
          for (uint32_t k = 0; k < 8; ++k) {
            const uint32_t tq = wbase + k * 8 + (lane >> 3);
            const uint32_t q = s_qi[tq];
            if (q != 0xffffffffu && col < ncol) lnl[(size_t)q * pitch + bcol] = accs[col * BSTR + tq];
          }
          __builtin_amdgcn_wave_barrier();
        }
      }
    }
    if (ACC && active) {
      double* out = lnl + (size_t)qi * pitch + b0;
      for (uint32_t j = 0; j < nb; ++j) out[j] = accs[j * GQ2 + t];
    }
  }
}

}

void launch_scan_counts(epa_ctx* ctx, uint32_t* cnt, uint32_t K, const uint32_t* tip_row, uint32_t* tip_total) {
  hipLaunchKernelGGL(k_scan_counts, dim3(1), dim3(1024), 0, ctx->stream, cnt, K, tip_row, tip_total);
}

int launch_build_lookup2(epa_ctx* ctx) {
  if (!ctx->lookup2)
    EPA_HIP(ctx, hipMalloc(&ctx->lookup2, sizeof(double) * (size_t)ctx->B * 2 * ((ctx->W + 1) / 2) * PE));
  for (uint32_t b0 = 0; b0 < ctx->B; b0 += EPA_GRID_Y)
    hipLaunchKernelGGL(k_build_lookup2, dim3((ctx->W * PE + 255) / 256, std::min<uint32_t>(EPA_GRID_Y, ctx->B - b0)), dim3(256), 0,
                       ctx->stream, ctx->lookup, ctx->W, ctx->lookup2, b0);
  EPA_HIP(ctx, hipGetLastError());
  return EPA_OK;
}

int launch_build_lookup2_block(epa_ctx* ctx, uint32_t nb, const double* blk_lookup, double* blk_lookup2) {
  for (uint32_t r0 = 0; r0 < nb; r0 += EPA_GRID_Y)
    hipLaunchKernelGGL(k_build_lookup2, dim3((ctx->W * PE + 255) / 256, std::min<uint32_t>(EPA_GRID_Y, nb - r0)), dim3(256), 0,
                       ctx->stream, blk_lookup, ctx->W, blk_lookup2, r0);
  EPA_HIP(ctx, hipGetLastError());
  return EPA_OK;
}

int launch_build_lookup2f(epa_ctx* ctx) {
  if (ctx->lookup2f || ctx->lookup2f_refused) return EPA_OK;
  if (!ctx->lookup2) return epa_fail(ctx, EPA_ERR_INVALID_ARG, "the fp32 pair table needs the resident site-pair table");
  const uint32_t BP = (ctx->B + 1) / 2, n = 2 * ((ctx->W + 1) / 2) * PE;
  const size_t bytes = sizeof(float2) * (size_t)BP * n;
  char* buf = nullptr;
  constexpr size_t SCREEN_RESERVE = (size_t)4 << 30;
  size_t free_b = 0, total_b = 0;
  const bool room = hipMemGetInfo(&free_b, &total_b) == hipSuccess && free_b >= bytes + 16 + SCREEN_RESERVE;
  if (!room || hipMalloc(&buf, bytes + 16) != hipSuccess) {
    (void)hipGetLastError();
    ctx->lookup2f_refused = true;
    return EPA_OK;
  }
  uint32_t* stats = reinterpret_cast<uint32_t*>(buf + bytes);
  EPA_HIP(ctx, hipMemsetAsync(stats, 0, 16, ctx->stream));
  for (uint32_t p0 = 0; p0 < BP; p0 += EPA_GRID_Y)
    hipLaunchKernelGGL(k_build_lookup2f, dim3((n + 255) / 256, std::min<uint32_t>(EPA_GRID_Y, BP - p0)), dim3(256), 0, ctx->stream,
                       ctx->lookup2, ctx->W, ctx->B, reinterpret_cast<float2*>(buf), p0, stats);
  uint32_t h[4] = {0, 0, 0, 0};
  hipError_t e = hipGetLastError();
  if (e == hipSuccess) e = hipMemcpyAsync(h, stats, 16, hipMemcpyDeviceToHost, ctx->stream);
  if (e == hipSuccess) e = hipStreamSynchronize(ctx->stream);
  if (e != hipSuccess) { (void)hipFree(buf); EPA_HIP(ctx, e); }
  float m;
  memcpy(&m, &h[0], 4);
  ctx->screen_M = (double)m;
  ctx->screen_nonfinite = h[1];
  ctx->lookup2f = reinterpret_cast<float2*>(buf);
  return EPA_OK;
}

double epa_screen_delta(const epa_ctx* ctx, uint32_t span_bound) {
  if (!ctx->lookup2f || ctx->screen_nonfinite) return -1.0;
  const double u = 0x1p-24, n = 2.0 * (span_bound >> 2) + 3.0;
  const double delta = 2.0 * (n + 1.0) * u * n * ctx->screen_M * (double)std::max(ctx->opt.preplace_screen_scale, 1);
  return delta <= 1.0 ? delta : -1.0;
}

int launch_preplace(epa_ctx* ctx, const uint8_t* d_codes, const uint32_t* d_begin, const uint32_t* d_span, uint32_t Q,
                    const PreTable& t, uint32_t max_span, const uint32_t** d_status, PreScreenProbe* probe) {
  double* const d_lnl = t.lnl;
  const uint32_t pitch = t.pitch, segp = t.segp;
  unsigned long long* const segmax = t.segmax;
  const bool blocked = ctx->lookup_blocks;
  const bool pairs = ctx->s == 4 && (ctx->lookup2 || blocked) && !ctx->opt.preplace_generic;
  const bool sites = ctx->s == 20 && ctx->ncols == 24 && !ctx->opt.preplace_generic;
  const uint32_t crel = ctx->code_stride ? 1u : 0u, cstride = crel ? ctx->code_stride : ctx->W;
  const uint32_t n_buckets = (ctx->W + SPREAD - 1) / SPREAD;
  const uint32_t Wp = n_buckets * SPREAD;
  const uint32_t n_blocks = pairs ? 4 : 1, class_blocks = pairs ? 2 : 1;
  const uint32_t gq0 = (pairs || sites) ? GQ2 : GQ, gq1 = GQ;
  const uint32_t max_runs = (Q + GQ - 1) / GQ + n_blocks;
  const uint32_t max_groups = max_runs + n_blocks * n_buckets;
  const uint32_t span_bound = (max_span == 0 || max_span > ctx->W) ? ctx->W : max_span;
  const uint32_t NP16 = pairs ? ((span_bound + 1) / 2 + CP - 1) / CP * CP
                        : sites ? (span_bound + CHS - 1) / CHS * CHS : 0;
  const uint32_t K = pairs ? n_blocks * Wp : sites ? ctx->W + 1 : 0;
  size_t temp_bytes = 0;
  (void)rocprim::radix_sort_pairs<epa_radix_cfg>(nullptr, temp_bytes, (uint32_t*)nullptr, (uint32_t*)nullptr,
                                  (uint32_t*)nullptr, (uint32_t*)nullptr, Q, 0, 32, ctx->stream);
  uint32_t *status, *key_cnt, *iota, *sorted_keys, *perm, *keys;
  const uint32_t nseg = (ctx->B + 63) / 64, seg32p = (nseg + 7u) & ~7u;
  const uint32_t KB = 2 * Wp, n_blocks_c = 2 * nseg;
  const uint64_t max_cells = (uint64_t)Q * nseg;
  const uint32_t Kc = nseg * KB + 1;
  const uint32_t max_runs_c = (uint32_t)std::min<uint64_t>((max_cells + GQ2 - 1) / GQ2 + n_blocks_c, 0xffffffu);
  const uint32_t max_groups_c = max_runs_c + n_blocks_c * n_buckets;
  const size_t smem_c = sizeof(uint32_t) * (2 * (n_blocks_c + 1) + 4 * (size_t)max_runs_c + 2);
  double delta = -1.0;
  constexpr uint64_t SCREEN_MIN_CELLS = 80000000ull;
  const bool big = ctx->opt.preplace_screen >= 2 || probe || (uint64_t)Q * ctx->B >= SCREEN_MIN_CELLS;
  if (pairs && !blocked && nseg <= 64 && max_span != 0 && max_span <= (uint32_t)CH && ctx->opt.preplace_screen && big &&
      (probe || (segmax && t.band_t > 0.0)) && max_cells < 0x80000000ull && smem_c <= 65536) {
    const int brc = launch_build_lookup2f(ctx);
    if (brc) return brc;
    delta = epa_screen_delta(ctx, span_bound);
  }
  const bool screen = delta >= 0.0;
  uint32_t *seg32, *cstatus, *ccnt, *crank, *csorted, *cperm;
  unsigned long long *seg_mask, *n_incl;
  Group* cgroups;
  Group* groups;
  uint16_t *packed, *tails;
  void* temp;
  auto layout = [&](Carver c) {
    status = c.take<uint32_t>(64);
    key_cnt = c.take<uint32_t>(K);
    seg32 = c.take<uint32_t>(screen ? (size_t)Q * seg32p : 0);
    n_incl = c.take<unsigned long long>(screen ? 1 : 0);
    cstatus = c.take<uint32_t>(screen ? 64 : 0);
    ccnt = c.take<uint32_t>(screen ? Kc : 0);
    iota = c.take<uint32_t>(Q);
    sorted_keys = c.take<uint32_t>(Q);
    perm = c.take<uint32_t>(Q);
    keys = c.take<uint32_t>(Q);
    groups = c.take<Group>(max_groups);
    packed = c.take<uint16_t>((size_t)Q * NP16);
    tails = c.take<uint16_t>((pairs || sites) ? 4 * (size_t)Q : 0);
    seg_mask = c.take<unsigned long long>(screen ? Q : 0);
    crank = c.take<uint32_t>(screen ? (size_t)Q * seg32p : 0);
    csorted = c.take<uint32_t>(screen ? max_cells : 0);
    cperm = c.take<uint32_t>(screen ? max_cells : 0);
    cgroups = c.take<Group>(screen ? max_groups_c : 0);
    temp = c.tail(temp_bytes);
    return c.off;
  };
  char* base = (char*)epa_scratch(ctx, SLOT_PREPLACE, layout(Carver{}));
  if (!base) return epa_fail(ctx, EPA_ERR_HIP, "hipMalloc(preplace scratch)");
  layout(Carver{base});
  *d_status = status;
  {
    const int zr = epa_zero_async(ctx, status, (char*)iota - (char*)status, segmax, sizeof(unsigned long long) * (size_t)Q * segp);
    if (zr) return zr;
  }
  const bool acc = max_span == 0 || max_span > (uint32_t)CH;
  const bool wide = pairs && !acc && (uint64_t)Q * SPREAD < (uint64_t)1400 * ctx->W;
  const uint32_t rowl = (wide || acc) ? ROWL_PACKED : ROWL_NARROW;
  if (pairs) {
    constexpr uint32_t pack_grid = 64;
    hipLaunchKernelGGL(k_pack_pairs, dim3(std::min<uint32_t>((Q + 15) / 16, (uint32_t)ctx->n_cu * pack_grid)), dim3(256), 0, ctx->stream, d_codes, d_begin,
                       d_span, Q, ctx->W, cstride, crel, span_bound, Wp, NP16, rowl, packed, tails, keys, K, status);
  } else if (sites) {
    hipLaunchKernelGGL(k_pack_sites<24>, dim3((Q + 3) / 4), dim3(256), 0, ctx->stream, d_codes, d_begin,
                       d_span, Q, ctx->W, cstride, crel, span_bound, NP16, packed, tails, keys, K, status);
  }
  if (pairs || sites) {
    hipLaunchKernelGGL(k_count_keys, dim3((Q + 255) / 256), dim3(256), 0, ctx->stream, keys, Q, key_cnt, iota);
    launch_scan_counts(ctx, key_cnt, K);
    hipLaunchKernelGGL(k_scatter_sorted, dim3((Q + 255) / 256), dim3(256), 0, ctx->stream, keys, iota, key_cnt, Q,
                       sorted_keys, perm);
  } else {
    hipLaunchKernelGGL(k_iota, dim3((Q + 255) / 256), dim3(256), 0, ctx->stream, iota, Q);
    hipLaunchKernelGGL(k_validate, dim3((Q + 255) / 256), dim3(256), 0, ctx->stream, d_begin, d_span, Q,
                       ctx->W, std::min(span_bound, crel ? cstride : 0xffffffffu), status);
    int wbits = 1;
    while (wbits < 32 && (1ull << wbits) <= (uint64_t)ctx->W) ++wbits;
    EPA_HIP(ctx, rocprim::radix_sort_pairs<epa_radix_cfg>(temp, temp_bytes, d_begin, sorted_keys, iota, perm, Q, 0, wbits,
                                           ctx->stream));
  }
  constexpr int SPREAD_WIDE = 288;
  hipLaunchKernelGGL(k_make_groups, dim3(1), dim3(256),
                     sizeof(uint32_t) * (2 * (n_blocks + 1) + 4 * (size_t)max_runs + 2), ctx->stream,
                     sorted_keys, Q, pairs ? Wp : 0xffffffffu, n_blocks, class_blocks, gq0, gq1,
                     (uint32_t)(wide ? SPREAD_WIDE : SPREAD), max_runs, groups, max_groups, status);
  const size_t codes_bytes = (size_t)Q * cstride;
  const uint32_t want_cls = pairs ? 1u : 0u;
  const size_t lds = sizeof(double) * ((size_t)TROWS * ctx->ncols + (acc ? (size_t)NB * GQ : 0));
  const size_t lds2 = wide ? (size_t)((CH + SPREAD_WIDE) / 2) * ROWL_PACKED + sizeof(double) * NB2_BURST * (GQ2 + 4)
                           : (size_t)TROWS2 * rowl + sizeof(double) * (acc ? NB2_ACC * GQ2 : NB2_BURST * (GQ2 + 4));
  const bool acc_s = max_span == 0 || max_span > (uint32_t)CHS;
  const size_t lds_s = (size_t)TROWS_S * 24 * 8 + sizeof(double) * (acc_s ? NB2_ACC_S * GQ2 : NB2_BURST * (GQ2 + 4));
  using FastKernel = decltype(&k_preplace_sites<24, false>);
  using GenericKernel = decltype(&k_preplace<16, false>);
  FastKernel k_fast = nullptr;
  if (pairs) k_fast = wide ? k_preplace_pairs<false, SPREAD_WIDE, ROWL_PACKED> : acc ? k_preplace_pairs<true, SPREAD, ROWL_PACKED> : k_preplace_pairs<false, SPREAD, ROWL_NARROW>;
  else if (sites) k_fast = acc_s ? k_preplace_sites<24, true> : k_preplace_sites<24, false>;
  const bool fast_acc = pairs ? acc : acc_s;
  const size_t lds_fast = pairs ? lds2 : lds_s;
  const GenericKernel k_generic = sites ? nullptr : ctx->ncols == 16 ? (acc ? k_preplace<16, true> : k_preplace<16, false>) : (acc ? k_preplace<24, true> : k_preplace<24, false>);
  if (k_fast) EPA_HIP(ctx, hipFuncSetAttribute((const void*)k_fast, hipFuncAttributeMaxDynamicSharedMemorySize, (int)lds_fast));
  if (k_generic) EPA_HIP(ctx, hipFuncSetAttribute((const void*)k_generic, hipFuncAttributeMaxDynamicSharedMemorySize, (int)lds));
  auto kernels = [&](const double* lk, const double* lk2, uint32_t nB, double* lnl, unsigned long long* sm, bool fast = true) {
    if (k_fast && fast) {
      const uint32_t tile = fast_acc ? (pairs ? NB2_ACC : NB2_ACC_S) : 16;
      const dim3 grid_f((uint32_t)std::min<uint64_t>((uint64_t)max_groups * ((nB + tile - 1) / tile), (uint64_t)ctx->n_cu));
      hipLaunchKernelGGL(k_fast, grid_f, dim3(GQ2), (uint32_t)lds_fast, ctx->stream, pairs ? lk2 : lk, (const uint16_t*)packed,
                         (const uint16_t*)tails, d_begin, d_span, perm, groups, ctx->W, nB, pitch, NP16, status, lnl,
                         fast_acc ? nullptr : sm, segp);
    }
    if (!k_generic) return;
    const uint32_t ntiles = (nB + NB - 1) / NB;
    const dim3 grid(pairs ? (uint32_t)std::min<uint64_t>((uint64_t)max_groups * ntiles, (uint64_t)ctx->n_cu * (acc ? 2 : 4))
                          : max_groups * ntiles);
    hipLaunchKernelGGL(k_generic, grid, dim3(GQ), (uint32_t)lds, ctx->stream, lk, d_codes, d_begin, d_span, perm, groups, ctx->W,
                       cstride, crel, nB, pitch, codes_bytes, want_cls, status, lnl);
  };
  if (probe) probe->ran = screen;
  if (probe && !screen) return EPA_OK;
  if (screen) {
    using ScreenKernel = decltype(&k_preplace_screen<SPREAD, ROWL_NARROW>);
    const ScreenKernel k_screen = wide ? k_preplace_screen<SPREAD_WIDE, ROWL_PACKED> : k_preplace_screen<SPREAD, ROWL_NARROW>;
    const FastKernel k_exact = wide ? k_preplace_pairs<false, SPREAD_WIDE, ROWL_PACKED, true> : k_preplace_pairs<false, SPREAD, ROWL_NARROW, true>;
    const size_t lds_scr = wide ? (size_t)((CH + SPREAD_WIDE) / 2) * ROWL_PACKED : (size_t)TROWS2 * ROWL_NARROW;
    EPA_HIP(ctx, hipFuncSetAttribute((const void*)k_screen, hipFuncAttributeMaxDynamicSharedMemorySize, (int)lds_scr));
    EPA_HIP(ctx, hipFuncSetAttribute((const void*)k_exact, hipFuncAttributeMaxDynamicSharedMemorySize, (int)lds_fast));
    const uint32_t BP = (ctx->B + 1) / 2;
    struct Events {
      hipEvent_t e[3] = {nullptr, nullptr, nullptr};
      ~Events() { for (hipEvent_t x : e) if (x) (void)hipEventDestroy(x); }
    } evs;
    hipEvent_t* const ev = evs.e;
    if (probe) for (hipEvent_t& e : evs.e) EPA_HIP(ctx, hipEventCreate(&e));
    if (probe) EPA_HIP(ctx, hipEventRecord(ev[0], ctx->stream));
    else epa_timer_start(ctx, epa_t(ctx, epa_ctx::T_PREPLACE));
    const dim3 grid_s((uint32_t)std::min<uint64_t>((uint64_t)max_groups * ((BP + 15) / 16), (uint64_t)ctx->n_cu));
    hipLaunchKernelGGL(k_screen, grid_s, dim3(GQ2), (uint32_t)lds_scr, ctx->stream, (const float2*)ctx->lookup2f, (const uint16_t*)packed,
                       (const uint16_t*)tails, d_begin, d_span, perm, groups, ctx->W, BP, NP16, status, seg32, seg32p);
    if (probe) EPA_HIP(ctx, hipEventRecord(ev[1], ctx->stream));
    const double band = (probe ? probe->band_t : t.band_t) + 2.0 * delta;
    hipLaunchKernelGGL(k_screen_band, dim3((Q + 255) / 256), dim3(256), 0, ctx->stream, (const uint32_t*)seg32, Q, nseg, seg32p, band,
                       delta, (const uint32_t*)keys, KB, probe ? nullptr : segmax, segp, probe ? nullptr : ccnt, crank, seg_mask, n_incl);
    if (probe) {
      EPA_HIP(ctx, hipEventRecord(ev[2], ctx->stream));
      EPA_HIP(ctx, hipGetLastError());
      EPA_HIP(ctx, hipEventSynchronize(ev[2]));
      (void)hipEventElapsedTime(&probe->ms_screen, ev[0], ev[1]);
      (void)hipEventElapsedTime(&probe->ms_band, ev[1], ev[2]);
      probe->delta = delta;
      probe->seg32 = seg32;
      probe->mask = seg_mask;
      probe->n_incl = n_incl;
      return EPA_OK;
    }
    ++ctx->screen_runs;
    launch_scan_counts(ctx, ccnt, Kc);
    hipLaunchKernelGGL(k_scatter_cells, dim3((Q + 255) / 256), dim3(256), 0, ctx->stream, (const unsigned long long*)seg_mask,
                       (const uint32_t*)keys, (const uint32_t*)crank, (const uint32_t*)ccnt, Q, seg32p, KB, (uint32_t)max_cells, csorted, cperm);
    hipLaunchKernelGGL(k_make_groups, dim3(1), dim3(256), smem_c, ctx->stream, (const uint32_t*)csorted, (uint32_t)max_cells, Wp, n_blocks_c,
                       n_blocks_c, (uint32_t)GQ2, (uint32_t)GQ2, (uint32_t)(wide ? SPREAD_WIDE : SPREAD), max_runs_c, cgroups, max_groups_c,
                       cstatus, (const uint32_t*)(ccnt + (Kc - 1)), KB);
    hipLaunchKernelGGL(k_exact, dim3(std::min<uint32_t>(max_groups_c, (uint32_t)ctx->n_cu)), dim3(GQ2), (uint32_t)lds_fast, ctx->stream,
                       (const double*)ctx->lookup2, (const uint16_t*)packed, (const uint16_t*)tails, d_begin, d_span, (const uint32_t*)cperm,
                       (const Group*)cgroups, ctx->W, ctx->B, pitch, NP16, (const uint32_t*)cstatus, d_lnl, segmax, segp);
    kernels(ctx->lookup, ctx->lookup2, ctx->B, d_lnl, segmax, false);
    epa_timer_stop(ctx, epa_t(ctx, epa_ctx::T_PREPLACE));
    EPA_HIP(ctx, hipGetLastError());
    return EPA_OK;
  }
  if (!blocked) {
    epa_timer_start(ctx, epa_t(ctx, epa_ctx::T_PREPLACE));
    kernels(ctx->lookup, ctx->lookup2, ctx->B, d_lnl, segmax);
    epa_timer_stop(ctx, epa_t(ctx, epa_ctx::T_PREPLACE));
    EPA_HIP(ctx, hipGetLastError());
    return EPA_OK;
  }
  const uint32_t blk = epa_block_branches(ctx);
  size_t off2 = 0;
  (void)epa_block_bytes(ctx->s, ctx->W, blk, &off2);
  char* buf = (char*)epa_block_buffer(ctx);
  if (!buf) return epa_fail(ctx, EPA_ERR_NO_MEMORY, "hipMalloc(lookup block buffer): " + std::to_string(epa_block_bytes(ctx->s, ctx->W, blk, nullptr)) +
                                                    " bytes needed for blocks of " + std::to_string(blk) + " branches (option lookup_block)");
  double* blk_lookup = reinterpret_cast<double*>(buf);
  double* blk_lookup2 = ctx->s == 4 ? reinterpret_cast<double*>(buf + off2) : nullptr;
  const uint32_t nblocks = (ctx->B + blk - 1) / blk;
  std::vector<hipEvent_t>& ev = ctx->blk_ev[ctx->bank];
  const bool timed = ctx->opt.timers != 0;
  ctx->blk_ev_n[ctx->bank] = 0;
  (void)epa_t(ctx, epa_ctx::T_PREPLACE);
  auto mark = [&](uint32_t i) -> int {
    if (!timed) return EPA_OK;
    while (ev.size() <= i) { hipEvent_t e = nullptr; EPA_HIP(ctx, hipEventCreate(&e)); ev.push_back(e); }
    EPA_HIP(ctx, hipEventRecord(ev[i], ctx->stream));
    return EPA_OK;
  };
  for (uint32_t k = 0; k < nblocks; ++k) {
    const uint32_t b0 = k * blk, nB = std::min(blk, ctx->B - b0);
    int rc = mark(2 * k);
    if (!rc) rc = launch_build_lookup_block(ctx, b0, nB, blk_lookup);
    if (!rc && pairs) rc = launch_build_lookup2_block(ctx, nB, blk_lookup, blk_lookup2);
    if (!rc) rc = mark(2 * k + 1);
    if (rc) return rc;
    kernels(blk_lookup, blk_lookup2, nB, d_lnl + b0, segmax ? segmax + (b0 >> 6) : nullptr);
  }
  { const int rc = mark(2 * nblocks); if (rc) return rc; }
  if (timed) ctx->blk_ev_n[ctx->bank] = 2 * nblocks + 1;
  EPA_HIP(ctx, hipGetLastError());
  return EPA_OK;
}

int preplace_window_error(epa_ctx* ctx, const uint32_t* st) {
  if (st[0])
    return epa_fail(ctx, EPA_ERR_QUERY_ALL_GAP, "Sequence " + std::to_string(st[0] & 0x7fffffffu) +
                                                    " does not appear to have any non-gap sites!");
  if (st[1])
    return epa_fail(ctx, EPA_ERR_QUERY_WIDTH, "Query sequence length not same as reference alignment!");
  return EPA_OK;
}

int preplace_check_status(epa_ctx* ctx, const uint32_t* d_status) {
  uint32_t st[4];
  EPA_HIP(ctx, hipMemcpy(st, d_status, sizeof(st), hipMemcpyDeviceToHost));
  return preplace_window_error(ctx, st);
}
```

include/epa_dev.h:

```cpp
#ifndef EPA_DEV_H
#define EPA_DEV_H

#include <stddef.h>
#include <stdint.h>

#ifdef __cplusplus
extern "C" {
#endif

typedef struct epa_ctx epa_ctx;

typedef enum {
  EPA_OK = 0,
  EPA_ERR_INVALID_ARG = -1,
  EPA_ERR_HIP = -2,
  EPA_ERR_NO_DEVICE = -3,
  EPA_ERR_QUERY_WIDTH = -4,
  EPA_ERR_QUERY_ALL_GAP = -5,
  EPA_ERR_INVALID_CHAR = -6,
  EPA_ERR_NEG_INF = -7,
  EPA_ERR_UNSUPPORTED = -8,
  EPA_ERR_PAIR_OVERFLOW = -9,
  EPA_ERR_NO_MEMORY = -10
} epa_status;

#define EPA_FLAG_SLIDING_BLO 0x1u
#define EPA_FLAG_RAXML_BLO 0x4u
#define EPA_FLAG_NEWTON_SLOW_BISECT 0x8u
#define EPA_FLAG_NEWTON_STRICT_DF 0x10u
#define EPA_FLAG_KEEP_EIGENVALUES 0x20u
#define EPA_FLAG_RATE_SCALERS 0x2u

#define EPA_FLAG_LOOKUP_BLOCKS 0x40u
#define EPA_FLAG_LOOKUP_AUTO 0x80u

typedef struct {
  uint32_t states;
  uint32_t rate_cats;
  uint32_t sites;
  uint32_t branches;

  const double* eigenvals;
  const double* eigenvecs_u;
  const double* eigenvecs_uinv;
  const double* freqs;
  const double* rates;
  const double* rate_weights;
  double prop_invar;

  const double* const* prox_clv;
  const uint32_t* const* prox_scaler;
  const double* const* dist_clv;
  const uint8_t* const* dist_tipchars;
  const uint32_t* const* dist_scaler;
  const double* branch_length;

  const uint32_t* tipmap;
  uint32_t tipmap_size;

  double blo_min_branch;
  double blo_max_branch;
  double blo_default_branch;
  double blo_epsilon;
  double pendant_default;
  uint32_t blo_max_rounds;
  uint32_t blo_max_newton;
  uint32_t flags;
  uint32_t aa_x_as_n;
  const int8_t* invariant_state;
} epa_ref_desc;

#define EPA_TIP 0x80000000u
typedef struct {
  epa_ref_desc ref;
  uint32_t tips;
  uint32_t inner_records;
  const uint8_t* tipchars;
  const uint32_t* rec_child_a;
  const uint32_t* rec_child_b;
  const double* rec_length_a;
  const double* rec_length_b;
  const uint32_t* branch_prox;
  const uint32_t* branch_dist;
} epa_tree_desc;

typedef struct {
  uint32_t branch_id;
  uint32_t seq_id;
} epa_pair;

typedef struct {
  double lnl;
  double pendant_length;
  double distal_length;
} epa_result;

typedef struct {
  uint64_t pairs;
  uint64_t rounds;
  uint64_t newton_evals;
  uint64_t reverts;
} epa_thorough_stats;

int epa_dev_device_count(void);

int epa_dev_create(const epa_ref_desc* desc, int device, epa_ctx** out);
void epa_dev_destroy(epa_ctx* ctx);
const char* epa_dev_last_error(const epa_ctx* ctx);

int epa_dev_create_from_tree(const epa_tree_desc* tree, int device, epa_ctx** out);

int epa_dev_tree_logl(epa_ctx* ctx, uint32_t branch, double* lnl);

int epa_dev_set_stream(epa_ctx* ctx, void* hip_stream);

int epa_dev_set_option(epa_ctx* ctx, const char* key, int value);

int epa_dev_build_lookup(epa_ctx* ctx);

typedef struct {
  uint64_t reft;
  uint64_t scsum;
  uint64_t lookup;
  uint64_t lookup2;
  uint64_t refi;
  uint64_t misc;
  uint64_t create_temp;
  uint64_t reference;
  uint64_t bank;
  uint64_t steady;
  uint64_t peak;
} epa_footprint;
int epa_dev_footprint(uint32_t states, uint32_t rate_cats, uint64_t sites, uint64_t branches, int flags, int from_tree,
                      uint32_t block_branches, int banks, epa_footprint* out);

#define EPA_LOOKUP_RESIDENT 0
#define EPA_LOOKUP_BLOCKS 1
int epa_dev_lookup_plan(uint64_t usable_bytes, uint32_t states, uint32_t rate_cats, uint64_t sites, uint64_t branches,
                        int flags, int from_tree, int banks, int* mode, uint32_t* block_branches);
void epa_dev_set_mem_cap(uint64_t bytes);
int epa_dev_lookup_mode(const epa_ctx* ctx, int* mode, uint32_t* block_branches);


int epa_encode_queries(uint32_t states, uint32_t sites, uint32_t Q, const char* const* seqs,
                       int premasking, int aa_x_as_n, uint8_t* codes, uint32_t* win_begin,
                       uint32_t* win_span, uint32_t* bad_query);

void epa_encode_set_threads(unsigned n);
int epa_encode_queries_compact(uint32_t states, uint32_t sites, uint32_t Q, const char* const* seqs,
                               int premasking, int aa_x_as_n, uint32_t stride, uint8_t* codes,
                               uint32_t* win_begin, uint32_t* win_span, uint32_t* bad_query);
int epa_dev_set_query_layout(epa_ctx* ctx, uint32_t code_stride);

int epa_pack_codes_4bit(const uint8_t* codes, uint32_t Q, uint32_t stride, uint8_t* packed);
int epa_unpack_codes_4bit(const uint8_t* packed, uint32_t Q, uint32_t stride, uint8_t* codes);
int epa_dev_set_query_packing(epa_ctx* ctx, int bits);

int epa_dev_preplace(epa_ctx* ctx, const uint8_t* q_codes, const uint32_t* win_begin,
                     const uint32_t* win_span, uint32_t Q, double* lnl);

int epa_dev_preplace_bounded(epa_ctx* ctx, const uint8_t* q_codes, const uint32_t* win_begin,
                             const uint32_t* win_span, uint32_t Q, uint32_t max_span, double* lnl, uint64_t* seg_keys);

int epa_dev_preplace_screen_probe(epa_ctx* ctx, const uint8_t* q_codes, const uint32_t* win_begin,
                                  const uint32_t* win_span, uint32_t Q, uint32_t max_span, double threshold,
                                  float* seg32, uint64_t* seg_mask, double* info);
uint64_t epa_dev_preplace_screen_runs(const epa_ctx* ctx);

int epa_dev_thorough(epa_ctx* ctx, const epa_pair* pairs, uint64_t n_pairs,
                     const uint8_t* q_codes, const uint32_t* win_begin, const uint32_t* win_span,
                     uint32_t Q, epa_result* out, epa_thorough_stats* stats);

int epa_dev_score_at(epa_ctx* ctx, const epa_pair* pairs, const double* pendant, const double* distal,
                     const double* proximal , uint64_t n,
                     const uint8_t* q_codes, const uint32_t* win_begin, const uint32_t* win_span, uint32_t Q,
                     double* lnl);

int epa_dev_site_lnl(epa_ctx* ctx, const epa_pair* pairs, const double* pendant, const double* distal,
                     const double* proximal , uint64_t n,
                     const uint8_t* q_codes, const uint32_t* win_begin, const uint32_t* win_span, uint32_t Q,
                     uint32_t pitch, double* site_lnl );

int epa_dev_preplace_profile(epa_ctx* ctx, const double* prof, uint32_t stride, const uint32_t* win_begin,
                             const uint32_t* win_span, uint32_t Q, double* lnl);
int epa_dev_thorough_profile(epa_ctx* ctx, const epa_pair* pairs, uint64_t n_pairs, const double* prof, uint32_t stride,
                             const uint32_t* win_begin, const uint32_t* win_span, uint32_t Q, epa_result* out,
                             epa_thorough_stats* stats);
int epa_dev_score_at_profile(epa_ctx* ctx, const epa_pair* pairs, const double* pendant, const double* distal,
                             const double* proximal , uint64_t n, const double* prof, uint32_t stride,
                             const uint32_t* win_begin, const uint32_t* win_span, uint32_t Q, double* lnl);
int epa_dev_site_lnl_profile(epa_ctx* ctx, const epa_pair* pairs, const double* pendant, const double* distal,
                             const double* proximal , uint64_t n, const double* prof, uint32_t stride,
                             const uint32_t* win_begin, const uint32_t* win_span, uint32_t Q, uint32_t pitch,
                             double* site_lnl );
int epa_dev_place_chunk_profile(epa_ctx* ctx, const double* prof, uint32_t stride, const uint32_t* win_begin,
                                const uint32_t* win_span, uint32_t Q, double threshold, epa_pair* pairs,
                                epa_result* results, uint64_t max_pairs, uint64_t* n_pairs, epa_thorough_stats* stats);
int epa_profile_from_phred(uint32_t states, uint32_t Q, uint32_t stride, const uint8_t* codes, const uint8_t* phred,
                           const uint32_t* win_span, double* prof);

int epa_dev_marginal_like(epa_ctx* ctx, const epa_pair* pairs, uint64_t n,
                          const double* x_frac, const double* x_logw, uint32_t Kx,
                          const double* p_len,  const double* p_logw, uint32_t Kp,
                          const uint8_t* q_codes, const uint32_t* win_begin, const uint32_t* win_span, uint32_t Q,
                          double* marginal , double* grid_lnl );

int epa_quadrature_legendre01(uint32_t K, double* nodes, double* log_weights);
int epa_quadrature_laguerre(uint32_t K, double* nodes, double* log_weights);

int epa_dev_rell_support(epa_ctx* ctx, const epa_pair* pairs, const double* pendant, const double* distal,
                         const double* proximal , uint64_t n,
                         const uint8_t* q_codes, const uint32_t* win_begin, const uint32_t* win_span, uint32_t Q,
                         const uint64_t* stream_id ,
                         uint32_t replicates, uint64_t seed, double* support );

int epa_dev_rell_tests(epa_ctx* ctx, const epa_pair* pairs, const double* pendant, const double* distal,
                       const double* proximal , uint64_t n,
                       const uint8_t* q_codes, const uint32_t* win_begin, const uint32_t* win_span, uint32_t Q,
                       const uint64_t* stream_id ,
                       uint32_t replicates, uint64_t seed,
                       double* support , double* elw , double* p_sh );

int epa_dev_rell_au(epa_ctx* ctx, const epa_pair* pairs, const double* pendant, const double* distal,
                    const double* proximal , uint64_t n,
                    const uint8_t* q_codes, const uint32_t* win_begin, const uint32_t* win_span, uint32_t Q,
                    const uint64_t* stream_id ,
                    uint32_t replicates, uint64_t seed,
                    const uint32_t* scale_pm , uint32_t n_scales,
                    double* p_au , uint32_t* counts ,
                    double* fit );

int epa_dev_rell_kh(epa_ctx* ctx, const epa_pair* pairs, const double* pendant, const double* distal,
                    const double* proximal , uint64_t n,
                    const uint8_t* q_codes, const uint32_t* win_begin, const uint32_t* win_span, uint32_t Q,
                    const uint64_t* stream_id ,
                    uint32_t replicates, uint64_t seed,
                    double* p_kh , double* p_wkh , double* p_wsh );

int epa_dev_select_candidates(epa_ctx* ctx, const double* lnl, uint32_t Q, double threshold,
                              epa_pair* pairs, uint64_t max_pairs, uint64_t* n_pairs);

#define EPA_HEUR_DYNAMIC 0
#define EPA_HEUR_FIXED 1
#define EPA_HEUR_BASEBALL 2
int epa_dev_set_heuristic(epa_ctx* ctx, int mode, double param);

int epa_dev_place_chunk(epa_ctx* ctx, const uint8_t* q_codes, const uint32_t* win_begin,
                        const uint32_t* win_span, uint32_t Q, uint32_t max_span, double threshold,
                        epa_pair* pairs, epa_result* results, uint64_t max_pairs,
                        uint64_t* n_pairs, epa_thorough_stats* stats);

int epa_dev_dedup_queries(epa_ctx* ctx, const uint8_t* q_codes, const uint32_t* win_begin, const uint32_t* win_span,
                          uint32_t Q, uint32_t* rep , uint32_t* first , uint32_t* n_unique);
int epa_dev_place_chunk_dedup(epa_ctx* ctx, const uint8_t* q_codes, const uint32_t* win_begin, const uint32_t* win_span,
                              uint32_t Q, uint32_t max_span, double threshold,
                              epa_pair* pairs, epa_result* results, uint64_t max_pairs, uint64_t* n_pairs,
                              epa_thorough_stats* stats,
                              uint32_t* rep , uint32_t* first , uint32_t* n_unique);

#define EPA_CHUNK_NO_D2H 0x1u
#define EPA_CHUNK_HOST_ORDERED 0x2u
int epa_dev_chunk_stage(epa_ctx* ctx, int slot, const uint8_t* q_codes, const uint32_t* win_begin,
                        const uint32_t* win_span, uint32_t Q);
int epa_dev_chunk_launch(epa_ctx* ctx, int slot, uint32_t max_span, double threshold,
                         epa_pair* d_pairs, epa_result* d_results, uint64_t max_pairs,
                         uint32_t flags);
int epa_dev_chunk_launch_begin(epa_ctx* ctx, int slot, uint32_t max_span, double threshold,
                               epa_pair* d_pairs, epa_result* d_results, uint64_t max_pairs,
                               uint32_t flags);
int epa_dev_chunk_launch_end(epa_ctx* ctx, int slot);
int epa_dev_chunk_finish(epa_ctx* ctx, int slot, const epa_pair** pairs, const epa_result** results,
                         uint64_t* n_pairs, epa_thorough_stats* stats);

int epa_dev_chunk_launch_many_begin(epa_ctx* ctx, const int* slots, int n_slots, uint32_t max_span,
                                    double threshold, uint64_t max_pairs, uint32_t flags);
int epa_dev_chunk_launch_many(epa_ctx* ctx, const int* slots, int n_slots, uint32_t max_span, double threshold,
                              uint64_t max_pairs, uint32_t flags);

int epa_dev_place_all(epa_ctx* ctx, const uint8_t* q_codes, const uint32_t* win_begin,
                      const uint32_t* win_span, uint32_t Q, uint32_t max_span, double min_lwr,
                      int acc_threshold, uint32_t filter_min, uint32_t filter_max, epa_pair* pairs,
                      epa_result* results, double* lwr, uint32_t* counts,
                      epa_thorough_stats* stats);

#define EPA_COMM_ID_BYTES 128
typedef struct epa_comm epa_comm;
typedef struct {
  uint32_t branch_id, seq_id;
  double lnl, pendant_length, distal_length;
} epa_row;
int epa_comm_set_library(const char* path);
const char* epa_comm_library_path(void);
int epa_comm_set_timeout(epa_comm* comm_or_null, double seconds);
int epa_comm_get_unique_id(void* id128);
int epa_comm_create(epa_ctx* ctx, const void* id128, int rank, int world, uint32_t rows_cap, int depth,
                    epa_comm** out);
void epa_comm_destroy(epa_comm* comm);
int epa_comm_probe(epa_ctx* ctx, epa_comm* comm, double timeout_s, uint64_t* device_ids);
int epa_comm_set_self_send(epa_comm* comm, int on);
int epa_dev_gather_results(epa_ctx* ctx, epa_comm* comm, const epa_pair* d_pairs, const epa_result* d_results,
                           uint64_t n, uint32_t seq_offset, uint64_t* ticket);
int epa_dev_gather_slot(epa_ctx* ctx, epa_comm* comm, int slot, uint32_t seq_offset, uint64_t* ticket);
#define EPA_ROW_LWR 0xfffffffeu
int epa_dev_place_all_rows(epa_ctx* ctx, const uint8_t* q_codes, const uint32_t* win_begin, const uint32_t* win_span,
                           uint32_t Q, uint32_t max_span, double min_lwr, int acc_threshold, uint32_t filter_min,
                           uint32_t filter_max, uint32_t seq_offset, const epa_row** d_rows, uint64_t* n_rows,
                           epa_thorough_stats* stats);
int epa_dev_gather_rows(epa_ctx* ctx, epa_comm* comm, const epa_row* d_rows, uint64_t n, uint64_t* ticket);
int epa_comm_collect(epa_comm* comm, uint64_t ticket, const epa_row** rows, uint32_t* counts, uint64_t* pending);
const epa_row* epa_comm_device_rows(const epa_comm* comm, uint64_t ticket, int rank);
int epa_comm_flush(epa_ctx* ctx, epa_comm* comm, uint64_t* first_extra_ticket, uint32_t* n_extra);
uint64_t epa_comm_carried_rows(const epa_comm* comm);
void epa_comm_abort(epa_comm* comm);

int epa_dev_mem_info(epa_ctx* ctx, uint64_t* free_bytes, uint64_t* total_bytes);

int epa_dev_xcd_shares(const epa_ctx* ctx, double shares[8]);

double epa_dev_last_sclk_mhz(const epa_ctx* ctx);
// ... 8 lines not shown
```

Before: 17.87 million placements/s.

## Bundle up to three adjacent window-slice groups per exact-pass preplace block

The screened exact preplace pass now packs several adjacent window-start slices of the same branch segment into one block as a bundle, each member on its own waves, instead of one group per block. The block stages a wider LDS row range (up to three spreads) so the members share the lookup gather and block launch slots. This is meant to cut underfilled blocks and per-group overhead when screened cells are sparse. The trade-off is more LDS per block, which may lower occupancy. A table-dump API is also added for checking the screen results.

```diff
diff --git a/epa_ng_amd/api.py b/epa_ng_amd/api.py
--- a/epa_ng_amd/api.py
+++ b/epa_ng_amd/api.py
@@ -98,6 +98,8 @@
                                                C.c_void_p, C.c_void_p]
         L.epa_dev_preplace_screen_probe.argtypes = [C.c_void_p, C.c_void_p, C.c_void_p, C.c_void_p, C.c_uint32, C.c_uint32,
                                                     C.c_double, C.c_void_p, C.c_void_p, C.c_void_p]
+        L.epa_dev_preplace_screen_table.argtypes = [C.c_void_p, C.c_void_p, C.c_void_p, C.c_void_p, C.c_uint32, C.c_uint32,
+                                                    C.c_double, C.c_void_p, C.c_void_p, C.c_void_p, C.c_void_p]
         L.epa_dev_preplace_screen_runs.argtypes = [C.c_void_p]
         L.epa_dev_preplace_screen_runs.restype = C.c_uint64
         L.epa_dev_thorough.argtypes = [C.c_void_p, C.c_void_p, C.c_uint64, C.c_void_p, C.c_void_p,
@@ -472,6 +474,19 @@
                 "nonfinite": int(info[4]), "band_t": float(info[5]), "ms_screen": float(info[6]),
                 "ms_band": float(info[7]), "seg32": seg32, "mask": mask}
 
+    def preplace_screen_table(self, codes, win_begin, win_span, max_span, threshold=0.99999):
+        Q = len(win_begin)
+        lnl = np.empty((Q, self.B), np.float64)
+        keys = np.zeros((Q, ((self.B + 63) // 64 + 7) // 8 * 8), np.uint64)
+        mask = np.zeros(Q, np.uint64)
+        info = np.zeros(4, np.float64)
+        self._layout(codes)
+        self._check(self.L.epa_dev_preplace_screen_table(self.h, _ptr(codes), _ptr(win_begin), _ptr(win_span), Q,
+                                                         int(max_span), float(threshold), _ptr(lnl), _ptr(keys),
+                                                         _ptr(mask), _ptr(info)))
+        return {"ran": bool(info[0]), "delta": float(info[1]), "included": int(info[2]), "bundles": int(info[3]),
+                "lnl": lnl, "keys": keys, "mask": mask}
+
     def thorough(self, pairs, codes, win_begin, win_span, Q=None, n_pairs=None, out=None):
         Q = len(win_begin) if Q is None else Q
         n = len(pairs) if n_pairs is None else n_pairs
diff --git a/epa_ng_amd/build.py b/epa_ng_amd/build.py
--- a/epa_ng_amd/build.py
+++ b/epa_ng_amd/build.py
@@ -11,7 +11,8 @@
 EXTRA_FLAGS = {"thorough_dna.hip": ["-mllvm", "-amdgpu-sched-strategy=iterative-ilp"],
                "thorough_dna_tipd.hip": ["-mllvm", "-amdgpu-sched-strategy=iterative-ilp"],
                "thorough_aa_mfma.hip": ["-mllvm", "-amdgpu-sched-strategy=iterative-ilp"]}
-EXTRA_DEPS = {"thorough_dna_tipd.hip": ["thorough_dna.hip"], "thorough_dna_tipd2h.hip": ["thorough_dna.hip"]}
+EXTRA_DEPS = {"thorough_dna_tipd.hip": ["thorough_dna.hip"], "thorough_dna_tipd2h.hip": ["thorough_dna.hip"],
+              "preplace.hip": ["preplace_bundle.hpp"]}
 DEV_FLAGS = ["--offload-arch=gfx950", "-O3", "-std=c++17", "-fPIC", "-I", os.path.join(ROOT, "include"),
              "-I", CSRC, "-Wall", "-Wno-unused-function", "-Wno-unused-result"]
 
diff --git a/epa_ng_amd/csrc/epa_dev.hip b/epa_ng_amd/csrc/epa_dev.hip
--- a/epa_ng_amd/csrc/epa_dev.hip
+++ b/epa_ng_amd/csrc/epa_dev.hip
@@ -588,7 +588,8 @@
       {"queued_thorough", &EpaOptions::queued_thorough},   {"xcd_balance", &EpaOptions::xcd_balance},
       {"aa_valu", &EpaOptions::aa_valu},                   {"timers", &EpaOptions::timers},
       {"newton_lds", &EpaOptions::newton_lds},             {"tip_distal", &EpaOptions::tip_distal},
-      {"preplace_screen", &EpaOptions::preplace_screen},   {"preplace_screen_scale", &EpaOptions::preplace_screen_scale}};
+      {"preplace_screen", &EpaOptions::preplace_screen},   {"preplace_screen_scale", &EpaOptions::preplace_screen_scale},
+      {"preplace_bundle", &EpaOptions::preplace_bundle}};
   for (const Entry& e : table)
     if (strcmp(key, e.name) == 0) {
       ctx->opt.*e.field = value;
@@ -1577,6 +1578,54 @@
         seg32[(size_t)q * nseg + s] = v;
       }
   }
+  return EPA_OK;
+}
+
+extern "C" int epa_dev_preplace_screen_table(epa_ctx* ctx, const uint8_t* q_codes, const uint32_t* win_begin,
+                                             const uint32_t* win_span, uint32_t Q, uint32_t max_span, double threshold,
+                                             double* lnl, uint64_t* seg_keys, uint64_t* seg_mask, double* info) {
+  if (!ctx || !q_codes || !win_begin || !win_span || !lnl || !seg_keys || !seg_mask || !info)
+    return epa_fail(ctx, EPA_ERR_INVALID_ARG, "null argument");
+  for (int i = 0; i < 4; ++i) info[i] = 0.0;
+  if (Q == 0) return EPA_OK;
+  EPA_HIP(ctx, hipSetDevice(ctx->device));
+  int rc = epa_dev_build_lookup(ctx);
+  if (rc) return rc;
+  if (max_span > ctx->W) max_span = ctx->W;
+  if (max_span && !epa_is_device_ptr(win_span))
+    for (uint32_t q = 0; q < Q; ++q)
+      if (win_span[q] > max_span) return epa_fail(ctx, EPA_ERR_INVALID_ARG, "preplace: a window is longer than max_span");
+  const uint32_t nseg = (ctx->B + 63) / 64, segp = (nseg + 7u) & ~7u;
+  if (nseg > 64) return epa_fail(ctx, EPA_ERR_INVALID_ARG, "preplace: segment maxima exist up to 4096 branches");
+  const size_t tab_bytes = sizeof(double) * (size_t)Q * ctx->B, seg_bytes = sizeof(unsigned long long) * (size_t)Q * segp;
+  unsigned long long* d_seg = (unsigned long long*)epa_scratch(ctx, SLOT_SEGMAX, seg_bytes);
+  double* d_lnl = (double*)epa_scratch(ctx, SLOT_TABLE, tab_bytes);
+  const uint8_t* d_codes = epa_codes_to_device(ctx, q_codes, Q);
+  const uint32_t* d_begin = (const uint32_t*)epa_to_device(ctx, SLOT_BEGIN, win_begin, sizeof(uint32_t) * Q);
+  const uint32_t* d_span = (const uint32_t*)epa_to_device(ctx, SLOT_SPAN, win_span, sizeof(uint32_t) * Q);
+  if (!d_seg || !d_lnl || !d_codes || !d_begin || !d_span) return epa_fail(ctx, EPA_ERR_HIP, "query upload or scratch failed");
+  EPA_HIP(ctx, hipMemsetAsync(d_lnl, 0xff, tab_bytes, ctx->stream));
+  PreScreenProbe probe;
+  probe.full = true;
+  PreTable t{d_lnl, ctx->B, d_seg, segp};
+  t.band_t = epa_select_band_t(threshold, ctx->B);
+  const uint32_t* d_status = nullptr;
+  rc = launch_preplace(ctx, d_codes, d_begin, d_span, Q, t, max_span, &d_status, &probe);
+  if (rc) return rc;
+  EPA_HIP(ctx, hipMemcpyAsync(lnl, d_lnl, tab_bytes, hipMemcpyDeviceToHost, ctx->stream));
+  EPA_HIP(ctx, hipMemcpyAsync(seg_keys, d_seg, seg_bytes, hipMemcpyDeviceToHost, ctx->stream));
+  EPA_HIP(ctx, hipStreamSynchronize(ctx->stream));
+  if ((rc = preplace_check_status(ctx, d_status))) return rc;
+  info[0] = probe.ran ? 1.0 : 0.0;
+  if (!probe.ran) return EPA_OK;
+  unsigned long long n_incl = 0;
+  uint32_t n_bundles = 0;
+  EPA_HIP(ctx, hipMemcpy(&n_incl, probe.n_incl, sizeof(n_incl), hipMemcpyDeviceToHost));
+  EPA_HIP(ctx, hipMemcpy(&n_bundles, probe.n_bundles, sizeof(n_bundles), hipMemcpyDeviceToHost));
+  EPA_HIP(ctx, hipMemcpy(seg_mask, probe.mask, sizeof(uint64_t) * Q, hipMemcpyDeviceToHost));
+  info[1] = probe.delta;
+  info[2] = (double)n_incl;
+  info[3] = (double)n_bundles;
   return EPA_OK;
 }
 
diff --git a/epa_ng_amd/csrc/epa_dev_internal.hpp b/epa_ng_amd/csrc/epa_dev_internal.hpp
--- a/epa_ng_amd/csrc/epa_dev_internal.hpp
+++ b/epa_ng_amd/csrc/epa_dev_internal.hpp
@@ -241,6 +241,7 @@
   int dedup_key_bits = 64;
   int preplace_screen = 1;
   int preplace_screen_scale = 1;
+  int preplace_bundle = 3;
   int dedup_sort_bits = 32;
 };
 
@@ -439,11 +440,13 @@
 double epa_screen_delta(const epa_ctx* ctx, uint32_t span_bound);
 struct PreScreenProbe {
   double band_t = 0.0;
+  bool full = false;
   bool ran = false;
   double delta = 0.0;
   const uint32_t* seg32 = nullptr;
   const unsigned long long* mask = nullptr;
   const unsigned long long* n_incl = nullptr;
+  const uint32_t* n_bundles = nullptr;
   float ms_screen = -1.f, ms_band = -1.f;
 };
 uint32_t epa_block_branches(const epa_ctx* ctx);
diff --git a/epa_ng_amd/csrc/preplace.hip b/epa_ng_amd/csrc/preplace.hip
--- a/epa_ng_amd/csrc/preplace.hip
+++ b/epa_ng_amd/csrc/preplace.hip
@@ -1,10 +1,12 @@
 #include "epa_dev_internal.hpp"
+#include "preplace_bundle.hpp"
 #include "wave_util.hpp"
 
 #include <cstdlib>
 #include <cstring>
 
 #include <algorithm>
+#include <type_traits>
 
 namespace {
 
@@ -106,10 +108,8 @@
                                                      uint32_t Wp, uint32_t n_blocks,
                                                      uint32_t class_blocks, uint32_t gq0, uint32_t gq1,
                                                      uint32_t spr0, uint32_t max_runs, Group* __restrict__ groups,
-                                                     uint32_t max_groups, uint32_t* __restrict__ status,
-                                                     const uint32_t* __restrict__ n_dev = nullptr, uint32_t seg_div = 0) {
+                                                     uint32_t max_groups, uint32_t* __restrict__ status) {
   extern __shared__ uint32_t sh[];
-  if (n_dev) Q = min(Q, *n_dev);
   uint32_t* lo = sh;
   uint32_t* runbase = lo + n_blocks + 1;
   uint32_t* run_start = runbase + n_blocks + 1;
@@ -169,17 +169,40 @@
     const uint32_t cls = b >= class_blocks ? 1u : 0u;
     const uint32_t start = run_start[r], end = run_end[r], g0 = run_off[r], n = run_off[r + 1] - g0;
     if (n == 1) {
-      if (g0 < max_groups) groups[g0] = Group{start, end - start, seg_div ? sorted_keys[start] / seg_div : 0u, cls};
+      if (g0 < max_groups) groups[g0] = Group{start, end - start, 0, cls};
     } else {
       const uint32_t spr = cls ? (uint32_t)SPREAD : spr0;
       const uint32_t kb = sorted_keys[start] / spr;
       uint32_t a = start;
       for (uint32_t k = 0; k < n; ++k) {
         const uint32_t e = k + 1 == n ? end : lower_bound(a, end, (uint64_t)(kb + k + 1) * spr);
-        if (g0 + k < max_groups) groups[g0 + k] = Group{a, e - a, (seg_div && e > a) ? sorted_keys[a] / seg_div : 0u, cls};
+        if (g0 + k < max_groups) groups[g0 + k] = Group{a, e - a, 0, cls};
         a = e;
       }
     }
+  }
+}
+
+__global__ void __launch_bounds__(256) k_make_bundles(const uint32_t* __restrict__ offs, uint32_t Wp, uint32_t n_blocks,
+                                                      uint32_t spr, uint32_t maxb, uint32_t maxm, Bundle* __restrict__ bundles,
+                                                      uint32_t max_bundles, uint32_t* __restrict__ status) {
+  __shared__ uint32_t s_off[256];
+  for (uint32_t b0 = 0, total = 0; b0 < n_blocks; b0 += 256) {
+    const uint32_t b = b0 + threadIdx.x;
+    uint32_t n = 0;
+    if (b < n_blocks) n = bundle_cut(offs, b * Wp, b >> 1, b & 1u, Wp, spr, maxb, maxm, [](const Bundle&) {});
+    __syncthreads();
+    s_off[threadIdx.x] = n;
+    __syncthreads();
+    uint32_t o = total;
+    for (uint32_t i = 0; i < threadIdx.x; ++i) o += s_off[i];
+    if (b < n_blocks)
+      bundle_cut(offs, b * Wp, b >> 1, b & 1u, Wp, spr, maxb, maxm, [&](const Bundle& x) {
+        if (o < max_bundles) bundles[o] = x;
+        ++o;
+      });
+    for (uint32_t i = 0; i < 256; ++i) total += s_off[i];
+    if (threadIdx.x == 0 && b0 + 256 >= n_blocks) status[4] = status[5] = min(total, max_bundles);
   }
 }
 
@@ -572,17 +595,18 @@
 #else
 #define PP_SCHED_BARRIER()
 #endif
-template <bool ACC, int SPR, int ROWL, bool SPARSE = false>
+template <bool ACC, int SPR, int ROWL, bool SPARSE = false, int RSPAN = SPR>
 __global__ void __launch_bounds__(GQ2, 4) k_preplace_pairs(
     const double* __restrict__ lookup2, const uint16_t* __restrict__ packed,
     const uint16_t* __restrict__ tails, const uint32_t* __restrict__ win_begin,
     const uint32_t* __restrict__ win_span, const uint32_t* __restrict__ perm,
-    const Group* __restrict__ groups, uint32_t W, uint32_t B, uint32_t pitch, uint32_t NP16,
+    const std::conditional_t<SPARSE, Bundle, Group>* __restrict__ groups, uint32_t W, uint32_t B, uint32_t pitch, uint32_t NP16,
     const uint32_t* __restrict__ status, double* __restrict__ lnl,
     unsigned long long* __restrict__ segmax, uint32_t segp) {
-  constexpr int TR2 = (CH + SPR) / 2;
+  constexpr int TR2 = (CH + RSPAN) / 2;
   extern __shared__ __attribute__((aligned(16))) char smem[];
-  static_assert(ROWL % 16 == 0 && ROWL >= PROWB && ((TR2 - 1) * ROWL + PROWB) < 65536, "16-bit LDS offsets");
+  static_assert(RSPAN >= SPR && (SPARSE || RSPAN == SPR), "only the exact pass stages more than one slice");
+  static_assert(ROWL % 16 == 0 && ROWL >= PROWB && (((CH + SPR) / 2 - 1) * ROWL + PROWB) < 65536, "16-bit LDS offsets");
   double* accs = reinterpret_cast<double*>(smem + (size_t)TR2 * ROWL);
   __shared__ uint32_t s_maxspan;
   __shared__ uint32_t s_qi[GQ2];
@@ -595,15 +619,36 @@
   for (uint32_t item = iw.pos; item < iw.end; item += iw.step) {
   uint32_t item_g = item, item_t = 0;
   if (!SPARSE) item_group_tile(item, iw.lo, iw.end, ng, ntiles, item_g, item_t);
-  const Group g = groups[item_g];
-  const uint32_t b0 = SPARSE ? min(g.min_begin * 64u, B - 1u) : item_t * NBP;
+  uint32_t g_start, g_count, g_lane = (uint32_t)t, b0;
+  uint32_t gmin, gspread, slice0, wboff = 0;
+  if constexpr (SPARSE) {
+    const Bundle* bd = groups + item_g;
+    const uint32_t nmem = bd->nmem, wv = (uint32_t)__builtin_amdgcn_readfirstlane(t >> 6);
+    uint32_t m = 0;
+    for (uint32_t k = 1; k < nmem; ++k) if (wv >= bd->wave[k]) m = k;
+    g_start = bd->start[m];
+    g_count = nmem ? bd->count[m] : 0u;
+    g_lane = (uint32_t)t - bd->wave[m] * 64u;
+    gmin = bd->min_begin[m];
+    slice0 = bd->first;
+    gspread = bd->spread;
+    wboff = ((gmin - slice0) >> 1) * ROWL;
+    b0 = min(bd->seg * 64u, B - 1u);
+    __syncthreads();
+    if (nmem == 0) continue;
+  } else {
+    const Group g = groups[item_g];
+    g_start = g.start;
+    g_count = g.count;
+    b0 = item_t * NBP;
+    __syncthreads();
+    if (g.count == 0) continue;
+  }
   const uint32_t nb = min(NBP, B - b0);
-  __syncthreads();
-  if (g.count == 0) continue;
-  const bool active = t < (int)g.count;
+  const bool active = g_lane < g_count;
   uint32_t qi = 0, begin = 0, span = 0;
   if (active) {
-    qi = perm[g.start + t];
+    qi = perm[g_start + g_lane];
     begin = win_begin[qi];
     span = win_span[qi];
     if ((uint64_t)begin + span > W) span = 0;
@@ -620,8 +665,10 @@
   }
   if (ACC) for (uint32_t j = 0; j < nb; ++j) accs[j * GQ2 + t] = 0.0;
   __syncthreads();
-  const uint32_t gmin = win_begin[perm[g.start]];
-  const uint32_t gspread = win_begin[perm[g.start + g.count - 1]] - gmin;
+  if constexpr (!SPARSE) {
+    gmin = slice0 = win_begin[perm[g_start]];
+    gspread = win_begin[perm[g_start + g_count - 1]] - gmin;
+  }
   const uint32_t rowoff = ((begin - gmin) >> 1) * ROWL;
   const uint32_t rowoff2 = rowoff | (rowoff << 16);
   const uint32_t nchunks = ACC ? (s_maxspan + CH - 1) / CH : 1;
@@ -652,7 +699,7 @@
 #pragma unroll
       for (int i = 0; i < PW; ++i) cw[i] = 0;
     }
-    const uint32_t row0 = gmin + cbase;
+    const uint32_t row0 = slice0 + cbase;
     const uint32_t need = min((uint32_t)TR2, (gspread >> 1) + (min((uint32_t)CH, s_maxspan - cbase) + 1) / 2);
     const uint32_t rows = (row0 < W) ? min(need, (W - row0 + 1) / 2) : 0;
     const uint32_t n2 = rows * (PE / 2);
@@ -758,7 +805,7 @@
         __syncthreads();
         if (j + 1 < nb) request(j + 1, pf);
         PP_SCHED_BARRIER();
-        gather(j, 0);
+        gather(j, SPARSE ? wboff : 0u);
         flush(j);
       }
     }
@@ -999,8 +1046,7 @@
 __global__ void __launch_bounds__(256) k_scatter_cells(const unsigned long long* __restrict__ mask,
                                                        const uint32_t* __restrict__ qkeys, const uint32_t* __restrict__ rank,
                                                        const uint32_t* __restrict__ offs, uint32_t Q, uint32_t seg32p,
-                                                       uint32_t KB, uint32_t ncell, uint32_t* __restrict__ sorted_keys,
-                                                       uint32_t* __restrict__ perm) {
+                                                       uint32_t KB, uint32_t ncell, uint32_t* __restrict__ perm) {
   const uint32_t q = blockIdx.x * 256 + threadIdx.x;
   if (q >= Q) return;
   unsigned long long m = mask[q];
@@ -1009,10 +1055,7 @@
     const uint32_t s = (uint32_t)__ffsll((long long)m) - 1u;
     m &= m - 1;
     const uint32_t key = s * KB + qk, pos = offs[key] + rank[(size_t)q * seg32p + s];
-    if (pos < ncell) {
-      sorted_keys[pos] = key;
-      perm[pos] = q;
-    }
+    if (pos < ncell) perm[pos] = q;
   }
 }
 
@@ -1330,9 +1373,10 @@
     delta = epa_screen_delta(ctx, span_bound);
   }
   const bool screen = delta >= 0.0;
-  uint32_t *seg32, *cstatus, *ccnt, *crank, *csorted, *cperm;
+  const bool screen_only = probe && !probe->full;
+  uint32_t *seg32, *cstatus, *ccnt, *crank, *cperm;
   unsigned long long *seg_mask, *n_incl;
-  Group* cgroups;
+  Bundle* cbundles;
   Group* groups;
   uint16_t *packed, *tails;
   void* temp;
@@ -1352,9 +1396,8 @@
     tails = c.take<uint16_t>((pairs || sites) ? 4 * (size_t)Q : 0);
     seg_mask = c.take<unsigned long long>(screen ? Q : 0);
     crank = c.take<uint32_t>(screen ? (size_t)Q * seg32p : 0);
-    csorted = c.take<uint32_t>(screen ? max_cells : 0);
     cperm = c.take<uint32_t>(screen ? max_cells : 0);
-    cgroups = c.take<Group>(screen ? max_groups_c : 0);
+    cbundles = c.take<Bundle>(screen ? max_groups_c : 0);
     temp = c.tail(temp_bytes);
     return c.off;
   };
@@ -1429,52 +1472,59 @@
                        cstride, crel, nB, pitch, codes_bytes, want_cls, status, lnl);
   };
   if (probe) probe->ran = screen;
-  if (probe && !screen) return EPA_OK;
+  if (screen_only && !screen) return EPA_OK;
   if (screen) {
     using ScreenKernel = decltype(&k_preplace_screen<SPREAD, ROWL_NARROW>);
     const ScreenKernel k_screen = wide ? k_preplace_screen<SPREAD_WIDE, ROWL_PACKED> : k_preplace_screen<SPREAD, ROWL_NARROW>;
-    const FastKernel k_exact = wide ? k_preplace_pairs<false, SPREAD_WIDE, ROWL_PACKED, true> : k_preplace_pairs<false, SPREAD, ROWL_NARROW, true>;
+    constexpr int RSPAN_NARROW = (int)BUNDLE_MAX * SPREAD;
+    using ExactKernel = decltype(&k_preplace_pairs<false, SPREAD, ROWL_NARROW, true, RSPAN_NARROW>);
+    const ExactKernel k_exact = wide ? k_preplace_pairs<false, SPREAD_WIDE, ROWL_PACKED, true, SPREAD_WIDE> : k_preplace_pairs<false, SPREAD, ROWL_NARROW, true, RSPAN_NARROW>;
+    const size_t lds_exact = (wide ? (size_t)((CH + SPREAD_WIDE) / 2) * ROWL_PACKED : (size_t)((CH + RSPAN_NARROW) / 2) * ROWL_NARROW) +
+                             sizeof(double) * NB2_BURST * (GQ2 + 4);
     const size_t lds_scr = wide ? (size_t)((CH + SPREAD_WIDE) / 2) * ROWL_PACKED : (size_t)TROWS2 * ROWL_NARROW;
     EPA_HIP(ctx, hipFuncSetAttribute((const void*)k_screen, hipFuncAttributeMaxDynamicSharedMemorySize, (int)lds_scr));
-    EPA_HIP(ctx, hipFuncSetAttribute((const void*)k_exact, hipFuncAttributeMaxDynamicSharedMemorySize, (int)lds_fast));
+    EPA_HIP(ctx, hipFuncSetAttribute((const void*)k_exact, hipFuncAttributeMaxDynamicSharedMemorySize, (int)lds_exact));
     const uint32_t BP = (ctx->B + 1) / 2;
     struct Events {
       hipEvent_t e[3] = {nullptr, nullptr, nullptr};
       ~Events() { for (hipEvent_t x : e) if (x) (void)hipEventDestroy(x); }
     } evs;
     hipEvent_t* const ev = evs.e;
-    if (probe) for (hipEvent_t& e : evs.e) EPA_HIP(ctx, hipEventCreate(&e));
-    if (probe) EPA_HIP(ctx, hipEventRecord(ev[0], ctx->stream));
+    if (screen_only) for (hipEvent_t& e : evs.e) EPA_HIP(ctx, hipEventCreate(&e));
+    if (screen_only) EPA_HIP(ctx, hipEventRecord(ev[0], ctx->stream));
     else epa_timer_start(ctx, epa_t(ctx, epa_ctx::T_PREPLACE));
     const dim3 grid_s((uint32_t)std::min<uint64_t>((uint64_t)max_groups * ((BP + 15) / 16), (uint64_t)ctx->n_cu));
     hipLaunchKernelGGL(k_screen, grid_s, dim3(GQ2), (uint32_t)lds_scr, ctx->stream, (const float2*)ctx->lookup2f, (const uint16_t*)packed,
                        (const uint16_t*)tails, d_begin, d_span, perm, groups, ctx->W, BP, NP16, status, seg32, seg32p);
-    if (probe) EPA_HIP(ctx, hipEventRecord(ev[1], ctx->stream));
-    const double band = (probe ? probe->band_t : t.band_t) + 2.0 * delta;
+    if (screen_only) EPA_HIP(ctx, hipEventRecord(ev[1], ctx->stream));
+    const double band = (screen_only ? probe->band_t : t.band_t) + 2.0 * delta;
     hipLaunchKernelGGL(k_screen_band, dim3((Q + 255) / 256), dim3(256), 0, ctx->stream, (const uint32_t*)seg32, Q, nseg, seg32p, band,
-                       delta, (const uint32_t*)keys, KB, probe ? nullptr : segmax, segp, probe ? nullptr : ccnt, crank, seg_mask, n_incl);
+                       delta, (const uint32_t*)keys, KB, screen_only ? nullptr : segmax, segp, screen_only ? nullptr : ccnt, crank, seg_mask, n_incl);
     if (probe) {
+      probe->delta = delta;
+      probe->seg32 = seg32;
+      probe->mask = seg_mask;
+      probe->n_incl = n_incl;
+      probe->n_bundles = cstatus + 5;
+    }
+    if (screen_only) {
       EPA_HIP(ctx, hipEventRecord(ev[2], ctx->stream));
       EPA_HIP(ctx, hipGetLastError());
       EPA_HIP(ctx, hipEventSynchronize(ev[2]));
       (void)hipEventElapsedTime(&probe->ms_screen, ev[0], ev[1]);
       (void)hipEventElapsedTime(&probe->ms_band, ev[1], ev[2]);
-      probe->delta = delta;
-      probe->seg32 = seg32;
-      probe->mask = seg_mask;
-      probe->n_incl = n_incl;
       return EPA_OK;
     }
     ++ctx->screen_runs;
     launch_scan_counts(ctx, ccnt, Kc);
     hipLaunchKernelGGL(k_scatter_cells, dim3((Q + 255) / 256), dim3(256), 0, ctx->stream, (const unsigned long long*)seg_mask,
-                       (const uint32_t*)keys, (const uint32_t*)crank, (const uint32_t*)ccnt, Q, seg32p, KB, (uint32_t)max_cells, csorted, cperm);
-    hipLaunchKernelGGL(k_make_groups, dim3(1), dim3(256), smem_c, ctx->stream, (const uint32_t*)csorted, (uint32_t)max_cells, Wp, n_blocks_c,
-                       n_blocks_c, (uint32_t)GQ2, (uint32_t)GQ2, (uint32_t)(wide ? SPREAD_WIDE : SPREAD), max_runs_c, cgroups, max_groups_c,
-                       cstatus, (const uint32_t*)(ccnt + (Kc - 1)), KB);
-    hipLaunchKernelGGL(k_exact, dim3(std::min<uint32_t>(max_groups_c, (uint32_t)ctx->n_cu)), dim3(GQ2), (uint32_t)lds_fast, ctx->stream,
+                       (const uint32_t*)keys, (const uint32_t*)crank, (const uint32_t*)ccnt, Q, seg32p, KB, (uint32_t)max_cells, cperm);
+    const uint32_t maxm = (uint32_t)std::clamp(ctx->opt.preplace_bundle, 1, (int)BUNDLE_MAX);
+    hipLaunchKernelGGL(k_make_bundles, dim3(1), dim3(256), 0, ctx->stream, (const uint32_t*)ccnt, Wp, n_blocks_c,
+                       (uint32_t)(wide ? SPREAD_WIDE : SPREAD), wide ? 1u : BUNDLE_MAX, maxm, cbundles, max_groups_c, cstatus);
+    hipLaunchKernelGGL(k_exact, dim3(std::min<uint32_t>(max_groups_c, (uint32_t)ctx->n_cu)), dim3(GQ2), (uint32_t)lds_exact, ctx->stream,
                        (const double*)ctx->lookup2, (const uint16_t*)packed, (const uint16_t*)tails, d_begin, d_span, (const uint32_t*)cperm,
-                       (const Group*)cgroups, ctx->W, ctx->B, pitch, NP16, (const uint32_t*)cstatus, d_lnl, segmax, segp);
+                       (const Bundle*)cbundles, ctx->W, ctx->B, pitch, NP16, (const uint32_t*)cstatus, d_lnl, segmax, segp);
     kernels(ctx->lookup, ctx->lookup2, ctx->B, d_lnl, segmax, false);
     epa_timer_stop(ctx, epa_t(ctx, epa_ctx::T_PREPLACE));
     EPA_HIP(ctx, hipGetLastError());
diff --git a/epa_ng_amd/csrc/preplace_bundle.hpp b/epa_ng_amd/csrc/preplace_bundle.hpp
--- /dev/null
+++ b/epa_ng_amd/csrc/preplace_bundle.hpp
@@ -0,0 +1,59 @@
+#pragma once
+#include <cstdint>
+
+#if defined(__HIPCC__) || defined(__CUDACC__)
+#define EPA_HD __host__ __device__
+#else
+#define EPA_HD
+#endif
+
+constexpr uint32_t BUNDLE_MAX = 3;
+constexpr uint32_t BUNDLE_LANES = 1024;
+constexpr uint32_t BUNDLE_WAVE = 64;
+
+struct Bundle {
+  uint32_t seg;
+  uint32_t nmem;
+  uint32_t first;
+  uint32_t spread;
+  uint32_t start[BUNDLE_MAX];
+  uint32_t count[BUNDLE_MAX];
+  uint32_t wave[BUNDLE_MAX];
+  uint32_t min_begin[BUNDLE_MAX];
+};
+
+template <class Emit>
+EPA_HD inline uint32_t bundle_cut(const uint32_t* offs, uint32_t key0, uint32_t seg, uint32_t parity, uint32_t wp,
+                                  uint32_t spr, uint32_t maxb, uint32_t maxm, Emit&& emit) {
+  Bundle cur{};
+  uint32_t n_out = 0, lanes = 0, kfirst = 0;
+  auto close = [&]() {
+    if (cur.nmem) { emit(cur); ++n_out; }
+    cur = Bundle{};
+    lanes = 0;
+  };
+  uint32_t a = offs[key0];
+  for (uint32_t k = 0; k * spr < wp; ++k) {
+    const uint32_t e = offs[key0 + ((k + 1) * spr < wp ? (k + 1) * spr : wp)];
+    while (a < e) {
+      const uint32_t n = e - a < BUNDLE_LANES ? e - a : BUNDLE_LANES;
+      const uint32_t w = (n + BUNDLE_WAVE - 1) / BUNDLE_WAVE * BUNDLE_WAVE;
+      if (cur.nmem && (cur.nmem >= maxm || lanes + w > BUNDLE_LANES || k - kfirst >= maxb)) close();
+      if (!cur.nmem) {
+        kfirst = k;
+        cur.seg = seg;
+        cur.first = k * spr + parity;
+      }
+      const uint32_t m = cur.nmem++;
+      cur.start[m] = a;
+      cur.count[m] = n;
+      cur.wave[m] = lanes / BUNDLE_WAVE;
+      cur.min_begin[m] = k * spr + parity;
+      cur.spread = (k + 1) * spr - 2 + parity - cur.first;
+      lanes += w;
+      a += n;
+    }
+  }
+  close();
+  return n_out;
+}
diff --git a/include/epa_dev.h b/include/epa_dev.h
--- a/include/epa_dev.h
+++ b/include/epa_dev.h
@@ -165,6 +165,9 @@
 int epa_dev_preplace_screen_probe(epa_ctx* ctx, const uint8_t* q_codes, const uint32_t* win_begin,
                                   const uint32_t* win_span, uint32_t Q, uint32_t max_span, double threshold,
                                   float* seg32, uint64_t* seg_mask, double* info);
+int epa_dev_preplace_screen_table(epa_ctx* ctx, const uint8_t* q_codes, const uint32_t* win_begin,
+                                  const uint32_t* win_span, uint32_t Q, uint32_t max_span, double threshold,
+                                  double* lnl, uint64_t* seg_keys, uint64_t* seg_mask, double* info);
 uint64_t epa_dev_preplace_screen_runs(const epa_ctx* ctx);
 
 int epa_dev_thorough(epa_ctx* ctx, const epa_pair* pairs, uint64_t n_pairs,
```

Result: no change. 18.02 million placements/s, median of 6 (+0.9%).
